# jibo27/3DGS_Hierarchical_Training

Measured on AMD Instinct MI355X. Metric: train-step images/sec + fwd+bwd ms @1M Gaussians, 980x545; 1/2/4/8 GPU, higher is better.
Workload: dtype f32

## Files before the change

### 3dgs_hierarchical_training_amd/csrc/gsr_kernels.hip

```cpp
#include <hip/hip_runtime.h>
#include <hip/hip_ext.h>
#include <type_traits>
#include <stdint.h>
#include <stdio.h>
#include <string.h>

#include <algorithm>
#include <atomic>
#include <chrono>
#include <cmath>
#include <map>
#include <mutex>
#include <tuple>
#include <vector>

#include "../../include/gsr.h"
#include "gsr_math.h"
#include "adam_math.h"
#include "radix_sort.h"
#include "blend_common.h"
#include "options.h"

#ifndef GSR_K9_UNROLL
#define GSR_K9_UNROLL 2
// ... 861 lines not shown
        uint32_t run = base + (idx ? s_incl[idx - 1] : 0u);
        for (int c0 = 0; c0 < full; c0 += 64) {
            const int c = c0 + lane;
            bool ok = false;
            int gx = 0, gy = 0;
            if (c < full) {
                const int ty = c / ww, tx = c - ty * ww;
                gx = x0 + tx; gy = y0 + ty;
                ok = tile_accept(tt, gx, gy, W, H);
            }
            const unsigned long long m = __ballot(ok);
            if (ok) {
                const uint32_t o = run + (uint32_t)__popcll(m & lt);
                if (o < cap) {
                    const uint32_t key = (uint32_t)((gy + vrow0) * tiles_x + gx);
                    out_tile[o] = (KeyT)key;
                    out_gid[o] = gg;
                    if (hist) count_key(key, o);
                }
            }
            run += (uint32_t)__popcll(m);
        }
    }
    if (hist) {
        __syncthreads();
#pragma unroll
        for (int q = 0; q < 8; q++) {
            const int e = q * kEmitThreads + tid, t = e >> 10, p = (e >> 8) & 3, d = e & 255;
            const uint32_t c = s_hist[t][p][d];
            if (c && x0 + (uint32_t)t < (uint32_t)kOsRanges) atomicAdd(&hz.ghist[((size_t)p * kOsRanges + x0 + t) * 256 + d], c);
        }
    }
}

template <typename KeyT>
__global__ __launch_bounds__(256) void k_tile_ranges(uint32_t R, const KeyT* __restrict__ keys, uint2* __restrict__ ranges,
                                                     const unsigned long long* __restrict__ n_dev)
{
    if (n_dev) R = (uint32_t)min((unsigned long long)R, *n_dev);
    constexpr uint32_t KPV = 16 / (uint32_t)sizeof(KeyT);
    const uint32_t i0 = (blockIdx.x * 256u + threadIdx.x) * KPV;
    if (i0 >= R) return;
    uint32_t t[KPV];
    if (i0 + KPV <= R && (((uintptr_t)keys & 15) == 0)) {
        const uint4 q = *reinterpret_cast<const uint4*>(keys + i0);
        const uint32_t w[4] = {q.x, q.y, q.z, q.w};
#pragma unroll
        for (uint32_t c = 0; c < KPV; c++) t[c] = sizeof(KeyT) == 4 ? w[c] : ((w[c / 2] >> (16 * (c & 1))) & 0xffffu);
    } else {
#pragma unroll
        for (uint32_t c = 0; c < KPV; c++) t[c] = i0 + c < R ? (uint32_t)keys[i0 + c] : 0u;
    }
    uint32_t prev = i0 ? (uint32_t)keys[i0 - 1] : 0xffffffffu;
#pragma unroll
    for (uint32_t c = 0; c < KPV; c++) {
        const uint32_t i = i0 + c;
        if (i < R) {
            if (i == 0) ranges[t[c]].x = 0;
            else if (prev != t[c]) { ranges[prev].y = i; ranges[t[c]].x = i; }
            if (i == R - 1) ranges[t[c]].y = R;
            prev = t[c];
        }
    }
}

constexpr int kDbMaxTiles = 4096;
constexpr int kDbCountWaves = 4;
struct DirectBin {
    int N, T, Tp , S, NC, G, Cg;
    uint16_t* M;
    uint32_t* GT;
    uint32_t* tbase;
    uint32_t* bsum;
};

constexpr uint32_t kCutOpenKey = 0xffffffffu;
struct ListCut {
    uint32_t* key;
    uint32_t* owner_n;
    uint32_t* stats;
    const uint32_t* cur;
    uint16_t* chunk;
    uint32_t* hist;
    uint32_t* tend;
    uint32_t* flag;
    uint32_t* ctl;
    uint32_t* bkey;
    const uint32_t* skey;
    const uint32_t* tbase;
    float margin;
    int dmax;
};

template <typename F>
__device__ __forceinline__ void big_rect_tiles(const Splat& s, uint32_t rect, int W, int H, int tiles_x, int tiles_y, int lane, F&& f)
{
    int x0, y0, x1, y1;
    tile_rect_tight(s.px, s.py, s.radius, s.ca, s.cb, s.cc, s.op, W, H, tiles_x, tiles_y, x0, y0, x1, y1);
    const int vrow0 = (int)((rect >> 12) & 0xfffu) - y0;
    const int ww = x1 - x0, full = ww * (y1 - y0);
    const TileTest tt = make_tile_test(s.px, s.py, s.ca, s.cb, s.cc, s.op);
    for (int c0 = 0; c0 < full; c0 += 64) {
        const int c = c0 + lane;
        bool ok = false;
        uint32_t key = 0u;
        if (c < full) {
            const int ty = c / ww, tx = c - ty * ww;
            ok = tile_accept(tt, x0 + tx, y0 + ty, W, H);
            key = (uint32_t)((y0 + ty + vrow0) * tiles_x + x0 + tx);
        }
        f(ok, key);
    }
}

template <typename F>
__device__ __forceinline__ void small_rect_tiles(const TileRec& r, int tiles_x, F&& f)
{
    const uint32_t ww = (r.rect >> 24) & 63u, rx0 = r.rect & 0xfffu, ry0 = (r.rect >> 12) & 0xfffu;
    const uint32_t rcp = (65536u + ww - 1u) / (ww ? ww : 1u);
    const uint32_t base = ry0 * (uint32_t)tiles_x + rx0, skip = (uint32_t)tiles_x - ww;
    for (uint32_t m = r.mask; m != 0u;) {
        const uint32_t m1 = m & (m - 1u);
        const uint32_t p0 = (uint32_t)__builtin_ctz(m);
        f(base + p0 + ((p0 * rcp) >> 16) * skip);
        if (m1 != 0u) {
            const uint32_t p1 = (uint32_t)__builtin_ctz(m1);
            f(base + p1 + ((p1 * rcp) >> 16) * skip);
        }
        m = m1 & (m1 - 1u);
    }
}

__device__ __forceinline__ uint32_t wave_inclusive_sum(uint32_t x)
{
#if defined(__HIP_DEVICE_COMPILE__)
    auto dpp = [](uint32_t v, auto ctrl, auto rmask, auto bmask) {
        return (uint32_t)__builtin_amdgcn_update_dpp(0, (int)v, decltype(ctrl)::value, decltype(rmask)::value, decltype(bmask)::value, false);
    };
    using std::integral_constant;
    uint32_t r = x;
    r += dpp(x, integral_constant<int, 0x111>{}, integral_constant<int, 0xf>{}, integral_constant<int, 0xf>{});
    r += dpp(x, integral_constant<int, 0x112>{}, integral_constant<int, 0xf>{}, integral_constant<int, 0xf>{});
    r += dpp(x, integral_constant<int, 0x113>{}, integral_constant<int, 0xf>{}, integral_constant<int, 0xf>{});
    r += dpp(r, integral_constant<int, 0x114>{}, integral_constant<int, 0xf>{}, integral_constant<int, 0xe>{});
    r += dpp(r, integral_constant<int, 0x118>{}, integral_constant<int, 0xf>{}, integral_constant<int, 0xc>{});
    r += dpp(r, integral_constant<int, 0x142>{}, integral_constant<int, 0xa>{}, integral_constant<int, 0xf>{});
    r += dpp(r, integral_constant<int, 0x143>{}, integral_constant<int, 0xc>{}, integral_constant<int, 0xf>{});
    return r;
#else
    return x;
#endif
}

__global__ __launch_bounds__(kEmitThreads) void k_chunk_counts(DirectBin db, int W, int H, int tiles_x, int tiles_y,
                                                               const uint32_t* __restrict__ sorted_gid, const TileRec* __restrict__ tilerec,
                                                               const Splat* __restrict__ splat, TileRec* __restrict__ sorted_rec, BlendBalance bb,
                                                               OsRider rider = OsRider{}, ListCut cut = ListCut{})
{
    const int nbuild = bb.hdr ? 8 : 0, c = (int)blockIdx.x - nbuild;
    if (c < 0) { balance_build(bb, (int)blockIdx.x); return; }
    if (cut.key && threadIdx.x == 0) {
        cut.bkey[c] = cut.skey[(size_t)c * db.S];
        cut.hist[c] = 0u;
        if (c == 0) { cut.ctl[0] = (uint32_t)(db.NC - 1); cut.ctl[1] = 0u; cut.ctl[2] = 0u; }
    }
    if (rider.host && blockIdx.x == gridDim.x - 1) {
        __shared__ unsigned long long s_r[2][16];
        onesweep_rider_publish(rider, s_r);
    }
    extern __shared__ uint32_t s_h[];
    const int tid = threadIdx.x, lane = tid & 63, wave = tid >> 6;
    for (int i = tid; i < db.Tp / 2; i += kEmitThreads) s_h[i] = 0u;
    __syncthreads();
    const int j0 = c * db.S + wave * 64, j1 = min(db.N, c * db.S + db.S);
    constexpr int kStride = 64 * kDbCountWaves;
    auto load_gid = [&](int j) -> uint32_t { return j < j1 ? (sorted_gid ? sorted_gid[j] : (uint32_t)j) : 0xffffffffu; };
    auto load_rec = [&](uint32_t g) -> TileRec { TileRec r; r.mask = 0u; r.rect = 1u << 24; if (g != 0xffffffffu) r = tilerec[g]; return r; };
    uint32_t gA = load_gid(j0 + lane), gB = load_gid(j0 + kStride + lane);
    TileRec rA = load_rec(gA);
    for (int j = j0 + lane; j - lane < j1; j += kStride) {
        const uint32_t g = gA;
        const TileRec r = rA;
        gA = gB;
        rA = load_rec(gA);
        gB = load_gid(j + 2 * kStride);
        if (sorted_rec && j < j1) sorted_rec[j] = r;
        const bool big = (r.rect & kTileRecBig) != 0u;
        if (!big) small_rect_tiles(r, tiles_x, [&](uint32_t t) { atomicAdd(&s_h[t >> 1], 1u << (16u * (t & 1u))); });
        for (unsigned long long bm = __ballot(big && r.mask != 0u); bm != 0ull; bm &= bm - 1ull) {
            const int b = (int)__builtin_ctzll(bm);
            const uint32_t gg = (uint32_t)__builtin_amdgcn_readlane((int)g, b), rect = (uint32_t)__builtin_amdgcn_readlane((int)r.rect, b);
            const Splat s = splat[gg];
            big_rect_tiles(s, rect, W, H, tiles_x, tiles_y, lane, [&](bool ok, uint32_t t) { if (ok) atomicAdd(&s_h[t >> 1], 1u << (16u * (t & 1u))); });
        }
    }
    __syncthreads();
    uint32_t* const row = reinterpret_cast<uint32_t*>(db.M + (size_t)c * db.Tp);
    for (int i = tid; i < db.Tp / 2; i += kEmitThreads) row[i] = s_h[i];
}

__global__ __launch_bounds__(256) void k_chunk_scan1(DirectBin db)
{
    __shared__ uint32_t s_w[4];
    const int tid = threadIdx.x, t = (int)(blockIdx.x * 256u) + tid, grp = (int)blockIdx.y;
    uint32_t run = 0u;
    if (t < db.Tp) {
        const int c0 = grp * db.Cg, c1 = min(db.NC, c0 + db.Cg);
        uint16_t* p = db.M + (size_t)c0 * db.Tp + t;
        int c = c0;
        for (; c + 8 <= c1; c += 8, p += 8 * (size_t)db.Tp) {
            uint32_t v[8];
#pragma unroll
            for (int k = 0; k < 8; k++) v[k] = p[(size_t)k * db.Tp];
#pragma unroll
            for (int k = 0; k < 8; k++) { p[(size_t)k * db.Tp] = (uint16_t)run; run += v[k]; }
        }
        for (; c < c1; c++, p += db.Tp) { const uint32_t v = *p; *p = (uint16_t)run; run += v; }
        db.GT[(size_t)grp * db.Tp + t] = run;
    }
    const uint32_t inc = wave_inclusive_sum(run);
    if ((tid & 63) == 63) s_w[tid >> 6] = inc;
    __syncthreads();
    if (tid == 0) db.bsum[(size_t)grp * gridDim.x + blockIdx.x] = s_w[0] + s_w[1] + s_w[2] + s_w[3];
}

constexpr int kDbMaxGroups = 64;
__global__ __launch_bounds__(256) void k_chunk_scan2(DirectBin db, unsigned long long* __restrict__ total_out, ZeroJobs zj,
                                                     unsigned long long* __restrict__ host_out, unsigned long long host_seq,
                                                     const unsigned int* __restrict__ window_overflow, unsigned long long* __restrict__ late_out = nullptr,
                                                     ListCut cut = ListCut{})
{
    extern __shared__ uint32_t s_bkey[];
    __shared__ unsigned long long s_lo[4], s_all[4];
    if (cut.key)
        for (int i = threadIdx.x; i < db.NC; i += 256) s_bkey[i] = cut.bkey[i];
    __shared__ uint32_t s_w[4];
    const int tid = threadIdx.x, lane = tid & 63, wave = tid >> 6;
    const int slab = (int)blockIdx.x, nslab = (int)gridDim.x, t = slab * 256 + tid;
#pragma unroll
    for (int j = 0; j < 3; j++) {
        uint32_t* z = static_cast<uint32_t*>(zj.p[j]);
        for (uint32_t q = (uint32_t)(slab * 256 + tid); q < zj.words[j]; q += (uint32_t)nslab * 256u) z[q] = 0u;
    }
    unsigned long long lo = 0ull, all = 0ull;
    for (int i = tid; i < db.G * nslab; i += 256) {
        const uint32_t v = db.bsum[i];
        all += v;
        if (i % nslab < slab) lo += v;
    }
#pragma unroll
    for (int off = 32; off > 0; off >>= 1) { lo += __shfl_xor(lo, off, 64); all += __shfl_xor(all, off, 64); }
    if (lane == 0) { s_lo[wave] = lo; s_all[wave] = all; }
    uint32_t tot = 0u;
    if (t < db.Tp) {
        uint32_t v[kDbMaxGroups];
#pragma unroll
        for (int g = 0; g < kDbMaxGroups; g++) v[g] = g < db.G ? db.GT[(size_t)g * db.Tp + t] : 0u;
#pragma unroll
        for (int g = 0; g < kDbMaxGroups; g++) {
            if (g < db.G) db.GT[(size_t)g * db.Tp + t] = tot;
            tot += v[g];
        }
    }
    if (t >= db.T) tot = 0u;
    const uint32_t inc = wave_inclusive_sum(tot);
    if (lane == 63) s_w[wave] = inc;
    __syncthreads();
    lo = s_lo[0] + s_lo[1] + s_lo[2] + s_lo[3];
    all = s_all[0] + s_all[1] + s_all[2] + s_all[3];
    uint32_t add = 0u;
#pragma unroll
    for (int w = 0; w < 4; w++) add += w < wave ? s_w[w] : 0u;
    const uint32_t base_t = (uint32_t)min(lo + add + inc - tot, 0xffffffffull);
    if (t < db.T) db.tbase[t] = base_t;
    if (cut.key) {
        if (t < db.T) {
            const uint32_t e = cut.cur[0] < (uint32_t)kVcEntries ? cut.cur[0] : 0u;
            const bool use = cut.cur[9] != 0u && cut.owner_n[e] == (uint32_t)db.N;
            uint32_t ck = (uint32_t)(db.NC - 1);
            const uint32_t k = use ? cut.key[(size_t)e * db.T + t] : kCutOpenKey;
            if (k != kCutOpenKey && k != 0u) {
                const float d = __uint_as_float(k);
                const uint32_t kc = __float_as_uint(fmaf(d, cut.margin, d));
                int a = 0, b = db.NC;
                while (a < b) { const int m = (a + b) >> 1; if (s_bkey[m] <= kc) a = m + 1; else b = m; }
                ck = (uint32_t)max(a - 1, 0);
            }
            cut.chunk[t] = (uint16_t)ck;
            cut.flag[t] = 0u;
            if (use) atomicAdd(&cut.hist[ck], 1u);
            if (t == 0) cut.ctl[3] = use ? 1u : 0u;
        }
    }
    if (slab == 0 && tid == 0) {
        db.tbase[db.T] = (uint32_t)min(all, 0xffffffffull);
        *total_out = all;
        if (host_out) {
            __atomic_store_n(host_out + 2, (unsigned long long)g_onesweep_giveups, __ATOMIC_RELAXED);
            __atomic_store_n(host_out + 3, (unsigned long long)(window_overflow ? *window_overflow : 0u), __ATOMIC_RELAXED);
            __atomic_store_n(host_out, all, __ATOMIC_RELAXED);
            __threadfence_system();
            __atomic_store_n(host_out + 1, host_seq, __ATOMIC_RELAXED);
            __threadfence_system();
        }
        if (late_out) scan_report_late(late_out, all, host_seq);
    }
}

constexpr int kDbPairs = 1024;
__device__ __forceinline__ void lds_order() { __builtin_amdgcn_fence(__ATOMIC_ACQ_REL, "wavefront"); __builtin_amdgcn_wave_barrier(); }

__device__ __forceinline__ uint32_t cut_frame(const ListCut& cut, const int NC, uint32_t& deep)
{
    const int lane = threadIdx.x & 63;
    deep = 0u;
    if (cut.ctl[3] == 0u) return (uint32_t)(NC - 1);
    constexpr int kR = 32;
    uint32_t v[kR];
#pragma unroll
    for (int q = 0; q < kR; q++) { const int c = NC - 1 - 64 * q - lane; v[q] = (64 * q < NC && c >= 0) ? cut.hist[c] : 0u; }
    uint32_t acc = 0u;
#pragma unroll
    for (int q = 0; q < kR; q++) {
        if (64 * q >= NC) break;
        const int c = NC - 1 - 64 * q - lane;
        const uint32_t inc = acc + wave_inclusive_sum(v[q]);
        const unsigned long long over = __ballot(c >= 0 && inc > (uint32_t)cut.dmax);
        if (over) {
            const int l = (int)__builtin_ctzll(over);
            deep = (uint32_t)__builtin_amdgcn_readlane((int)(inc - v[q]), l);
            return (uint32_t)(NC - 1 - 64 * q - l);
        }
        acc = (uint32_t)__builtin_amdgcn_readlane((int)inc, 63);
    }
    for (int top = NC - 1 - 64 * kR; top >= 0; top -= 64) {
        const int c = top - lane;
        const uint32_t w = c >= 0 ? cut.hist[c] : 0u;
        const uint32_t inc = acc + wave_inclusive_sum(w);
        const unsigned long long over = __ballot(c >= 0 && inc > (uint32_t)cut.dmax);
        if (over) {
            const int l = (int)__builtin_ctzll(over);
            deep = (uint32_t)__builtin_amdgcn_readlane((int)(inc - w), l);
            return (uint32_t)(top - l);
        }
        acc = (uint32_t)__builtin_amdgcn_readlane((int)inc, 63);
    }
    deep = acc;
    return 0u;
}

template <typename Want>
__device__ __forceinline__ void cut_chunk_tiles(const DirectBin& db, const int c, const int W, const int H, const int tiles_x, const int tiles_y,
                                                const uint32_t* __restrict__ sorted_gid, const TileRec* __restrict__ sorted_rec,
                                                const Splat* __restrict__ splat, uint32_t* __restrict__ list, const uint32_t cap,
                                                uint32_t* s_txy , uint32_t* s_pos , Want&& want)
{
    const int lane = threadIdx.x & 63;
    const unsigned long long lt = lanemask_lt();
    const int j0 = c * db.S, j1 = min(db.N, j0 + db.S);
    const uint32_t* gt = db.GT + (size_t)(c / db.Cg) * db.Tp;
    const uint16_t* mr = db.M + (size_t)c * db.Tp;
    auto load_rec = [&](int j) -> TileRec { TileRec r; r.mask = 0u; r.rect = 1u << 24; if (j < j1) r = sorted_rec[j]; return r; };
    auto load_gid = [&](int j) -> uint32_t { return j < j1 ? sorted_gid[j] : 0u; };
    unsigned long long mine = 0ull;
#pragma unroll
    for (int q = 0; q < kDbMaxTiles / 64; q++) {
        const int t = 64 * q + lane;
        if (64 * q < db.T && t < db.T && want((uint32_t)t)) mine |= 1ull << q;
    }
    for (int t0 = 0; t0 < db.T;) {
        int nt = 0;
        while (t0 < db.T) {
            const int t = t0 + lane;
            const bool w = ((mine >> (t0 >> 6)) & 1ull) != 0ull;
            const unsigned long long b = __ballot(w);
            const int got = (int)__popcll(b);
            if (nt + got > 64) break;
            if (w) {
                const int k = nt + (int)__popcll(b & lt);
                s_txy[k] = ((uint32_t)(t / tiles_x) << 16) | (uint32_t)(t % tiles_x);
                s_pos[k] = db.tbase[t] + gt[t] + (uint32_t)mr[t];
            }
            nt += got;
            t0 += 64;
        }
        if (nt == 0) break;
        lds_order();
        TileRec rA = load_rec(j0 + lane), rB = load_rec(j0 + 64 + lane);
        uint32_t gA = load_gid(j0 + lane), gB = load_gid(j0 + 64 + lane);
        for (int j = j0; j < j1; j += 64) {
            const TileRec r = rA;
            const uint32_t g = gA;
            rA = rB; gA = gB;
            rB = load_rec(j + 128 + lane);
            gB = load_gid(j + 128 + lane);
            const bool big = (r.rect & kTileRecBig) != 0u && r.mask != 0u;
            const uint32_t ww = (r.rect >> 24) & 63u, rx0 = r.rect & 0xfffu, ry0 = (r.rect >> 12) & 0xfffu;
            TileTest tt = {};
            int bx0 = 0, by0 = 0, bx1 = 0, by1 = 0;
            if (big) {
                const Splat sp = splat[g];
                tile_rect_tight(sp.px, sp.py, sp.radius, sp.ca, sp.cb, sp.cc, sp.op, W, H, tiles_x, tiles_y, bx0, by0, bx1, by1);
                tt = make_tile_test(sp.px, sp.py, sp.ca, sp.cb, sp.cc, sp.op);
            }
            const bool any_big = __ballot(big) != 0ull;
            for (int k = 0; k < nt; k++) {
                const uint32_t txy = s_txy[k], tx = txy & 0xffffu, ty = txy >> 16;
                const uint32_t dx = tx - rx0, dy = ty - ry0, bit = dy * ww + dx;
                bool in = !big && dx < ww && bit < 32u && ((r.mask >> bit) & 1u) != 0u;
                if (any_big && big) in = (int)tx >= bx0 && (int)tx < bx1 && (int)ty >= by0 && (int)ty < by1 && tile_accept(tt, (int)tx, (int)ty, W, H);
                const unsigned long long b = __ballot(in);
                if (b == 0ull) continue;
                const uint32_t p0 = s_pos[k];
                if (in) { const uint32_t pos = p0 + (uint32_t)__popcll(b & lt); if (pos < cap) list[pos] = g; }
                lds_order();
                if (lane == 0) s_pos[k] = p0 + (uint32_t)__popcll(b);
                lds_order();
            }
        }
        lds_order();
    }
}

#ifdef GSR_DB_TIMING
__device__ unsigned long long g_db_dbg[16];
#define DB_T(k) do { const unsigned long long now_ = __builtin_readcyclecounter(); if (lane == 0) dbt[k] += now_ - dbt_last; dbt_last = now_; } while (0)
#else
#define DB_T(k) do { } while (0)
#endif
template <bool PAIRS = false, int CUT = 0>
__global__ __launch_bounds__(64) void k_chunk_scatter(DirectBin db, int W, int H, int tiles_x, int tiles_y,
                                                      const uint32_t* __restrict__ sorted_gid, const TileRec* __restrict__ sorted_rec,
                                                      const Splat* __restrict__ splat, uint32_t* __restrict__ list, uint2* __restrict__ ranges,
                                                      uint32_t cap, const uint32_t* __restrict__ dkey = nullptr, uint2* __restrict__ pairs = nullptr,
                                                      ListCut cut = ListCut{})
{
    static_assert(!CUT || !PAIRS, "the list cut serves the plain direct binning");
    extern __shared__ unsigned long long s_dyn[];
    const int LT = db.Tp;
    unsigned long long* const s_mask = s_dyn;
    uint32_t* const s_cnt = reinterpret_cast<uint32_t*>(s_dyn + LT);
    uint32_t* const s_pair = s_cnt + LT;
    const int lane = threadIdx.x, b = (int)blockIdx.x;
    if (CUT == 2 && cut.ctl[2] == 0u) return;
    uint32_t cstar = 0u, ndeep = 0u;
    if (CUT == 1) cstar = cut_frame(cut, db.NC, ndeep);
    if (CUT == 2) cstar = cut.ctl[0];
    {
        const int t = b * 64 + lane;
        if (t < db.T) {
            uint32_t tend = db.tbase[t + 1];
            if (CUT == 1) {
                const uint32_t c1 = max((uint32_t)cut.chunk[t], cstar) + 1u;
                if (c1 < (uint32_t)db.NC) tend = db.tbase[t] + db.GT[(size_t)(c1 / (uint32_t)db.Cg) * db.Tp + t] + (uint32_t)db.M[(size_t)c1 * db.Tp + t];
                cut.tend[t] = tend;
            }
            const uint32_t lo = min(db.tbase[t], cap), hi = min(tend, cap);
            if (CUT != 2 || cut.flag[t]) ranges[t] = hi > lo ? make_uint2(lo, hi) : make_uint2(0u, 0u);
            if (CUT == 1) {
                const uint32_t e = cut.cur[0] < (uint32_t)kVcEntries ? cut.cur[0] : 0u;
                cut.key[(size_t)e * db.T + t] = 0u;
            }
        }
        if (CUT && b == 0 && lane == 0) {
            if (CUT == 1) {
                const uint32_t e = cut.cur[0] < (uint32_t)kVcEntries ? cut.cur[0] : 0u;
                cut.owner_n[e] = (uint32_t)db.N;
                cut.ctl[0] = cstar; cut.ctl[1] = ndeep;
                cut.stats[0] += 1u;
                cut.stats[3] += (uint32_t)(db.NC - 1) - min(cstar, (uint32_t)(db.NC - 1));
                cut.stats[4] += ndeep;
            } else { cut.stats[1] += 1u; cut.stats[2] += cut.ctl[2]; }
        }
    }
    const int per = (db.NC + 7) >> 3, kk = b >> 3, c = (b & 7) * per + kk;
    if (kk >= per || c >= db.NC) return;
    if (CUT && (uint32_t)c > cstar) {
        if (CUT == 1 && ndeep == 0u) return;
        uint32_t* const s_tile = s_pair;
        uint32_t* const s_pos = s_pair + 64;
        if (CUT == 1) cut_chunk_tiles(db, c, W, H, tiles_x, tiles_y, sorted_gid, sorted_rec, splat, list, cap, s_tile, s_pos,
                                      [&](uint32_t t) { return (uint32_t)cut.chunk[t] >= (uint32_t)c; });
        else cut_chunk_tiles(db, c, W, H, tiles_x, tiles_y, sorted_gid, sorted_rec, splat, list, cap, s_tile, s_pos,
                             [&](uint32_t t) { return cut.flag[t] != 0u && (uint32_t)cut.chunk[t] < (uint32_t)c; });
        return;
    }
    if (CUT == 2) return;
#ifdef GSR_DB_TIMING
    unsigned long long dbt[8] = {0, 0, 0, 0, 0, 0, 0, 0}, dbt_last = __builtin_readcyclecounter();
#endif
    {
        const uint32_t* gt = db.GT + (size_t)(c / db.Cg) * db.Tp;
        const uint16_t* mr = db.M + (size_t)c * db.Tp;
        constexpr int kRows = 36;
        for (int i0 = 0; i0 < LT; i0 += 64 * kRows) {
            uint32_t tb[kRows], gb[kRows], mc[kRows];
#pragma unroll
            for (int q = 0; q < kRows; q++) {
                const int i = i0 + 64 * q + lane;
                const bool v = i < LT && (uint32_t)i < (uint32_t)LT;
                tb[q] = v && i < db.T ? db.tbase[i] : 0u;
                gb[q] = v ? gt[i] : 0u;
                mc[q] = v ? (uint32_t)mr[i] : 0u;
            }
#pragma unroll
            for (int q = 0; q < kRows; q++) {
                const int i = i0 + 64 * q + lane;
                if (i < LT) { s_cnt[i] = tb[q] + gb[q] + mc[q]; s_mask[i] = 0ull; }
            }
        }
    }
    lds_order();
    DB_T(0);
    const unsigned long long me = 1ull << lane, lt = lanemask_lt();
    const int j0 = c * db.S, j1 = min(db.N, j0 + db.S);
    auto load_gid = [&](int j) -> uint32_t { return j < j1 ? (PAIRS ? (uint32_t)j : sorted_gid[j]) : 0u; };
    auto load_rec = [&](int j) -> TileRec { TileRec r; r.mask = 0u; r.rect = 1u << 24; if (j < j1) r = sorted_rec[j]; return r; };
    auto load_key = [&](int j) -> uint32_t { return (PAIRS && j < j1) ? dkey[j] : 0u; };
    uint32_t gA = load_gid(j0 + lane), gB = load_gid(j0 + 64 + lane);
    TileRec rA = load_rec(j0 + lane), rB = load_rec(j0 + 64 + lane);
    uint32_t kA = load_key(j0 + lane), kB = load_key(j0 + 64 + lane);
    for (int j = j0 + lane; j - lane < j1; j += 64) {
        const uint32_t g = gA;
        TileRec r = rA;
        const uint32_t kd = kA;
        gA = gB; rA = rB; kA = kB;
        gB = load_gid(j + 128);
        rB = load_rec(j + 128);
        kB = load_key(j + 128);
        const bool big = (r.rect & kTileRecBig) != 0u && r.mask != 0u, huge = big && r.mask > (uint32_t)kDbPairs;
        const unsigned long long bigs = __ballot(big && !huge), huges = __ballot(huge);
        const uint32_t cnt = huge ? 0u : tilerec_count(r);
        const uint32_t incl = wave_inclusive_sum(cnt);
        auto run_end = [&](int lo, uint32_t before) -> int {
            const unsigned long long over = __ballot(incl - before > (uint32_t)kDbPairs) & ~((1ull << lo) - 1ull);
            return over ? (int)__builtin_ctzll(over) : 64;
        };
        auto owners = [&](int lo, int hi, uint32_t before, bool with_or) {
            const bool mine = lane >= lo && lane < hi;
            if (!big && (with_or || mine)) {
                uint32_t* o = s_pair + (incl - cnt - before);
                small_rect_tiles(r, tiles_x, [&](uint32_t t) {
                    if (with_or) atomicOr(&s_mask[t], me);
                    if (mine) *o++ = (t << 6) | (uint32_t)lane;
                });
            }
            for (unsigned long long bm = bigs; bm != 0ull; bm &= bm - 1ull) {
                const int bl = (int)__builtin_ctzll(bm);
                const bool in_run = bl >= lo && bl < hi;
                if (!with_or && !in_run) continue;
                const uint32_t gg = (uint32_t)__builtin_amdgcn_readlane((int)g, bl), rect = (uint32_t)__builtin_amdgcn_readlane((int)r.rect, bl);
                uint32_t o = (uint32_t)__builtin_amdgcn_readlane((int)(incl - cnt), bl) - before;
                const Splat s = splat[gg];
                big_rect_tiles(s, rect, W, H, tiles_x, tiles_y, lane, [&](bool ok, uint32_t t) {
                    const unsigned long long acc = __ballot(ok);
                    if (ok) {
                        if (with_or) atomicOr(&s_mask[t], 1ull << bl);
                        if (in_run) s_pair[(o + (uint32_t)__popcll(acc & lt)) & (uint32_t)(kDbPairs - 1)] = (t << 6) | (uint32_t)bl;
                    }
                    o += (uint32_t)__popcll(acc);
                });
            }
        };
        int lo = 0, hi = run_end(0, 0u);
        uint32_t before = 0u;
        const bool one_run = hi == 64;
        DB_T(1);
        owners(0, hi, 0u, true);
        DB_T(2);
        for (unsigned long long bm = huges; bm != 0ull; bm &= bm - 1ull) {
            const int bl = (int)__builtin_ctzll(bm);
            const uint32_t gg = (uint32_t)__builtin_amdgcn_readlane((int)g, bl), rect = (uint32_t)__builtin_amdgcn_readlane((int)r.rect, bl);
            const Splat s = splat[gg];
            big_rect_tiles(s, rect, W, H, tiles_x, tiles_y, lane, [&](bool ok, uint32_t t) { if (ok && t < (uint32_t)db.T) atomicOr(&s_mask[t], 1ull << bl); });
        }
        asm volatile("" : "+v"(gA), "+v"(rA.mask), "+v"(rA.rect));
        if (PAIRS) asm volatile("" : "+v"(kA));
        lds_order();
        DB_T(3);
        for (;;) {
            const uint32_t P = (uint32_t)__builtin_amdgcn_readlane((int)incl, hi - 1) - before;
            for (uint32_t p0 = 0u; p0 < P; p0 += 512u) {
                const uint32_t left = P - p0;
                auto batch = [&](auto rounds_tag) {
                    constexpr int RN = decltype(rounds_tag)::value;
                    uint32_t e[RN], go[RN], base[RN], ko[PAIRS ? RN : 1];
                    unsigned long long mk[RN];
#pragma unroll
                    for (int q = 0; q < RN; q++) e[q] = s_pair[(p0 + 64u * q + (uint32_t)lane) & (uint32_t)(kDbPairs - 1)];
#pragma unroll
                    for (int q = 0; q < RN; q++) {
                        const bool v = 64u * q + (uint32_t)lane < left;
                        e[q] = v ? e[q] : 0xffffffffu;
                        const uint32_t t = v ? e[q] >> 6 : 0u;
                        go[q] = (uint32_t)__builtin_amdgcn_ds_bpermute((int)((e[q] & 63u) << 2), (int)g);
                        if (PAIRS) ko[q] = (uint32_t)__builtin_amdgcn_ds_bpermute((int)((e[q] & 63u) << 2), (int)kd);
                        mk[q] = s_mask[t];
                        base[q] = s_cnt[t];
                    }
#pragma unroll
                    for (int q = 0; q < RN; q++)
                        if (e[q] != 0xffffffffu) {
                            const uint32_t pos = base[q] + (uint32_t)__popcll(mk[q] & ((1ull << (e[q] & 63u)) - 1ull));
                            if (pos < cap) {
                                if (PAIRS) pairs[pos] = make_uint2(ko[q], go[q]);
                                else list[pos] = go[q];
                            }
                        }
                };
                if (left <= 128u) batch(std::integral_constant<int, 2>{});
                else if (left <= 256u) batch(std::integral_constant<int, 4>{});
                else if (left <= 384u) batch(std::integral_constant<int, 6>{});
                else batch(std::integral_constant<int, 8>{});
            }
            if (hi == 64) break;
            lds_order();
            before += P;
            lo = hi;
            hi = run_end(lo, before);
            owners(lo, hi, before, false);
            lds_order();
        }
        for (unsigned long long bm = huges; bm != 0ull; bm &= bm - 1ull) {
            const int bl = (int)__builtin_ctzll(bm);
            const uint32_t gg = (uint32_t)__builtin_amdgcn_readlane((int)g, bl), rect = (uint32_t)__builtin_amdgcn_readlane((int)r.rect, bl);
            const Splat s = splat[gg];
            big_rect_tiles(s, rect, W, H, tiles_x, tiles_y, lane, [&](bool ok, uint32_t t) {
                if (ok && t < (uint32_t)db.T) {
                    const uint32_t pos = s_cnt[t] + (uint32_t)__popcll(s_mask[t] & ((1ull << bl) - 1ull));
                    if (pos < cap) {
                        if (PAIRS) pairs[pos] = make_uint2((uint32_t)__builtin_amdgcn_readlane((int)kd, bl), gg);
                        else list[pos] = gg;
                    }
                }
            });
        }
        lds_order();
        DB_T(4);
        if (one_run) {
            const uint32_t P = (uint32_t)__builtin_amdgcn_readlane((int)incl, 63);
            for (uint32_t p0 = 0u; p0 < P; p0 += 512u) {
                const uint32_t left = P - p0;
                auto batch = [&](auto rounds_tag) {
                    constexpr int RN = decltype(rounds_tag)::value;
                    uint32_t e[RN];
#pragma unroll
                    for (int q = 0; q < RN; q++) e[q] = s_pair[(p0 + 64u * q + (uint32_t)lane) & (uint32_t)(kDbPairs - 1)];
#pragma unroll
                    for (int q = 0; q < RN; q++)
                        if (64u * q + (uint32_t)lane < left) { atomicAdd(&s_cnt[e[q] >> 6], 1u); s_mask[e[q] >> 6] = 0ull; }
                };
                if (left <= 128u) batch(std::integral_constant<int, 2>{});
                else if (left <= 256u) batch(std::integral_constant<int, 4>{});
                else if (left <= 384u) batch(std::integral_constant<int, 6>{});
                else batch(std::integral_constant<int, 8>{});
            }
        } else {
            if (!big) small_rect_tiles(r, tiles_x, [&](uint32_t t) { atomicAdd(&s_cnt[t], 1u); s_mask[t] = 0ull; });
            for (unsigned long long bm = bigs; bm != 0ull; bm &= bm - 1ull) {
                const int bl = (int)__builtin_ctzll(bm);
                const uint32_t gg = (uint32_t)__builtin_amdgcn_readlane((int)g, bl), rect = (uint32_t)__builtin_amdgcn_readlane((int)r.rect, bl);
                const Splat s = splat[gg];
                big_rect_tiles(s, rect, W, H, tiles_x, tiles_y, lane, [&](bool ok, uint32_t t) { if (ok && t < (uint32_t)db.T) { atomicAdd(&s_cnt[t], 1u); s_mask[t] = 0ull; } });
            }
        }
        for (unsigned long long bm = huges; bm != 0ull; bm &= bm - 1ull) {
            const int bl = (int)__builtin_ctzll(bm);
            const uint32_t gg = (uint32_t)__builtin_amdgcn_readlane((int)g, bl), rect = (uint32_t)__builtin_amdgcn_readlane((int)r.rect, bl);
            const Splat s = splat[gg];
            big_rect_tiles(s, rect, W, H, tiles_x, tiles_y, lane, [&](bool ok, uint32_t t) { if (ok && t < (uint32_t)db.T) { atomicAdd(&s_cnt[t], 1u); s_mask[t] = 0ull; } });
        }
        lds_order();
        DB_T(5);
    }
#ifdef GSR_DB_TIMING
    if (lane == 0) {
        for (int k = 0; k < 6; k++) atomicAdd(&g_db_dbg[k], dbt[k]);
        atomicAdd(&g_db_dbg[6], 1ull);
        atomicAdd(&g_db_dbg[7], (unsigned long long)((j1 - j0 + 63) / 64));
    }
#endif
}

constexpr int kTsCap = 4096, kTsSmallMax = 1024;

template <int THREADS, int IPT, bool GATHER = false>
__device__ __forceinline__ void tile_sort_regs(const uint2* __restrict__ src, uint32_t* dst, uint32_t n, const uint32_t* __restrict__ dkey,
                                               unsigned long long (*s_mask)[256], uint32_t (*s_cnt)[256], uint32_t* s_keys, uint32_t* s_vals,
                                               uint32_t* s_start, uint32_t* s_wsum, uint32_t* s_bits)
{
    constexpr int WAVES = THREADS / 64;
    const int tid = threadIdx.x, wave = tid >> 6, lane = tid & 63;
    uint32_t key[IPT], val[IPT], dig[IPT], rnk[IPT];
    uint32_t k_or = 0u, k_and = 0xffffffffu;
#pragma unroll
    for (int r = 0; r < IPT; r++) {
        const uint32_t p = (uint32_t)(wave * (IPT * 64) + r * 64 + lane);
        if (GATHER) val[r] = p < n ? dst[p] : 0u;
        else if (p < n) { const uint2 e = src[p]; key[r] = e.x; val[r] = e.y; }
        if (!GATHER && p >= n) { key[r] = 0xffffffffu; val[r] = 0u; }
    }
    if (GATHER) {
#pragma unroll
        for (int r = 0; r < IPT; r++) {
            const uint32_t p = (uint32_t)(wave * (IPT * 64) + r * 64 + lane);
            key[r] = p < n ? dkey[val[r]] : 0xffffffffu;
        }
    }
#pragma unroll
    for (int r = 0; r < IPT; r++) {
        const uint32_t p = (uint32_t)(wave * (IPT * 64) + r * 64 + lane);
        if (p < n) { k_or |= key[r]; k_and &= key[r]; }
    }
#pragma unroll
    for (int off = 32; off > 0; off >>= 1) { k_or |= (uint32_t)__shfl_xor((int)k_or, off, 64); k_and &= (uint32_t)__shfl_xor((int)k_and, off, 64); }
    if (lane == 0) { s_bits[wave] = k_or; s_bits[WAVES + wave] = k_and; }
    __syncthreads();
    uint32_t differ = 0u;
    {
        uint32_t o = 0u, a = 0xffffffffu;
#pragma unroll
        for (int w = 0; w < WAVES; w++) { o |= s_bits[w]; a &= s_bits[WAVES + w]; }
        differ = o & ~a;
    }
#pragma unroll 1
    for (int shift = 0; shift < 32; shift += 8) {
        if (((differ >> shift) & 0xffu) == 0u) continue;
#pragma unroll
        for (int r = 0; r < IPT; r++) dig[r] = (key[r] >> shift) & 0xffu;
        wave_rank<IPT, 256>(s_mask[wave], s_cnt[wave], dig, rnk, lane);
        __syncthreads();
        uint32_t mine = 0u;
        if (tid < 256) {
#pragma unroll
            for (int w = 0; w < WAVES; w++) { const uint32_t c = s_cnt[w][tid]; s_cnt[w][tid] = mine; mine += c; }
        }
        const uint32_t ex = block_scan_excl<WAVES>(mine, s_wsum, tid);
        if (tid < 256) s_start[tid] = ex;
        __syncthreads();
#pragma unroll
        for (int r = 0; r < IPT; r++) {
            const uint32_t lp = s_start[dig[r]] + s_cnt[wave][dig[r]] + rnk[r];
            s_keys[lp] = key[r]; s_vals[lp] = val[r];
        }
        __syncthreads();
#pragma unroll
        for (int r = 0; r < IPT; r++) {
            const uint32_t p = (uint32_t)(wave * (IPT * 64) + r * 64 + lane);
            key[r] = s_keys[p]; val[r] = s_vals[p];
        }
        __syncthreads();
    }
#pragma unroll
    for (int r = 0; r < IPT; r++) {
        const uint32_t p = (uint32_t)(wave * (IPT * 64) + r * 64 + lane);
        if (p < n) dst[p] = val[r];
    }
}

template <int IPT, bool GATHER>
__device__ __forceinline__ void tile_sort_wave(const uint2* __restrict__ src, uint32_t* dst, uint32_t n, const uint32_t* __restrict__ dkey,
                                               unsigned long long* s_mask, uint32_t* s_cnt, uint32_t* s_start, uint32_t* s_keys, uint32_t* s_vals)
{
    const int lane = threadIdx.x;
    uint32_t key[IPT], val[IPT], dig[IPT], rnk[IPT];
#pragma unroll
    for (int r = 0; r < IPT; r++) {
        const uint32_t p = (uint32_t)(r * 64 + lane);
        if (GATHER) val[r] = p < n ? dst[p] : 0u;
        else if (p < n) { const uint2 e = src[p]; key[r] = e.x; val[r] = e.y; }
        if (!GATHER && p >= n) { key[r] = 0xffffffffu; val[r] = 0u; }
    }
    if (GATHER) {
#pragma unroll
        for (int r = 0; r < IPT; r++) key[r] = (uint32_t)(r * 64 + lane) < n ? dkey[val[r]] : 0xffffffffu;
    }
    uint32_t k_or = 0u, k_and = 0xffffffffu;
#pragma unroll
    for (int r = 0; r < IPT; r++)
        if ((uint32_t)(r * 64 + lane) < n) { k_or |= key[r]; k_and &= key[r]; }
#pragma unroll
    for (int off = 32; off > 0; off >>= 1) { k_or |= (uint32_t)__shfl_xor((int)k_or, off, 64); k_and &= (uint32_t)__shfl_xor((int)k_and, off, 64); }
    const uint32_t differ = k_or & ~k_and;
#pragma unroll 1
    for (int shift = 0; shift < 32; shift += 8) {
        if (((differ >> shift) & 0xffu) == 0u) continue;
#pragma unroll
        for (int r = 0; r < IPT; r++) dig[r] = (key[r] >> shift) & 0xffu;
        wave_rank<IPT, 256>(s_mask, s_cnt, dig, rnk, lane);
        lds_order();
        {
            const uint4 c = reinterpret_cast<const uint4*>(s_cnt)[lane];
            const uint32_t sum = c.x + c.y + c.z + c.w;
            const uint32_t ex = wave_inclusive_sum(sum) - sum;
            reinterpret_cast<uint4*>(s_start)[lane] = make_uint4(ex, ex + c.x, ex + c.x + c.y, ex + c.x + c.y + c.z);
        }
        lds_order();
#pragma unroll
        for (int r = 0; r < IPT; r++) {
            const uint32_t lp = s_start[dig[r]] + rnk[r];
            s_keys[lp] = key[r]; s_vals[lp] = val[r];
        }
        lds_order();
#pragma unroll
        for (int r = 0; r < IPT; r++) { key[r] = s_keys[r * 64 + lane]; val[r] = s_vals[r * 64 + lane]; }
        lds_order();
    }
#pragma unroll
    for (int r = 0; r < IPT; r++) {
        const uint32_t p = (uint32_t)(r * 64 + lane);
        if (p < n) dst[p] = val[r];
    }
}

template <bool GATHER = false>
__global__ __launch_bounds__(64) void k_tile_sort_wave(const uint2* __restrict__ ranges, const uint2* __restrict__ pairs, uint32_t* list, int T,
                                                       const uint32_t* __restrict__ dkey = nullptr)
{
    __shared__ unsigned long long s_mask[256];
    __shared__ __attribute__((aligned(16))) uint32_t s_cnt[256];
    __shared__ __attribute__((aligned(16))) uint32_t s_start[256];
    __shared__ uint32_t s_keys[kTsSmallMax], s_vals[kTsSmallMax];
    const int t = (int)blockIdx.x;
    if (t >= T) return;
    const uint2 rg = ranges[t];
    const uint32_t n = rg.y - rg.x;
    if (n == 0u || n > (uint32_t)kTsSmallMax) return;
    const uint2* src = pairs + rg.x;
    uint32_t* dst = list + rg.x;
    if (n <= 64u) tile_sort_wave<1, GATHER>(src, dst, n, dkey, s_mask, s_cnt, s_start, s_keys, s_vals);
    else if (n <= 128u) tile_sort_wave<2, GATHER>(src, dst, n, dkey, s_mask, s_cnt, s_start, s_keys, s_vals);
    else if (n <= 256u) tile_sort_wave<4, GATHER>(src, dst, n, dkey, s_mask, s_cnt, s_start, s_keys, s_vals);
    else if (n <= 512u) tile_sort_wave<8, GATHER>(src, dst, n, dkey, s_mask, s_cnt, s_start, s_keys, s_vals);
    else tile_sort_wave<16, GATHER>(src, dst, n, dkey, s_mask, s_cnt, s_start, s_keys, s_vals);
}

template <int THREADS, bool GATHER = false>
__global__ __launch_bounds__(THREADS) void k_tile_sort(const uint2* __restrict__ ranges, uint2* pairs, uint2* pairs_alt, uint32_t* list, int T,
                                                       const uint32_t* __restrict__ dkey = nullptr)
{
    constexpr int WAVES = THREADS / 64, CAP = THREADS == 256 ? kTsSmallMax : kTsCap;
    static_assert(CAP * 8 == WAVES * 256 * 8, "the pair buffer aliases the mask tables exactly");
    __shared__ unsigned long long s_mask[WAVES][256];
    __shared__ uint32_t s_cnt[WAVES][256];
    __shared__ uint32_t s_start[256], s_wsum[WAVES], s_bits[2 * WAVES], s_base[256], s_hist[256];
    uint32_t* const s_keys = reinterpret_cast<uint32_t*>(&s_mask[0][0]);
    uint32_t* const s_vals = s_keys + CAP;
    static_assert(THREADS == 1024, "the short segments are k_tile_sort_wave's");
    __shared__ uint32_t s_todo[256];
    __shared__ uint32_t s_ntodo;
    if (threadIdx.x == 0) s_ntodo = 0u;
    __syncthreads();
    for (int k = (int)threadIdx.x; (int)blockIdx.x + k * (int)gridDim.x < T; k += THREADS) {
        const int tt = (int)blockIdx.x + k * (int)gridDim.x;
        const uint2 q = ranges[tt];
        if (q.y - q.x > (uint32_t)kTsSmallMax) { const uint32_t slot = atomicAdd(&s_ntodo, 1u); if (slot < 256u) s_todo[slot] = (uint32_t)tt; }
    }
    __syncthreads();
    const uint32_t ntodo = s_ntodo;
    const bool walk_all = ntodo > 256u;
    const int nloop = walk_all ? (T - (int)blockIdx.x + (int)gridDim.x - 1) / (int)gridDim.x : (int)ntodo;
    for (int it = 0; it < nloop; it++) {
    const int t = walk_all ? (int)blockIdx.x + it * (int)gridDim.x : (int)s_todo[it];
    const uint2 rg = ranges[t];
    const uint32_t n = rg.y - rg.x;
    if (n <= (uint32_t)kTsSmallMax) continue;
    __syncthreads();
    if (n <= 2048u) { tile_sort_regs<THREADS, 2, GATHER>(pairs + rg.x, list + rg.x, n, dkey, s_mask, s_cnt, s_keys, s_vals, s_start, s_wsum, s_bits); continue; }
    if (n <= (uint32_t)kTsCap) { tile_sort_regs<THREADS, 4, GATHER>(pairs + rg.x, list + rg.x, n, dkey, s_mask, s_cnt, s_keys, s_vals, s_start, s_wsum, s_bits); continue; }
    const int tid = threadIdx.x, wave = tid >> 6, lane = tid & 63;
    constexpr int IPT = kTsCap / THREADS;
    uint2* src = pairs + rg.x;
    uint2* dst = pairs_alt + rg.x;
    if (GATHER) {
        for (uint32_t i = (uint32_t)tid; i < n; i += THREADS) { const uint32_t g = list[rg.x + i]; src[i] = make_uint2(dkey[g], g); }
        __syncthreads();
    }
    uint32_t k_or = 0u, k_and = 0xffffffffu;
    for (uint32_t i = (uint32_t)tid; i < n; i += THREADS) { const uint32_t k = src[i].x; k_or |= k; k_and &= k; }
#pragma unroll
    for (int off = 32; off > 0; off >>= 1) { k_or |= (uint32_t)__shfl_xor((int)k_or, off, 64); k_and &= (uint32_t)__shfl_xor((int)k_and, off, 64); }
    if (lane == 0) { s_bits[wave] = k_or; s_bits[WAVES + wave] = k_and; }
    __syncthreads();
    uint32_t differ = 0u;
    {
        uint32_t o = 0u, a = 0xffffffffu;
#pragma unroll
        for (int w = 0; w < WAVES; w++) { o |= s_bits[w]; a &= s_bits[WAVES + w]; }
        differ = o & ~a;
    }
#pragma unroll 1
    for (int shift = 0; shift < 32; shift += 8) {
        if (((differ >> shift) & 0xffu) == 0u) continue;
        __syncthreads();
        if (tid < 256) s_hist[tid] = 0u;
        __syncthreads();
        for (uint32_t i = (uint32_t)tid; i < n; i += THREADS) atomicAdd(&s_hist[(src[i].x >> shift) & 0xffu], 1u);
        __syncthreads();
        const uint32_t tot = tid < 256 ? s_hist[tid] : 0u;
        const uint32_t ex = block_scan_excl<WAVES>(tot, s_wsum, tid);
        if (tid < 256) s_base[tid] = ex;
        __syncthreads();
        for (uint32_t c0 = 0u; c0 < n; c0 += (uint32_t)kTsCap) {
            const uint32_t m = min((uint32_t)kTsCap, n - c0);
            uint32_t key[IPT], val[IPT], dig[IPT], rnk[IPT];
#pragma unroll
            for (int r = 0; r < IPT; r++) {
                const uint32_t p = (uint32_t)(wave * (IPT * 64) + r * 64 + lane);
                if (p < m) { const uint2 e = src[c0 + p]; key[r] = e.x; val[r] = e.y; dig[r] = (e.x >> shift) & 0xffu; }
                else { key[r] = 0xffffffffu; val[r] = 0u; dig[r] = 255u; }
            }
            wave_rank<IPT, 256>(s_mask[wave], s_cnt[wave], dig, rnk, lane);
            __syncthreads();
            uint32_t mine = 0u;
            if (tid < 256) {
#pragma unroll
                for (int w = 0; w < WAVES; w++) { const uint32_t c = s_cnt[w][tid]; s_cnt[w][tid] = mine; mine += c; }
                s_start[tid] = s_base[tid];
            }
            __syncthreads();
            if (tid < 256) s_base[tid] += mine - (tid == 255 ? (uint32_t)kTsCap - m : 0u);
#pragma unroll
            for (int r = 0; r < IPT; r++) {
                const uint32_t p = (uint32_t)(wave * (IPT * 64) + r * 64 + lane);
                if (p < m) dst[s_start[dig[r]] + s_cnt[wave][dig[r]] + rnk[r]] = make_uint2(key[r], val[r]);
            }
            __syncthreads();
        }
        uint2* tmp = src; src = dst; dst = tmp;
    }
    __syncthreads();
    for (uint32_t i = (uint32_t)tid; i < n; i += THREADS) list[rg.x + i] = src[i].y;
    }
}

#ifdef GSR_K6_TIMING
__device__ unsigned long long g_k6_dbg[4 * 65536];
__device__ unsigned long long g_k8_dbg[4 * 65536];
__device__ unsigned long long g_k6_cyc[2 * 65536];
__device__ uint32_t g_k6_cnt[2 * 65536];
#endif
#ifndef GSR_FWD_BUFS
#define GSR_FWD_BUFS 2
#endif
constexpr int kFwdBufs = GSR_FWD_BUFS;

struct ImpArgs {
    const float* color;
    float* S;
    float (*s_sum)[64];
    uint32_t* s_id;
};
constexpr int kImpStride = 4;
__device__ __forceinline__ float wave_swap_rows_sum(float t)
{
    {
        const unsigned u = __float_as_uint(t);
        const auto r = __builtin_amdgcn_permlane16_swap(u, u, false, false);
        t = __uint_as_float(r[0]) + __uint_as_float(r[1]);
    }
    {
        const unsigned u = __float_as_uint(t);
        const auto r = __builtin_amdgcn_permlane32_swap(u, u, false, false);
        t = __uint_as_float(r[0]) + __uint_as_float(r[1]);
    }
    return t;
}
__device__ __forceinline__ float wave_reduce_one(float v)
{
    return wave_swap_rows_sum(bfly_single<0x128>(bfly_single<0x124>(bfly_single<0x4E>(bfly_single<0xB1>(v)))));
}
__device__ __forceinline__ float wave_reduce_three(float v0, float v1, float v2, int lane)
{
    const float r01 = bfly_pair<0x124>(v0, v1, (lane & 4) != 0);
    const float r2 = bfly_single<0x124>(v2);
    const float q = bfly_pair<0x128>(r01, r2, (lane & 8) != 0);
    return wave_swap_rows_sum(bfly_single<0x4E>(bfly_single<0xB1>(q)));
}

template <bool IMP = false, bool LEAN = false, bool HAS_DA = true>
__device__ __forceinline__ void blend_fwd_item(const int xcd, const int kslot, float4 (*s_ab)[64], float2 (*s_c)[64],
                                               int W, int H, int tiles_x, int T, const uint2* __restrict__ ranges,
                                               const uint32_t* __restrict__ list, const Splat* __restrict__ splat,
                                               const float* __restrict__ bg, float* __restrict__ out_color,
                                               float* __restrict__ out_depth, float* __restrict__ out_alpha,
                                               float* __restrict__ img, uint32_t* __restrict__ staged4,
                                               float* __restrict__ ckpt, int kCkptFirst, int tiles_y, uint16_t* __restrict__ cost_out,
                                               float* __restrict__ out_clamped, const ListCut& cut, const int cut_pass,
                                               const ImpArgs imp = ImpArgs{})
{
    constexpr int NT = 64;
    uint32_t visits = 0u;
#ifdef GSR_K6_TIMING
    const unsigned long long dbg_t0 = wall_clock64();
    uint32_t dbg_visits = 0u, dbg_taken = 0u;
    unsigned long long dbg_stage = 0ull, dbg_loop = 0ull, dbg_mark = 0ull;
#endif
    const int tile = slot_tile(xcd, kslot >> 2, T, tiles_x);
    const int sub = kslot & 3;
    const int lane = (int)(threadIdx.x & 63u);
    if (tile < 0) { if (cost_out && lane == 0) cost_out[xcd + 8 * kslot] = 0; return; }
    if (cut_pass == 2 && cut.flag[tile] == 0u) return;
    const int Tl = tiles_x * tiles_y, bimg = tile / Tl, tl = tile - bimg * Tl;
    const int tx = tl % tiles_x, ty = tl / tiles_x;
    const int px = tx * kTile + (sub & 1) * 8 + (lane & 7);
    const int py = ty * kTile + (sub >> 1) * 8 + (lane >> 3);
    const float pxf = (float)((sub & 1) * 8 + (lane & 7)), pyf = (float)((sub >> 1) * 8 + (lane >> 3));
    const float tox = (float)(tx * kTile) - 0.5f * (float)W, toy = (float)(ty * kTile) - 0.5f * (float)H;
    const uint2 rg = ranges[tile];
    const int n = IMP ? min((int)(rg.y - rg.x), (int)staged4[tile * 4 + sub]) : (int)(rg.y - rg.x);
    const int nb = (n + NT - 1) / NT;
    const bool inside = px < W && py < H;
    float Tr = inside ? 1.f : -1.f;
    float C0 = 0.f, C1 = 0.f, C2 = 0.f, Dd = 0.f, Aa = 0.f;
    uint32_t last = 0;
    float g0 = 0.f, g1 = 0.f, g2 = 0.f;
    uint32_t lastp = 0u, id_rec = 0u;
    bool uni = false;
    if constexpr (IMP) {
        if (inside) {
            const size_t Pl = (size_t)W * H, P = Pl * (size_t)(T / Tl), pl = (size_t)py * W + px, pid = (size_t)bimg * Pl + pl;
            const float* oc = imp.color + (size_t)bimg * 3 * Pl + pl;
            const float o0 = oc[0], o1 = oc[Pl], o2 = oc[2 * Pl];
            g0 = (o0 >= 0.f && o0 <= 1.f) ? 1.f : 0.f;
            g1 = (o1 >= 0.f && o1 <= 1.f) ? 1.f : 0.f;
            g2 = (o2 >= 0.f && o2 <= 1.f) ? 1.f : 0.f;
            lastp = reinterpret_cast<const uint32_t*>(img)[P + pid];
        }
        const bool want = lastp > 0u && (g0 + g1 + g2) > 0.f;
        if (!__any(want)) return;
        Tr = want ? 1.f : -1.f;
        if (!want) g0 = g1 = g2 = 0.f;
        uni = __all(g0 == g1 && g1 == g2);
        imp.s_sum[0][lane] = 0.f; imp.s_sum[1][lane] = 0.f; imp.s_sum[2][lane] = 0.f;
    }
    float4 ra = {0, 0, 0, 0}, rb = ra, rc = ra;
    constexpr float kL2E = 1.4426950408889634f;
    const float sbx0 = (float)(tx * kTile + (sub & 1) * 8) - 0.5f * (float)W, sby0 = (float)(ty * kTile + (sub >> 1) * 8) - 0.5f * (float)H;
    const float sbx1 = fminf(sbx0 + 7.f, (float)(W - 1) - 0.5f * (float)W), sby1 = fminf(sby0 + 7.f, (float)(H - 1) - 0.5f * (float)H);
    uint32_t id_nn = 0u;
    auto fetch = [&](uint32_t id) {
        const float4* sp = reinterpret_cast<const float4*>(splat + id);
        ra = sp[0]; rb = sp[1]; rc = sp[2];
    };
    if (n > 0) {
        id_rec = list[rg.x + min(lane, n - 1)];
        fetch(id_rec);
        id_nn = list[rg.x + min(NT + lane, n - 1)];
    }
    int batches = 0;
    for (int b = 0; b < nb; b++) {
        const int buf = b & (kFwdBufs - 1);
        if (__all(Tr < 0.f)) break;
        if constexpr (!LEAN) {
        if (ckpt && !(b & 1) && (b >> 1) >= kCkptFirst) {
            float* c = ckpt + ((size_t)(rg.x >> 7) + tile + (b >> 1) - kCkptFirst) * kCkptFloats + sub * 64 + lane;
            c[0] = fabsf(Tr); c[256] = C0; c[512] = C1; c[768] = C2; c[1024] = Dd; c[1280] = Aa;
        }
        }
#ifdef GSR_K6_TIMING
        dbg_mark = __builtin_readcyclecounter();
#endif
        const int cnt = min(NT, n - b * NT);
        const bool reach_me = box_accept(make_tile_test(ra.x, ra.y, ra.z, ra.w, rb.x, rb.y), sbx0, sby0, sbx1, sby1);
        {
            const uint32_t lo = __float_as_uint(rc.w);
            ra.x = pixel_rel(ra.x, pixel_lo_x(lo), tox); ra.y = pixel_rel(ra.y, pixel_lo_y(lo), toy);
        }
        ra.z *= -0.5f * kL2E; ra.w *= -kL2E; rb.x *= -0.5f * kL2E;
        s_ab[buf][lane] = ra; s_ab[kFwdBufs + buf][lane] = rb;
        if constexpr (IMP) imp.s_id[lane] = id_rec;
        else s_c[buf][lane] = make_float2(rc.x, rc.y);
        const unsigned long long reach = __ballot(reach_me && lane < cnt);
        visits += (uint32_t)__popcll(reach);
        __builtin_amdgcn_fence(__ATOMIC_RELEASE, "wavefront");
        __builtin_amdgcn_wave_barrier();
        __builtin_amdgcn_fence(__ATOMIC_ACQUIRE, "wavefront");
        batches = b + 1;
#ifdef GSR_K6_TIMING
        { const unsigned long long t = __builtin_readcyclecounter(); dbg_stage += t - dbg_mark; dbg_mark = t; }
#endif
        const int nxt = (b + 1) * NT + lane;
        fetch(id_nn);
        if constexpr (IMP) id_rec = id_nn;
        id_nn = list[rg.x + min(nxt + NT, n - 1)];
        auto alpha_of = [&](int j, float& p2) {
// ... 1354 lines not shown
                d_shs[(size_t)(base + g) * row + e] = e < NC3 ? s_sh[g * kShStride + e] : 0.f;
            }
        }
    }
}

__global__ __launch_bounds__(256) void k_det_iota(uint32_t R, uint32_t* __restrict__ pos, const uint32_t* __restrict__ list, uint32_t* __restrict__ ids,
                                                  uint32_t n_gaussians)
{
    const uint32_t i = blockIdx.x * 256u + threadIdx.x;
    if (i < R) { pos[i] = i; ids[i] = min(list[i], n_gaussians - 1u); }
}
__global__ __launch_bounds__(256) void k_det_reduce(uint32_t R, const uint32_t* __restrict__ gid_sorted, const uint32_t* __restrict__ pos_sorted,
                                                    const float* __restrict__ part, double* __restrict__ ggrad)
{
    const uint32_t i = blockIdx.x * 256u + threadIdx.x;
    if (i >= R) return;
    const uint32_t g = gid_sorted[i];
    if (i > 0 && gid_sorted[i - 1] == g) return;
    double acc[kDetStride];
#pragma unroll
    for (int r = 0; r < kDetStride; r++) acc[r] = 0.0;
    for (uint32_t j = i; j < R && gid_sorted[j] == g; j++) {
        const float* p = part + (size_t)pos_sorted[j] * kDetStride;
#pragma unroll
        for (int r = 0; r < kDetStride; r++) acc[r] += (double)p[r];
    }
#pragma unroll
    for (int r = 0; r < kDetStride; r++) ggrad[(size_t)g * kGG + r] = acc[r];
}

__global__ __launch_bounds__(256) void k_cam_reduce(const float* __restrict__ partial, int nblocks, float* __restrict__ d_vm,
                                                    float* __restrict__ d_pm, float* __restrict__ d_campos, float* __restrict__ d_xf,
                                                    BatchDev bt)
{
    __shared__ double s[256];
    const int q = blockIdx.x, m = blockIdx.y;
    int lo = 0, hi = nblocks;
    if (bt.B > 1) {
#pragma unroll
        for (int k = 0; k < kMaxBatch; k++)
            if (k == m) { lo = bt.first_block[k]; hi = min(nblocks, bt.first_block[k + 1]); }
        if (d_vm) d_vm += 16 * m;
        if (d_pm) d_pm += 16 * m;
        if (d_campos) d_campos += 3 * m;
        if (d_xf) d_xf += 12 * m;
    }
    double a = 0;
    for (int b = lo + threadIdx.x; b < hi; b += 256) a += partial[(size_t)b * kCamVals + q];
    s[threadIdx.x] = a;
    __syncthreads();
    for (int off = 128; off > 0; off >>= 1) {
        if (threadIdx.x < off) s[threadIdx.x] += s[threadIdx.x + off];
        __syncthreads();
    }
    if (threadIdx.x == 0) {
        const float v = (float)s[0];
        if (q < 16) { if (d_vm) d_vm[q] = v; }
        else if (q < 32) { if (d_pm) d_pm[q - 16] = v; }
        else if (q < 35) { if (d_campos) d_campos[q - 32] = v; }
        else if (d_xf) d_xf[q - 35] = v;
    }
}

struct GeomLayout {
    size_t splat;
    size_t total;
};
static GeomLayout geom_layout(int32_t N)
{
    GeomLayout g;
    g.splat = 0;
    g.total = align256((size_t)(N > 0 ? N : 1) * sizeof(Splat));
    return g;
}

struct PrepLayout {
    size_t splat, radii, dkey, gid, rec, sort, early, bytes;
};
static PrepLayout prep_layout(int32_t N)
{
    const size_t n = (size_t)(N > 0 ? N : 1);
    PrepLayout p;
    size_t o = 0;
    p.splat = o; o += align256(n * sizeof(Splat));
    p.radii = o; o += align256(n * 4);
    p.dkey = o; o += align256(n * 4);
    p.gid = o; o += align256(n * 4);
    p.rec = o; o += align256(n * sizeof(TileRec));
    p.sort = o; o += align256(onesweep_scratch_bytes((uint32_t)n));
    p.early = o; o += align256(((n + kPreThreads - 1) / kPreThreads) * sizeof(uint2));
    p.bytes = o;
    return p;
}

struct FwdScratch {
    size_t dkey, gid, dkey_alt, gid_alt, ntiles, srec, block_sums, total, early, sort;
    size_t bytes;
};
static FwdScratch fwd_scratch_layout(int32_t N)
{
    const size_t n = (size_t)(N > 0 ? N : 1);
    FwdScratch s;
    size_t o = 0;
    s.dkey = o; o += align256(n * 4);
    s.gid = o; o += align256(n * 4);
    s.dkey_alt = o; o += align256(n * 4);
    s.gid_alt = o; o += align256(n * 4);
    s.ntiles = o; o += align256(n * sizeof(TileRec));
    s.srec = o; o += align256(n * sizeof(TileRec));
    s.block_sums = o; o += align256(((n + kEmitThreads - 1) / kEmitThreads) * 4);
    s.total = o; o += 256;
    s.early = o; o += align256(((n + kPreThreads - 1) / kPreThreads) * sizeof(uint2));
    s.sort = o; o += onesweep_scratch_bytes((uint32_t)n);
    s.bytes = o;
    return s;
}

struct BinLayout {
    size_t list, ranges, ckpt, items, bytes;
};

static size_t bwd_list_cap(int64_t R, size_t T) { return ((size_t)(R > 0 ? R : 0) >> 7) + T + 8; }
static BinLayout bin_layout(int64_t R, int32_t W, int32_t H, int32_t B = 1)
{
    const size_t T = (size_t)((W + kTile - 1) / kTile) * ((H + kTile - 1) / kTile) * (size_t)(B > 1 ? B : 1);
    BinLayout b;
    b.ranges = 0;
    b.list = align256((T ? T : 1) * sizeof(uint2));
    b.ckpt = b.list + align256((size_t)(R > 0 ? R : 1) * 4);
    b.items = b.ckpt + align256((((size_t)(R > 0 ? R : 0) >> 7) + T + 1) * kCkptFloats * sizeof(float));
    b.bytes = b.items + kItemHdrBytes + align256(8 * bwd_list_cap(R, T) * sizeof(uint2));
    return b;
}

struct BinScratch {
    size_t tile, tile_alt, gid_alt, sort, bytes;
};
static BinScratch bin_scratch_layout(int64_t R, int key_bytes = 4)
{
    const size_t r = (size_t)(R > 0 ? R : 1);
    BinScratch s;
    size_t o = 0;
    s.tile = o; o += align256(r * (size_t)key_bytes);
    s.tile_alt = o; o += align256(r * (size_t)key_bytes);
    s.gid_alt = o; o += align256(r * 4);
    s.sort = o; o += onesweep_scratch_bytes((uint32_t)r);
    s.bytes = o;
    return s;
}

struct ViewCostCache { int dev, W, H, items; uint8_t* mem; size_t bytes; };
static std::vector<ViewCostCache> g_view_costs;
static std::map<std::tuple<int, int, int, int>, bool> g_full_depth_sort;

struct PinSlot { unsigned long long* host = nullptr; unsigned long long* dev = nullptr; bool busy = false;
                 unsigned long long seq = 0;
                 bool pending = false; unsigned long long pending_seq = 0, pending_R = 0, pending_giveups = 0; };
static std::mutex g_state_mutex;
static std::map<int, std::vector<PinSlot*>> g_pin_slots;
static std::map<std::tuple<int, int, int, int>, uint64_t> g_hints;
static long long g_hint_override = -1;
static long long g_late_bias = 0;
static std::atomic<long long> g_spec_overflows{0}, g_spec_forwards{0}, g_exact_forwards{0}, g_depth_window_resorts{0};
static std::atomic<long long> g_fwd_calls{0}, g_fwd_ns{0}, g_fwd_wait_ns{0}, g_bwd_calls{0}, g_bwd_ns{0}, g_frozen_bwd_calls{0};
struct CallTimer {
    std::atomic<long long>&calls, &ns;
    std::chrono::steady_clock::time_point t0 = std::chrono::steady_clock::now();
    CallTimer(std::atomic<long long>& c, std::atomic<long long>& n) : calls(c), ns(n) {}
    ~CallTimer() { calls++; ns += std::chrono::duration_cast<std::chrono::nanoseconds>(std::chrono::steady_clock::now() - t0).count(); }
};

static int n_bucket(int N) { return N > 0 ? (int)std::floor(2.0 * std::log2((double)N)) : 0; }

static PinSlot* acquire_pin_slot(int dev)
{
    std::lock_guard<std::mutex> lk(g_state_mutex);
    auto& v = g_pin_slots[dev];
    for (PinSlot* s : v)
        if (!s->busy) { s->busy = true; return s; }
    PinSlot* s = new PinSlot();
    if (hipHostMalloc((void**)&s->host, 64, hipHostMallocMapped) != hipSuccess ||
        hipHostGetDevicePointer((void**)&s->dev, s->host, 0) != hipSuccess) { delete s; return nullptr; }
    s->host[0] = 0; s->host[1] = 0;
    for (int q = 4; q < 8; q++) s->host[q] = 0;
    s->busy = true;
    v.push_back(s);
    return s;
}
static std::atomic<long long> g_late_checks{0}, g_late_mismatches{0};
static int late_check(PinSlot* s, bool wait, unsigned long long* got_total, unsigned long long* want_total)
{
    if (!s->pending) return 0;
    volatile unsigned long long* hp = s->host;
    if (hp[5] != s->pending_seq) {
        if (!wait) return 0;
        const auto limit = std::chrono::steady_clock::now() + std::chrono::milliseconds(200);
        while (hp[5] != s->pending_seq && std::chrono::steady_clock::now() < limit) cpu_relax();
        if (hp[5] != s->pending_seq) { (void)hipDeviceSynchronize(); }
        if (hp[5] != s->pending_seq) { s->pending = false; return 0; }
    }
    std::atomic_thread_fence(std::memory_order_acquire);
    s->pending = false;
    g_late_checks++;
    *got_total = hp[4]; *want_total = s->pending_R;
    if (hp[4] != s->pending_R || hp[6] != s->pending_giveups) { g_late_mismatches++; return 1; }
    return 0;
}
struct PinLease {
    PinSlot* s;
    explicit PinLease(PinSlot* s_) : s(s_) {}
    ~PinLease() { if (s) { std::lock_guard<std::mutex> lk(g_state_mutex); s->busy = false; } }
};

static inline int64_t pack_fwd_flags(int ckpt_first)
{
    return 1 | ((int64_t)7 << 1) | ((int64_t)2 << 4) | ((int64_t)ckpt_first << 6) | ((int64_t)1 << 13);
}
static inline bool flags_from_forward(int64_t flags) { return ((flags >> 1) & 7) == 7 && ((flags >> 4) & 3) == 2; }

static int batch_dev(const GsrBatch* bt, int32_t N, int32_t H, BatchDev& out)
{
    out = BatchDev{};
    out.B = 1;
    if (!bt || bt->B <= 1) return GSR_OK;
    if (bt->B > kMaxBatch || !bt->first_block) return fail(GSR_ERR_ARG, "batch: 2..16 models and a first_block table expected%s");
    const int nblocks = (N + kPreThreads - 1) / kPreThreads;
    if (bt->first_block[0] != 0 || bt->first_block[bt->B] != nblocks || (N % kPreThreads) != 0)
        return fail(GSR_ERR_ARG, "batch: first_block must run from 0 to N / 128 and N must be a multiple of 128 (pad every model)%s");
    for (int q = 0; q < bt->B; q++)
        if (bt->first_block[q + 1] < bt->first_block[q]) return fail(GSR_ERR_ARG, "batch: first_block must be non-decreasing%s");
    if ((long long)bt->B * ((H + kTile - 1) / kTile) > 4095) return fail(GSR_ERR_RANGE, "batch: more than 4095 tile rows in total%s");
    out.B = bt->B;
    for (int q = 0; q <= bt->B; q++) out.first_block[q] = bt->first_block[q];
    for (int q = bt->B + 1; q <= kMaxBatch; q++) out.first_block[q] = nblocks;
    return GSR_OK;
}

static int check_common(int32_t N, int32_t M, int32_t D, int32_t W, int32_t H)
{
    if (N < 0 || W <= 0 || H <= 0) return fail(GSR_ERR_ARG, "bad sizes%s");
    if (D < 0 || D > 3) return fail(GSR_ERR_ARG, "sh_degree must be 0..3%s");
    if (M < 0 || M > 16) return fail(GSR_ERR_ARG, "at most 16 SH coefficients per Gaussian%s");
    if (W > 4095 * kTile || H > 4095 * kTile) return fail(GSR_ERR_RANGE, "image side longer than 65520 pixels%s");
    return GSR_OK;
}

template <typename KeyT>
static int sort_pairs_entry(KeyT* keys, uint32_t* vals, KeyT* keys_alt, uint32_t* vals_alt, uint32_t n, int begin_bit, int end_bit, void* scratch,
                            size_t scratch_bytes, int* result_in_alt, void* stream)
{
    if (!result_in_alt) return fail(GSR_ERR_ARG, "sort: result_in_alt is null%s");
    if (scratch_bytes < onesweep_scratch_bytes(n)) return fail(GSR_ERR_ARG, "sort scratch too small%s");
    if (begin_bit < 0 || end_bit <= begin_bit || end_bit > 8 * (int)sizeof(KeyT)) return fail(GSR_ERR_ARG, "sort bit range outside the key%s");
    GSR_HIP(onesweep_sort_pairs<KeyT>(keys, vals, keys_alt, vals_alt, n, begin_bit, end_bit, scratch, result_in_alt, (hipStream_t)stream));
    return GSR_OK;
}

}

using namespace gsr;

extern "C" {

size_t gsr_geom_bytes(int32_t N) { return geom_layout(N).total; }
static size_t image_balance_offset(int32_t W, int32_t H, int32_t B) { return align256((size_t)W * H * (size_t)(B > 1 ? B : 1) * kImgPlanes * 4); }
static size_t image_balance_bytes(int32_t W, int32_t H, int32_t B)
{
    if (B > 1) return 0;
    const int tiles_x = (W + kTile - 1) / kTile, T = tiles_x * ((H + kTile - 1) / kTile);
    return 256 + align256((size_t)32 * slots_per_xcd(T, tiles_x) * sizeof(uint16_t) + 64);
}
static size_t image_staged_offset(int32_t W, int32_t H, int32_t B) { return image_balance_offset(W, H, B) + image_balance_bytes(W, H, B); }
size_t gsr_image_staged_offset(int32_t W, int32_t H) { return image_staged_offset(W, H, 1); }
size_t gsr_image_bytes_batched(int32_t W, int32_t H, int32_t B)
{
    const size_t T = (size_t)((W + kTile - 1) / kTile) * ((H + kTile - 1) / kTile) * (size_t)(B > 1 ? B : 1);
    return image_staged_offset(W, H, B) + align256(T * 4 * 4);
}
size_t gsr_image_bytes(int32_t W, int32_t H) { return gsr_image_bytes_batched(W, H, 1); }

int gsr_profile_read(const char* name, double* total_ms, int64_t* count)
{
    if (!name || !total_ms || !count) return GSR_ERR_ARG;
    for (int id = 0; id < P_COUNT; id++) {
        if (strcmp(name, kProfNames[id])) continue;
        std::lock_guard<std::mutex> lk(g_prof_mutex);
        double tot = 0; int64_t n = 0;
        for (auto& p : g_prof_events[id]) {
            float ms = 0.f;
            if (hipEventSynchronize(p.b) == hipSuccess && hipEventElapsedTime(&ms, p.a, p.b) == hipSuccess) { tot += ms; n++; }
            (void)hipEventDestroy(p.a); (void)hipEventDestroy(p.b);
        }
        g_prof_events[id].clear();
        *total_ms = tot; *count = n;
        return GSR_OK;
    }
    return GSR_ERR_ARG;
}
size_t gsr_forward_scratch_bytes(int32_t N) { return fwd_scratch_layout(N).bytes; }
size_t gsr_binning_bytes(int64_t R, int32_t W, int32_t H) { return bin_layout(R, W, H).bytes; }
size_t gsr_binning_scratch_bytes(int64_t R) { return bin_scratch_layout(R).bytes; }
size_t gsr_backward_scratch_bytes(int32_t N)
{
    const size_t n = (size_t)(N > 0 ? N : 1);
    return align256(n * kGG * sizeof(double)) + align256(((n + kPreThreads - 1) / kPreThreads) * kCamVals * 4);
}
size_t gsr_sort_scratch_bytes(uint32_t n) { return onesweep_scratch_bytes(n); }
size_t gsr_prepared_bytes(int32_t N) { return prep_layout(N).bytes; }
size_t gsr_prepared_radii_offset(int32_t N) { return prep_layout(N).radii; }
int gsr_prepare_supported(int32_t M, int32_t D, int32_t raw_params) { return (raw_params && M == 16 && D >= 0 && D <= 3) ? 1 : 0; }
const char* gsr_last_error(void) { return g_err; }
int gsr_version(void) { return 122; }
size_t gsr_struct_bytes(int32_t which)
{
    return which == 0 ? sizeof(GsrForwardArgs) : which == 1 ? sizeof(GsrBackwardArgs) : which == 2 ? sizeof(GsrForwardOut) : 0;
}

#ifdef GSR_K8_PHASES
int gsr_debug_k8_phases(unsigned long long* host_dst) { return (int)hipMemcpyFromSymbol(host_dst, HIP_SYMBOL(g_k8ph), sizeof(unsigned long long) * 8 * 8192); }
#endif
#ifdef GSR_OS_TIMING
int gsr_debug_os_timing(unsigned long long* host_dst) { return (int)hipMemcpyFromSymbol(host_dst, HIP_SYMBOL(g_os_dbg), sizeof(unsigned long long) * 8 * 4096); }
int gsr_debug_gh_timing(unsigned long long* host_dst) { return (int)hipMemcpyFromSymbol(host_dst, HIP_SYMBOL(g_gh_dbg), sizeof(unsigned long long) * 8 * 512); }
#endif
#ifdef GSR_K9_TIMING
int gsr_debug_k9_timing(unsigned long long* host_dst, int reset)
{
    (void)reset;
    return (int)hipMemcpyFromSymbol(host_dst, HIP_SYMBOL(g_k9_dbg), sizeof(unsigned long long) * 8 * kK9DbgWaves);
}
#endif
#ifdef GSR_DB_TIMING
int gsr_debug_db_timing(unsigned long long* host_dst) { return (int)hipMemcpyFromSymbol(host_dst, HIP_SYMBOL(g_db_dbg), sizeof(unsigned long long) * 16); }
#endif
#ifdef GSR_K6_TIMING
int gsr_debug_k6_timing(unsigned long long* host_dst, int blocks)
{
    return (int)hipMemcpyFromSymbol(host_dst, HIP_SYMBOL(g_k6_dbg), sizeof(unsigned long long) * 4 * (size_t)blocks);
}
int gsr_debug_k6_counts(uint32_t* host_dst, int blocks)
{
    return (int)hipMemcpyFromSymbol(host_dst, HIP_SYMBOL(g_k6_cnt), sizeof(uint32_t) * 2 * (size_t)blocks);
}
int gsr_debug_k6_cycles(unsigned long long* host_dst, int blocks)
{
    return (int)hipMemcpyFromSymbol(host_dst, HIP_SYMBOL(g_k6_cyc), sizeof(unsigned long long) * 2 * (size_t)blocks);
}
int gsr_debug_k8_timing(unsigned long long* host_dst, int blocks)
{
    return (int)hipMemcpyFromSymbol(host_dst, HIP_SYMBOL(g_k8_dbg), sizeof(unsigned long long) * 4 * (size_t)blocks);
}
#endif
int gsr_set_option(const char* name, int value)
{
    if (!name) return GSR_ERR_ARG;
    switch (options_set(name, value)) {
        case SetResult::Stored: return GSR_OK;
        case SetResult::Refused: return GSR_ERR_ARG;
        case SetResult::Unknown: break;
    }
    if (!strcmp(name, "view_cache_reset")) {
        int dev_id = 0;
        if (hipGetDevice(&dev_id) != hipSuccess || hipDeviceSynchronize() != hipSuccess) return GSR_ERR_HIP;
        std::lock_guard<std::mutex> lk(g_state_mutex);
        for (auto& c : g_view_costs)
            if (c.dev == dev_id && hipMemset(c.mem, 0, c.bytes) != hipSuccess) return GSR_ERR_HIP;
        return GSR_OK;
    }
    if (!strcmp(name, "debug_late_bias")) {
        std::lock_guard<std::mutex> lk(g_state_mutex);
        g_late_bias = value;
        return GSR_OK;
    }
    if (!strcmp(name, "binning_capacity_hint")) {
        std::lock_guard<std::mutex> lk(g_state_mutex);
        g_hint_override = value > 0 ? value : -1;
        return GSR_OK;
    }
    if (!strcmp(name, "reset_speculation")) {
        std::lock_guard<std::mutex> lk(g_state_mutex);
        g_hints.clear(); g_hint_override = -1;
        g_spec_overflows = 0; g_spec_forwards = 0; g_exact_forwards = 0; g_depth_window_resorts = 0;
        g_full_depth_sort.clear();
        return GSR_OK;
    }
    if (!strcmp(name, "profile")) { g_profile = (value == 2 || value == 3) ? value : (value ? 1 : 0); g_profile_tick = 0; return GSR_OK; }
    return GSR_ERR_ARG;
}

struct DirectBinScratch { size_t M, GT, tbase, bsum, cut_chunk, cut_tend, cut_flag, cut_ctl, cut_bkey, cut_hist, bytes; };
static bool direct_bin_geometry(int N, int T, DirectBin& db, DirectBinScratch& ds)
{
    if (N < 1 || T < 1 || T > kDbMaxTiles) return false;
    static std::atomic<int> cus_cached{0};
    int cus = cus_cached.load(std::memory_order_relaxed);
    if (!cus) {
        int dev = 0, n = 0;
        cus = (hipGetDevice(&dev) == hipSuccess && hipDeviceGetAttribute(&n, hipDeviceAttributeMultiprocessorCount, dev) == hipSuccess && n > 0) ? n : 256;
        cus_cached.store(cus, std::memory_order_relaxed);
    }
    db.N = N; db.T = T; db.Tp = (T + 63) & ~63;
    const int lds = 12 * db.Tp + 4 * kDbPairs;
    const int per_cu = std::min(16, (160 * 1024) / lds);
    const long long resident = std::max<long long>(1, (long long)cus * per_cu);
    const int min_s = 128;
    long long S = ((long long)N + resident - 1) / resident;
    S = std::max<long long>(min_s, (S + 63) & ~63ll);
    if (S > 65472) return false;
    db.S = (int)S;
    db.NC = (int)(((long long)N + S - 1) / S);
    int G = 1;
    while (G * G < db.NC) G++;
    db.Cg = std::max(1, std::min((db.NC + G - 1) / G, 65535 / db.S));
    db.G = (db.NC + db.Cg - 1) / db.Cg;
    if (db.G > kDbMaxGroups) return false;
    size_t o = 0;
    ds.M = o; o += align256((size_t)db.NC * db.Tp * sizeof(uint16_t));
    ds.GT = o; o += align256((size_t)db.G * db.Tp * sizeof(uint32_t));
    ds.tbase = o; o += align256((size_t)(db.Tp + 1) * sizeof(uint32_t));
    ds.bsum = o; o += align256((size_t)db.G * ((db.Tp + 255) / 256) * sizeof(uint32_t));
    ds.cut_chunk = o; o += align256((size_t)db.Tp * sizeof(uint16_t));
    ds.cut_tend = o; o += align256((size_t)db.Tp * sizeof(uint32_t));
    ds.cut_flag = o; o += align256((size_t)db.Tp * sizeof(uint32_t));
    ds.cut_ctl = o; o += 256;
    ds.cut_bkey = o; o += align256((size_t)db.NC * sizeof(uint32_t));
    ds.cut_hist = o; o += align256((size_t)db.NC * sizeof(uint32_t));
    ds.bytes = o;
    return true;
}

static int forward_impl(const GsrForwardArgs* a, const int32_t* retired_at, int64_t retire_step, GsrForwardOut* out, void* stream_)
{
    CallTimer call_timer(g_fwd_calls, g_fwd_ns);
    hipStream_t st = (hipStream_t)stream_;
    if (!a || !out) return fail(GSR_ERR_ARG, "null args%s");
    const Options opt = options_snapshot();
    int rc = check_common(a->N, a->M, a->D, a->W, a->H);
    if (rc) return rc;
    const bool ro = a->render_only != 0;
    if (retired_at) {
        if (ro) return fail(GSR_ERR_ARG, "retired_at: a retire table is not served with render_only (no training step, nothing to retire)%s");
        if (retire_step < 1 || retire_step > 0x7fffffffll) return fail(GSR_ERR_ARG, "retired_at: retire_step must be the 1-based step of the call%s");
    }
    if (ro) {
        if ((a->out_depth == nullptr) != (a->out_alpha == nullptr))
            return fail(GSR_ERR_ARG, "render_only: out_depth and out_alpha are given both or neither%s");
        if ((a->batch && a->batch->B > 1) || a->prepared)
            return fail(GSR_ERR_ARG, "render_only is not served with a batch of B > 1 or a prepared buffer%s");
        if (!a->out_color || !a->bg || !a->alloc) return fail(GSR_ERR_ARG, "missing output / workspace pointer%s");
    } else if (!a->out_color || !a->out_depth || !a->out_alpha || !a->image || !a->bg || !a->alloc)
        return fail(GSR_ERR_ARG, "missing output / workspace pointer%s");
    const int N = a->N, W = a->W, H = a->H;
    BatchDev bt;
    rc = batch_dev(a->batch, N, H, bt);
    if (rc) return rc;
    const int NB = bt.B;
    const int tiles_x = (W + kTile - 1) / kTile, tiles_y = (H + kTile - 1) / kTile, T = tiles_x * tiles_y * NB;
    if (a->sh_origin && (!a->shs || NB > 1 || a->prepared))
        return fail(GSR_ERR_ARG, "sh_origin needs shs and is not served with a batch of B > 1 or a prepared buffer%s");
    out->num_rendered = 0; out->binning = nullptr; out->binning_bytes = 0; out->binning_capacity = 0;
    out->forward_flags = pack_fwd_flags(opt.ckpt_first) | (ro ? GSR_FWD_FLAG_RENDER_ONLY : 0);
    uint64_t R = 0;
    BlendBalance bb = {};
    ListCut lc = {};
    uint64_t lc_capacity = 0;
    Splat* splat = static_cast<Splat*>(a->geom);
    float* img = static_cast<float*>(a->image);
    uint8_t* img_base = static_cast<uint8_t*>(a->image);
    size_t balance_off = image_balance_offset(W, H, NB), staged_off = image_staged_offset(W, H, NB);
    uint32_t* staged = img_base ? reinterpret_cast<uint32_t*>(img_base + staged_off) : nullptr;
    auto ro_workspace = [&]() -> int {
        if (!ro) return GSR_OK;
        if (!img_base) {
            staged_off -= balance_off; balance_off = 0;
            img_base = static_cast<uint8_t*>(a->alloc(staged_off + align256((size_t)T * 16), GSR_ALLOC_SCRATCH, a->alloc_user));
            if (!img_base) return fail(GSR_ERR_ALLOC, "image workspace allocation failed%s");
            img = reinterpret_cast<float*>(img_base);
            staged = reinterpret_cast<uint32_t*>(img_base + staged_off);
        }
        if (!splat && N > 0) {
            splat = static_cast<Splat*>(a->alloc(gsr_geom_bytes(N), GSR_ALLOC_SCRATCH, a->alloc_user));
            if (!splat) return fail(GSR_ERR_ALLOC, "splat record allocation failed%s");
        }
        return GSR_OK;
    };
    const FwdScratch L = fwd_scratch_layout(N);
    uint8_t* fs = nullptr;
    uint32_t* sorted_gid = nullptr;
    int bits = 1;
    while ((1 << bits) < T) bits++;
    const int tile_passes = (bits + 7) / 8;
    const bool wide_keys = T > 65536;
    const int nb = (N + kEmitThreads - 1) / kEmitThreads;

    BinLayout B = bin_layout(0, W, H, NB);
    BinScratch S = bin_scratch_layout(0);
    uint8_t *bin = nullptr, *bs = nullptr;
    DirectBin db = {};
    DirectBinScratch dbs = {};
    const bool direct = opt.direct_binning && !wide_keys && direct_bin_geometry(N, T, db, dbs);
    bool tsort = false;
    uint2* ranges = nullptr;
    uint32_t* list = nullptr;
    uint2 *pairs = nullptr, *pairs_alt = nullptr;
    auto alloc_binning = [&](uint64_t capacity) -> int {
        B = bin_layout((int64_t)capacity, W, H, NB);
        bin = static_cast<uint8_t*>(ro ? a->alloc(B.ckpt, GSR_ALLOC_SCRATCH, a->alloc_user) : a->alloc(B.bytes, GSR_ALLOC_BINNING, a->alloc_user));
        if (!bin) return fail(GSR_ERR_ALLOC, "binning allocation failed%s");
        ranges = reinterpret_cast<uint2*>(bin + B.ranges);
        list = reinterpret_cast<uint32_t*>(bin + B.list);
        bs = nullptr;
        if (capacity > 0 && tsort) {
            const size_t pb = align256((size_t)capacity * sizeof(uint2));
            uint8_t* pm = static_cast<uint8_t*>(a->alloc(2 * pb, GSR_ALLOC_SCRATCH, a->alloc_user));
            if (!pm) return fail(GSR_ERR_ALLOC, "pair buffer allocation failed%s");
            pairs = reinterpret_cast<uint2*>(pm);
            pairs_alt = reinterpret_cast<uint2*>(pm + pb);
        }
        if (capacity == 0 || direct) return GSR_OK;
        S = bin_scratch_layout((int64_t)capacity, wide_keys ? 4 : 2);
        bs = static_cast<uint8_t*>(a->alloc(S.bytes, GSR_ALLOC_SCRATCH, a->alloc_user));
        if (!bs) return fail(GSR_ERR_ALLOC, "binning scratch allocation failed%s");
        return GSR_OK;
    };
    const TileRec* ts_rec = nullptr;
    const uint32_t* ts_dkey = nullptr;
    auto launch_binning_t = [&](auto key_tag, uint64_t capacity, const unsigned long long* n_dev, bool prezeroed) -> int {
        using KeyT = decltype(key_tag);
        if (!prezeroed) GSR_HIP(hipMemsetAsync(ranges, 0, (size_t)T * sizeof(uint2), st));
        if (capacity == 0) return GSR_OK;
        KeyT* tkey = reinterpret_cast<KeyT*>(bs + S.tile);
        KeyT* tkey_alt = reinterpret_cast<KeyT*>(bs + S.tile_alt);
        uint32_t* gid_alt2 = reinterpret_cast<uint32_t*>(bs + S.gid_alt);
        uint32_t* block_sums = reinterpret_cast<uint32_t*>(fs + L.block_sums);
        uint32_t* v0 = (tile_passes & 1) ? gid_alt2 : list;
        uint32_t* v1 = (tile_passes & 1) ? list : gid_alt2;
        const bool emit_hist = prezeroed && opt.emit_hist;
        EmitHist eh = {};
        if (emit_hist) {
            eh.ghist = reinterpret_cast<uint32_t*>(bs + S.sort);
            eh.status = onesweep_status(bs + S.sort);
            eh.status_words = onesweep_status_words<KeyT>((uint32_t)capacity, bits);
            eh.bits = bits;
            eh.n_dev = n_dev;
        }
        {
            ProfScope ps(P_EMIT, st);
            hipLaunchKernelGGL(k_emit<KeyT>, dim3(nb), dim3(kEmitThreads), 0, st, N, W, H, tiles_x, tiles_y, sorted_gid, splat,
                               tsort ? ts_rec : reinterpret_cast<const TileRec*>(fs + L.srec), block_sums, tkey, v0,
                               (uint32_t)capacity, eh);
        }
        int in_alt = 0;
        {
            ProfScope ps(P_SORT_TILE, st);
            GSR_HIP(onesweep_sort_pairs<KeyT>(tkey, v0, tkey_alt, v1, (uint32_t)capacity, 0, bits, bs + S.sort, &in_alt, st, n_dev, prezeroed,
                                              emit_hist));
        }
        const KeyT* skey = in_alt ? tkey_alt : tkey;
        {
            ProfScope ps(P_RANGES, st);
            constexpr uint32_t kpb = 256u * (16u / (uint32_t)sizeof(KeyT));
            hipLaunchKernelGGL(k_tile_ranges<KeyT>, dim3(((uint32_t)capacity + kpb - 1) / kpb), dim3(256), 0, st, (uint32_t)capacity, skey, ranges, n_dev);
        }
        if (tsort) {
            ProfScope ps(P_SORT_DEPTH, st);
            hipLaunchKernelGGL(k_tile_sort_wave<true>, dim3(T), dim3(64), 0, st, ranges, pairs, list, T, ts_dkey);
            hipLaunchKernelGGL((k_tile_sort<1024, true>), dim3(std::min(T, 512)), dim3(1024), 0, st, ranges, pairs, pairs_alt, list, T, ts_dkey);
        }
        return GSR_OK;
    };
    auto launch_binning = [&](uint64_t capacity, const unsigned long long* n_dev, bool prezeroed) -> int {
        if (direct) {
            if (capacity == 0) { GSR_HIP(hipMemsetAsync(ranges, 0, (size_t)T * sizeof(uint2), st)); return GSR_OK; }
            const int per = (db.NC + 7) / 8, grid = std::max(8 * per, (T + 63) / 64);
            if (tsort) {
                {
                    ProfScope ps(P_EMIT, st);
                    hipLaunchKernelGGL((k_chunk_scatter<true>), dim3(grid), dim3(64), (size_t)12 * db.Tp + 4 * kDbPairs, st, db, W, H, tiles_x, tiles_y,
                                       (const uint32_t*)nullptr, ts_rec, splat, list, ranges, (uint32_t)std::min<uint64_t>(capacity, 0xffffffffull), ts_dkey, pairs);
                }
                ProfScope ps2(P_SORT_TILE, st);
                hipLaunchKernelGGL(k_tile_sort_wave<false>, dim3(T), dim3(64), 0, st, ranges, pairs, list, T, (const uint32_t*)nullptr);
                hipLaunchKernelGGL(k_tile_sort<1024>, dim3(std::min(T, 512)), dim3(1024), 0, st, ranges, pairs, pairs_alt, list, T);
                return GSR_OK;
            }
            ProfScope ps(P_EMIT, st);
            if (lc.key) {
                lc_capacity = capacity;
                hipLaunchKernelGGL((k_chunk_scatter<false, 1>), dim3(grid), dim3(64), (size_t)12 * db.Tp + 4 * kDbPairs, st, db, W, H,
                                   tiles_x, tiles_y, sorted_gid, reinterpret_cast<const TileRec*>(fs + L.srec), splat, list, ranges,
                                   (uint32_t)std::min<uint64_t>(capacity, 0xffffffffull), (const uint32_t*)nullptr, (uint2*)nullptr, lc);
            } else
                hipLaunchKernelGGL(k_chunk_scatter<false>, dim3(grid), dim3(64), (size_t)12 * db.Tp + 4 * kDbPairs, st, db, W, H, tiles_x, tiles_y, sorted_gid,
                                   reinterpret_cast<const TileRec*>(fs + L.srec), splat, list, ranges, (uint32_t)std::min<uint64_t>(capacity, 0xffffffffull));
            return GSR_OK;
        }
        return wide_keys ? launch_binning_t(uint32_t{}, capacity, n_dev, prezeroed) : launch_binning_t(uint16_t{}, capacity, n_dev, prezeroed);
    };
    auto launch_blend = [&](bool prezeroed) -> int {
        if (!prezeroed) GSR_HIP(hipMemsetAsync(staged, 0, (size_t)T * 16, st));
        float* ckpt = ro ? nullptr : reinterpret_cast<float*>(bin + B.ckpt);
        auto k7 = ro ? (a->out_depth ? k_blend_fwd_render<true> : k_blend_fwd_render<false>) : k_blend_fwd_w6;
        const int prof = g_profile.load(std::memory_order_relaxed);
        if (prof && (prof != 3 || g_profile_tick.fetch_add(1u) % 3u == 0u)) {
            hipEvent_t ea = nullptr, eb = nullptr;
            if (hipEventCreate(&ea) != hipSuccess || hipEventCreate(&eb) != hipSuccess) return fail(GSR_ERR_HIP, "hipEventCreate failed%s");
            hipExtLaunchKernelGGL(k7, dim3(8 * 4 * slots_per_xcd(T, tiles_x)), dim3(64), 0, st, ea, eb, 0, W, H, tiles_x, T, ranges, list,
                                  splat, a->bg, a->out_color, a->out_depth, a->out_alpha, img, staged, ckpt, opt.ckpt_first, tiles_y, bb, a->out_color_clamped,
                                  lc, lc.key ? 1 : 0);
            std::lock_guard<std::mutex> lk(g_prof_mutex);
            g_prof_events[P_BLEND_FWD].push_back({ea, eb});
        } else {
            ProfScope ps(prof == 3 ? P_COUNT : P_BLEND_FWD, st);
            hipLaunchKernelGGL(k7, dim3(8 * 4 * slots_per_xcd(T, tiles_x)), dim3(64), 0, st, W, H, tiles_x, T, ranges, list, splat, a->bg,
                               a->out_color, a->out_depth, a->out_alpha, img, staged, ckpt, opt.ckpt_first, tiles_y, bb, a->out_color_clamped,
                               lc, lc.key ? 1 : 0);
        }
        if (lc.key && lc_capacity > 0) {
            ProfScope ps(P_CUT_REPAIR, st);
            const int per = (db.NC + 7) / 8, grid = std::max(8 * per, (T + 63) / 64);
            hipLaunchKernelGGL((k_chunk_scatter<false, 2>), dim3(grid), dim3(64), (size_t)12 * db.Tp + 4 * kDbPairs, st, db, W, H,
                               tiles_x, tiles_y, sorted_gid, reinterpret_cast<const TileRec*>(fs + L.srec), splat, list, ranges,
                               (uint32_t)std::min<uint64_t>(lc_capacity, 0xffffffffull), (const uint32_t*)nullptr, (uint2*)nullptr, lc);
            hipLaunchKernelGGL(k_blend_fwd_w6, dim3(8 * 4 * slots_per_xcd(T, tiles_x)), dim3(64), 0, st, W, H, tiles_x, T, ranges, list, splat, a->bg,
                               a->out_color, a->out_depth, a->out_alpha, img, staged, ckpt, opt.ckpt_first, tiles_y, bb, a->out_color_clamped, lc, 2);
        }
        GSR_HIP(hipGetLastError());
        return GSR_OK;
    };

    if (N == 0) {
        rc = ro_workspace();
        if (rc) return rc;
        rc = alloc_binning(0);
        if (rc) return rc;
        rc = launch_binning(0, nullptr, false);
        if (rc) return rc;
        rc = launch_blend(false);
        if (rc) return rc;
        if (!ro) { out->binning = bin; out->binning_bytes = B.bytes; }
        return GSR_OK;
    }

    if (!a->means3D || !a->opacities || (!ro && !a->geom) || !a->radii || !a->viewmatrix || !a->projmatrix)
        return fail(GSR_ERR_ARG, "missing input pointer%s");
    if ((a->shs == nullptr) == (a->colors_precomp == nullptr)) return fail(GSR_ERR_ARG, "provide exactly one of shs / colors_precomp%s");
    if ((a->cov3D_precomp == nullptr) == (a->scales == nullptr || a->rotations == nullptr))
        return fail(GSR_ERR_ARG, "provide exactly one of (scales, rotations) / cov3D_precomp%s");
    if (a->shs && (!a->campos || a->M < (a->D + 1) * (a->D + 1))) return fail(GSR_ERR_ARG, "shs needs campos and M >= (D+1)^2%s");
    rc = ro_workspace();
    if (rc) return rc;

    int dev_id = 0;
    GSR_HIP(hipGetDevice(&dev_id));
    const auto hint_key = std::make_tuple(dev_id, W, H * NB, n_bucket(N));
    uint64_t hint = 0;
    {
        std::lock_guard<std::mutex> lk(g_state_mutex);
        if (g_hint_override > 0) { hint = (uint64_t)g_hint_override; g_hint_override = -1; }
        else { auto it = g_hints.find(hint_key); if (it != g_hints.end()) hint = it->second; }
    }
    const bool speculative = opt.speculative_binning && hint > 0;
    const uint64_t cap = speculative ? hint : 0;
    {
        const int ts_mode = opt.tile_sort;
        const uint64_t avg = (hint > 0 ? hint : (uint64_t)N * 4u) / (uint64_t)T;
        const bool auto_ok = ts_mode == 1 && avg <= (uint64_t)opt.tile_sort_max_avg && (direct || N / std::max(1, NB) <= opt.tile_sort_emit_max_n);
        tsort = (ts_mode == 2 || auto_ok) && (direct ? NB == 1 : true);
    }

    fs = static_cast<uint8_t*>(a->alloc(align256(L.bytes) + (direct ? dbs.bytes : 0), GSR_ALLOC_SCRATCH, a->alloc_user));
    if (!fs) return fail(GSR_ERR_ALLOC, "scratch allocation failed%s");
    if (speculative) {
        rc = alloc_binning(cap);
        if (rc) return rc;
    }
    uint32_t* dkey = reinterpret_cast<uint32_t*>(fs + L.dkey);
    uint32_t* gid = reinterpret_cast<uint32_t*>(fs + L.gid);
    uint32_t* dkey_alt = reinterpret_cast<uint32_t*>(fs + L.dkey_alt);
    uint32_t* gid_alt = reinterpret_cast<uint32_t*>(fs + L.gid_alt);
    TileRec* ntiles = reinterpret_cast<TileRec*>(fs + L.ntiles);
    uint32_t* block_sums = reinterpret_cast<uint32_t*>(fs + L.block_sums);
    unsigned long long* total = reinterpret_cast<unsigned long long*>(fs + L.total);
    CamParams cp = {a->viewmatrix, a->projmatrix, a->campos, a->tanfovx, a->tanfovy, a->scale_modifier, W, H, a->D, a->M, a->points_transform, bt};
    const int grid = (N + kPreThreads - 1) / kPreThreads;
    const RetireDev rt = {retired_at, (int)retire_step};
    uint32_t* zero_words = reinterpret_cast<uint32_t*>(fs + L.sort);
    const int zero_count = (int)kOnesweepHeadWordsMax;
    uint8_t* depth_scratch = fs + L.sort;
    bool depth_hist_done = false;
    const bool early_r = opt.early_r && speculative;
    uint2* early_parts = early_r ? reinterpret_cast<uint2*>(a->prepared ? static_cast<uint8_t*>(a->prepared) + prep_layout(N).early : fs + L.early) : nullptr;
    const uint32_t early_window = (N > opt.prep_hist_max_n || (opt.small_sort9 && !a->prepared && N >= opt.small_sort9)) ? (1u << 27) - 1u : 0xffffffffu;
    if (a->prepared) {
        if (a->prepared != a->geom) return fail(GSR_ERR_ARG, "prepared: geom must be the prepared buffer itself%s");
        const PrepLayout PL = prep_layout(N);
        uint8_t* pb = static_cast<uint8_t*>(a->prepared);
        dkey = reinterpret_cast<uint32_t*>(pb + PL.dkey);
        gid = reinterpret_cast<uint32_t*>(pb + PL.gid);
        ntiles = reinterpret_cast<TileRec*>(pb + PL.rec);
        ProfScope ps(P_PRE_FWD, st);
        depth_scratch = pb + PL.sort;
        depth_hist_done = opt.prep_counts_digits(N);
        if (a->radii != reinterpret_cast<const int32_t*>(pb + PL.radii))
            hipLaunchKernelGGL(k_prepared_begin, dim3((N + 255) / 256), dim3(256), 0, st, N, reinterpret_cast<const int32_t*>(pb + PL.radii),
                               a->radii, (uint32_t*)nullptr, 0);
    } else {
#define GSR_PRE_(DEG, RAW, SHO)                                                                                                     \
    hipLaunchKernelGGL((k_preprocess<DEG, RAW, SHO>), dim3(grid), dim3(kPreThreads), 0, st, cp, N, a->means3D, a->scales,           \
                       a->rotations, a->cov3D_precomp, a->opacities, a->shs, a->shs_rest, a->colors_precomp, splat, a->radii, dkey, gid, \
                       ntiles, zero_words, zero_count, 0, DepthHist{}, early_parts, early_window, a->visible, a->sh_origin, rt)
#define GSR_PRE(DEG) do { if (a->raw_params) GSR_PRE_(DEG, true, false); else GSR_PRE_(DEG, false, false); } while (0)
#define GSR_PRE_SHO(DEG) do { if (a->raw_params) GSR_PRE_(DEG, true, true); else GSR_PRE_(DEG, false, true); } while (0)
    {
        ProfScope ps(P_PRE_FWD, st);
        if (a->sh_origin) {
            switch (a->D) {
                case 0: GSR_PRE(0); break;
                case 1: GSR_PRE_SHO(1); break;
                case 2: GSR_PRE_SHO(2); break;
                default: GSR_PRE_SHO(3); break;
            }
        } else {
        switch (a->shs ? a->D : 0) {
            case 0: GSR_PRE(0); break;
            case 1: GSR_PRE(1); break;
            case 2: GSR_PRE(2); break;
            default: GSR_PRE(3); break;
        }
        }
    }
#undef GSR_PRE_SHO
#undef GSR_PRE
#undef GSR_PRE_
    }
    int in_alt = 0;
    bool wide_depth = opt.depth_sort9 && !depth_hist_done && (N > opt.prep_hist_max_n || (opt.small_sort9 && N >= opt.small_sort9));
    if (wide_depth) {
        std::lock_guard<std::mutex> lk(g_state_mutex);
        auto it = g_full_depth_sort.find(hint_key);
        if (it != g_full_depth_sort.end() && it->second) wide_depth = false;
    }
    const unsigned int* window_overflow = wide_depth ? onesweep_overflow_word(depth_scratch) : nullptr;
    if (tsort) wide_depth = false;
    const unsigned int* window_overflow_ = tsort ? nullptr : window_overflow;
    PinLease pin(acquire_pin_slot(dev_id));
    if (!pin.s) return fail(GSR_ERR_HIP, "pinned read-back slot allocation failed%s");
    {
        unsigned long long got = 0, want = 0;
        if (late_check(pin.s, true, &got, &want)) {
            char msg[200];
            snprintf(msg, sizeof msg, "a PREVIOUS forward's binning was invalid: early instance count %llu, its scan counted %llu (or a sort look-back gave up)%%s", want, got);
            return fail(GSR_ERR_HIP, msg);
        }
    }
    OsRider rider = {};
    if (early_r) { rider.parts = early_parts; rider.nparts = (uint32_t)grid; rider.host = pin.s->dev; rider.seq = ++pin.s->seq; }
    ts_rec = ntiles; ts_dkey = dkey;
    if (!tsort) {
        ProfScope ps(P_SORT_DEPTH, st);
        GSR_HIP(onesweep_sort_pairs<uint32_t>(dkey, gid, dkey_alt, gid_alt, (uint32_t)N, 0, wide_depth ? 27 : 32, depth_scratch, &in_alt, st, nullptr, true,
                                              depth_hist_done, wide_depth ? 9 : 8, kDepthKeyBias, early_r ? &rider : nullptr));
    }
    sorted_gid = tsort ? nullptr : (in_alt ? gid_alt : gid);
    auto launch_counts = [&](const BlendBalance& bal, const ZeroJobs& zjobs, const unsigned int* wo, unsigned long long seq, bool publish = true) {
        TileRec* srec = reinterpret_cast<TileRec*>(fs + L.srec);
        unsigned long long* const host_slot = publish ? pin.s->dev : nullptr;
        unsigned long long* const late_slot = publish ? nullptr : pin.s->dev + 4;
        if (direct) {
            hipLaunchKernelGGL(k_chunk_counts, dim3(db.NC + (bal.hdr ? 8 : 0)), dim3(kEmitThreads), (size_t)2 * db.Tp, st, db, W, H,
                               tiles_x, tiles_y, sorted_gid, ntiles, splat, tsort ? (TileRec*)nullptr : srec, bal,
                               (tsort && early_r && !publish) ? rider : OsRider{}, lc);
            hipLaunchKernelGGL(k_chunk_scan1, dim3((db.Tp + 255) / 256, db.G), dim3(256), 0, st, db);
            hipLaunchKernelGGL(k_chunk_scan2, dim3((db.Tp + 255) / 256), dim3(256), lc.key ? (size_t)db.NC * 4 : 0, st, db, total, zjobs, host_slot, seq, wo,
                               late_slot, lc);
        } else {
            hipLaunchKernelGGL(k_tile_counts, dim3(nb + (bal.hdr ? 8 : 0)), dim3(kEmitThreads), 0, st, N, sorted_gid, ntiles, block_sums,
                               tsort ? (TileRec*)nullptr : srec, bal, nb, (tsort && early_r && !publish) ? rider : OsRider{});
            hipLaunchKernelGGL(k_block_scan, dim3(1), dim3(1024), 0, st, block_sums, nb, total, zjobs, host_slot, seq, wo, late_slot);
        }
    };
    {
        ProfScope ps(P_SCAN, st);
        ZeroJobs zj = {};
        if (speculative) {
            zj.p[0] = ranges; zj.words[0] = (uint32_t)((size_t)T * sizeof(uint2) / 4);
            zj.p[1] = staged; zj.words[1] = (uint32_t)T * 4u;
            if (bs) { zj.p[2] = bs + S.sort; zj.words[2] = kOnesweepHeadWords; }
        }
        {
            const int nslots4 = 4 * slots_per_xcd(T, tiles_x), items = 8 * nslots4;
            if (opt.blend_balance && NB == 1 && items <= 65535 && nslots4 <= 20 * kEmitThreads && a->viewmatrix) {
                const size_t hdr_bytes = align256(sizeof(ViewCostHdr));
                const size_t vc_cut = align256(hdr_bytes + (size_t)kVcEntries * items * sizeof(uint16_t));
                const size_t vc_own = vc_cut + align256((size_t)kVcEntries * T * sizeof(uint32_t));
                const size_t vc_bytes = vc_own + align256((size_t)kVcEntries * sizeof(uint32_t));
                uint8_t* mem = nullptr;
                {
                    std::lock_guard<std::mutex> lk(g_state_mutex);
                    for (auto& c : g_view_costs)
                        if (c.dev == dev_id && c.W == W && c.H == H && c.items == items) mem = c.mem;
                    if (!mem && g_view_costs.size() < 64) {
                        if (hipMalloc((void**)&mem, vc_bytes) == hipSuccess) {
                            if (hipMemset(mem, 0, vc_bytes) == hipSuccess) {
                                g_view_costs.push_back({dev_id, W, H, items, mem, vc_bytes});
                            } else {
                                (void)hipGetLastError();
                                (void)hipFree(mem);
                                mem = nullptr;
                            }
                        } else {
                            (void)hipGetLastError();
                            mem = nullptr;
                        }
                    }
                }
                if (mem) {
                    uint8_t* ib = img_base + balance_off;
                    bb.hdr = reinterpret_cast<ViewCostHdr*>(mem);
                    bb.cost = reinterpret_cast<uint16_t*>(mem + hdr_bytes);
                    bb.cur = reinterpret_cast<uint32_t*>(ib);
                    bb.perm = reinterpret_cast<uint16_t*>(ib + 256);
                    bb.vm = a->viewmatrix; bb.pt = a->points_transform; bb.view_id = (long long)a->view_id;
                    bb.tol = 1e-6f * (float)opt.view_pose_tol_e6;
                    bb.items = items; bb.nslots4 = nslots4; bb.W = W; bb.H = H;
                    if (!ro && direct && !tsort && db.NC <= 16000 && T == db.T && (opt.list_cut == 2 || (opt.list_cut == 1 && N >= opt.list_cut_min_n))) {
                        uint8_t* dm = fs + align256(L.bytes);
                        lc.key = reinterpret_cast<uint32_t*>(mem + vc_cut);
                        lc.owner_n = reinterpret_cast<uint32_t*>(mem + vc_own);
                        lc.stats = &bb.hdr->pad[2];
                        lc.cur = bb.cur;
                        lc.chunk = reinterpret_cast<uint16_t*>(dm + dbs.cut_chunk);
                        lc.tend = reinterpret_cast<uint32_t*>(dm + dbs.cut_tend);
                        lc.flag = reinterpret_cast<uint32_t*>(dm + dbs.cut_flag);
                        lc.ctl = reinterpret_cast<uint32_t*>(dm + dbs.cut_ctl);
                        lc.bkey = reinterpret_cast<uint32_t*>(dm + dbs.cut_bkey);
                        lc.hist = reinterpret_cast<uint32_t*>(dm + dbs.cut_hist);
                        lc.skey = in_alt ? dkey_alt : dkey;
                        lc.tbase = reinterpret_cast<uint32_t*>(dm + dbs.tbase);
                        lc.margin = 1e-3f * (float)opt.list_cut_margin_e3;
                        lc.dmax = std::max(0, opt.list_cut_deep);
                    }
                }
            }
        }
        if (direct) {
            uint8_t* dm = fs + align256(L.bytes);
            db.M = reinterpret_cast<uint16_t*>(dm + dbs.M); db.GT = reinterpret_cast<uint32_t*>(dm + dbs.GT); db.tbase = reinterpret_cast<uint32_t*>(dm + dbs.tbase);
            db.bsum = reinterpret_cast<uint32_t*>(dm + dbs.bsum);
            zj.p[0] = nullptr; zj.words[0] = 0u;
            zj.p[2] = nullptr; zj.words[2] = 0u;
        }
        if (early_r) launch_counts(bb, zj, window_overflow_, rider.seq, false);
        else launch_counts(bb, zj, window_overflow_, ++pin.s->seq);
    }
    GSR_HIP(hipGetLastError());

    if (speculative) {
        rc = launch_binning(cap, total, true);
        if (rc) return rc;
        rc = launch_blend(true);
        if (rc) return rc;
        {
            const auto w0 = std::chrono::steady_clock::now();
            volatile unsigned long long* hp = pin.s->host;
            const unsigned long long want = pin.s->seq;
            bool seen = false;
            if (opt.poll_iters > 0) {
                const auto limit = w0 + std::chrono::nanoseconds((long long)opt.poll_iters * 50);
                while (!(seen = (hp[1] == want))) {
                    for (int it = 0; it < 64 && !(seen = (hp[1] == want)); it++) cpu_relax();
                    if (seen || std::chrono::steady_clock::now() > limit) break;
                }
            }
            if (!seen) GSR_HIP(hipStreamSynchronize(st));
            std::atomic_thread_fence(std::memory_order_acquire);
            g_fwd_wait_ns += std::chrono::duration_cast<std::chrono::nanoseconds>(std::chrono::steady_clock::now() - w0).count();
        }
        g_spec_forwards++;
    } else {
        const auto w0 = std::chrono::steady_clock::now();
        GSR_HIP(hipStreamSynchronize(st));
        g_fwd_wait_ns += std::chrono::duration_cast<std::chrono::nanoseconds>(std::chrono::steady_clock::now() - w0).count();
        g_exact_forwards++;
    }
    R = *static_cast<volatile unsigned long long*>(pin.s->host);
    {
        static std::map<int, unsigned long long> seen_giveups;
        const unsigned long long gv = static_cast<volatile unsigned long long*>(pin.s->host)[2];
        bool fresh;
        long long late_bias = 0;
        {
            std::lock_guard<std::mutex> lk(g_state_mutex);
            unsigned long long& seen = seen_giveups[dev_id];
            fresh = gv != seen;
            seen = gv;
            if (early_r && !fresh) { late_bias = g_late_bias; g_late_bias = 0; }
        }
        if (fresh)
            return fail(GSR_ERR_HIP, "a radix-sort look-back gave up (status words overwritten?): the binning of this or the previous forward is invalid%s");
        if (early_r) {
            pin.s->pending = true; pin.s->pending_seq = rider.seq; pin.s->pending_R = R + (unsigned long long)late_bias; pin.s->pending_giveups = gv;
        }
    }
    bool resorted = false;
    if (wide_depth && static_cast<volatile unsigned long long*>(pin.s->host)[3] != 0ull) {
        { std::lock_guard<std::mutex> lk(g_state_mutex); g_full_depth_sort[hint_key] = true; }
        g_depth_window_resorts++;
        uint32_t *k0 = in_alt ? dkey_alt : dkey, *v0 = in_alt ? gid_alt : gid, *k1 = in_alt ? dkey : dkey_alt, *v1 = in_alt ? gid : gid_alt;
        int alt2 = 0;
        GSR_HIP(onesweep_sort_pairs<uint32_t>(k0, v0, k1, v1, (uint32_t)N, 0, 32, depth_scratch, &alt2, st));
        sorted_gid = alt2 ? v1 : v0;
        launch_counts(BlendBalance{}, ZeroJobs{}, nullptr, ++pin.s->seq);
        GSR_HIP(hipStreamSynchronize(st));
        std::atomic_thread_fence(std::memory_order_acquire);
        R = *static_cast<volatile unsigned long long*>(pin.s->host);
        resorted = true;
    }
    if (R > 0xfffffff0ull) return fail(GSR_ERR_RANGE, "more than 2^32 instances%s");
    if (!speculative || R > cap || resorted) {
        if (speculative && !resorted) g_spec_overflows++;
        rc = alloc_binning(R);
        if (rc) return rc;
        rc = launch_binning(R, nullptr, false);
        if (rc) return rc;
        rc = launch_blend(false);
        if (rc) return rc;
    }
    {
        std::lock_guard<std::mutex> lk(g_state_mutex);
        uint64_t& h = g_hints[hint_key];
        h = std::max<uint64_t>(std::max<uint64_t>(R + R / 4, h - h / 32), 1u << 16);
        if (g_hints.size() > 4096) g_hints.clear();
    }
    out->num_rendered = (int64_t)R;
    if (ro) return GSR_OK;
    out->binning = bin;
    out->binning_bytes = B.bytes;
    out->binning_capacity = (int64_t)((speculative && R <= cap && !resorted) ? cap : R);
    return GSR_OK;
}

int gsr_forward(const GsrForwardArgs* a, GsrForwardOut* out, void* stream_) { return forward_impl(a, nullptr, 0, out, stream_); }
int gsr_forward_retire(const GsrForwardArgs* a, const int32_t* retired_at, int64_t retire_step, GsrForwardOut* out, void* stream_)
{
    return forward_impl(a, retired_at, retire_step, out, stream_);
}

static int blend_bwd_resident(int has_da)
{
    static int cached[2] = {0, 0};
    if (cached[has_da]) return cached[has_da];
    int dev = 0, cus = 256, per_cu = 0;
    hipDeviceProp_t prop;
    if (hipGetDevice(&dev) == hipSuccess && hipGetDeviceProperties(&prop, dev) == hipSuccess) cus = prop.multiProcessorCount;
    const hipError_t e = has_da ? hipOccupancyMaxActiveBlocksPerMultiprocessor(&per_cu, k_blend_bwd2<true>, 128, 0)
                                : hipOccupancyMaxActiveBlocksPerMultiprocessor(&per_cu, k_blend_bwd2<false>, 128, 0);
    if (e != hipSuccess || per_cu < 1) per_cu = 12;
    return cached[has_da] = per_cu * cus;
}

int gsr_backward(const GsrBackwardArgs* a, void* stream_)
{
    CallTimer call_timer(g_bwd_calls, g_bwd_ns);
    hipStream_t st = (hipStream_t)stream_;
    if (!a) return fail(GSR_ERR_ARG, "null args%s");
    const Options opt = options_snapshot();
    if (a->forward_flags & GSR_FWD_FLAG_RENDER_ONLY)
        return fail(GSR_ERR_ARG, "gsr_backward: forward_flags come from a render-only forward, which keeps nothing a backward could read%s");
    int rc = check_common(a->N, a->M, a->D, a->W, a->H);
    if (rc) return rc;
    const int N = a->N, W = a->W, H = a->H;
    BatchDev bt;
    rc = batch_dev(a->batch, N, H, bt);
    if (rc) return rc;
    const int NB = bt.B;
    if (a->sh_origin && (!a->shs || NB > 1 || a->next_view))
        return fail(GSR_ERR_ARG, "sh_origin needs shs and is not served with a batch of B > 1 or a next_view%s");
    const bool want_cam = a->d_viewmatrix || a->d_projmatrix || a->d_campos || a->d_points_transform;
    const bool want_other_pg = a->d_opacities || a->d_colors_precomp || a->d_shs || a->d_shs_rest || a->d_scales || a->d_rotations || a->d_cov3D_precomp;
    const bool frozen = !a->fused_adam && !a->d_means3D && !want_other_pg && want_cam;
    if (a->retired_at) {
        if (frozen) return fail(GSR_ERR_ARG, "retired_at: a retire table is not served on the frozen backward (no update to gate)%s");
        if (!a->fused_adam) return fail(GSR_ERR_ARG, "retired_at: a retire table needs fused_adam (the update it gates runs in this call)%s");
        if (a->retire_step < 1 || a->retire_step > 0x7fffffffll) return fail(GSR_ERR_ARG, "retired_at: retire_step must be the 1-based step of the call%s");
        if (a->densify_stats) return fail(GSR_ERR_ARG, "retired_at: a retire table is not served with densify_stats%s");
        for (int q = 0; q < 6; q++)
            if (a->fused_adam->param_out[q] || a->fused_adam->exp_avg_out[q] || a->fused_adam->exp_avg_sq_out[q])
                return fail(GSR_ERR_ARG, "retired_at: a retire table is not served with the deferred step (GsrFusedAdam::param_out)%s");
    }
    if (!a->fused_adam && !a->d_means3D && a->N > 0) {
        if (want_other_pg)
            return fail(GSR_ERR_ARG, "d_means3D is NULL but another per-Gaussian gradient pointer is set: they come together, or none of them (frozen call)%s");
        if (!want_cam)
            return fail(GSR_ERR_ARG, "no gradient output: every per-Gaussian gradient pointer is NULL and so are d_viewmatrix, d_projmatrix, d_campos and "
                                     "d_points_transform%s");
        if (a->next_view || a->prepared_out)
            return fail(GSR_ERR_ARG, "a frozen call (no per-Gaussian gradient pointer) cannot prepare a next view: next_view / prepared_out need fused_adam%s");
        if (a->densify_stats)
            return fail(GSR_ERR_ARG, "a frozen call (no per-Gaussian gradient pointer) cannot accumulate densify_stats: they are fed by the per-Gaussian "
                                     "gradients it leaves out%s");
    }
    {
        int dev_id = 0;
        (void)hipGetDevice(&dev_id);
        unsigned long long got = 0, want = 0;
        bool bad = false;
        {
            std::lock_guard<std::mutex> lk(g_state_mutex);
            auto it = g_pin_slots.find(dev_id);
            if (it != g_pin_slots.end())
                for (PinSlot* s : it->second)
                    if (!s->busy && late_check(s, false, &got, &want)) { bad = true; break; }
        }
        if (bad) {
            char msg[200];
            snprintf(msg, sizeof msg, "a forward's binning was invalid: early instance count %llu, its scan counted %llu (or a sort look-back gave up)%%s", want, got);
            return fail(GSR_ERR_HIP, msg);
        }
    }
    int f_ckpt = opt.ckpt_first;
    if (a->forward_flags & 1) {
        f_ckpt = (int)((a->forward_flags >> 6) & 127);
        if (!flags_from_forward(a->forward_flags) || f_ckpt < 1) return fail(GSR_ERR_ARG, "forward_flags do not come from gsr_forward%s");
    }
    if (N == 0) {
        if (a->d_viewmatrix) GSR_HIP(hipMemsetAsync(a->d_viewmatrix, 0, 64 * NB, st));
        if (a->d_projmatrix) GSR_HIP(hipMemsetAsync(a->d_projmatrix, 0, 64 * NB, st));
        if (a->d_campos) GSR_HIP(hipMemsetAsync(a->d_campos, 0, 12 * NB, st));
        if (a->d_points_transform) GSR_HIP(hipMemsetAsync(a->d_points_transform, 0, 48 * NB, st));
        return GSR_OK;
    }
    if (!a->geom || !a->image || !a->binning || !a->scratch || (!a->d_means2D && !frozen))
        return fail(GSR_ERR_ARG, "missing workspace / gradient pointer%s");
    const int tiles_x = (W + kTile - 1) / kTile, tiles_y = (H + kTile - 1) / kTile, T = tiles_x * tiles_y * NB;
    const Splat* splat = static_cast<const Splat*>(a->geom);
    BinLayout B = bin_layout(a->binning_capacity > 0 ? a->binning_capacity : a->num_rendered, W, H, NB);
    const uint8_t* bin = static_cast<const uint8_t*>(a->binning);
    const uint2* ranges = reinterpret_cast<const uint2*>(bin + B.ranges);
    const uint32_t* list = reinterpret_cast<const uint32_t*>(bin + B.list);
    double* gg = static_cast<double*>(a->scratch);
    uint32_t* prep_head = (a->next_view && a->prepared_out) ? reinterpret_cast<uint32_t*>(static_cast<uint8_t*>(a->prepared_out) + prep_layout(N).sort) : nullptr;
    bool prep_head_cleared = false;
    const bool blend_items = a->num_rendered > 0;
    BwdItemHdr* item_hdr = nullptr;
    const uint2* items = nullptr;
    int bwd_grid = 0;
    {
        const uint32_t* staged4 = reinterpret_cast<const uint32_t*>(static_cast<const uint8_t*>(a->image) + image_staged_offset(W, H, NB));
        const int tpad = 8 * slots_per_xcd(T, tiles_x);
        const int want_split = opt.bwd_split ? opt.bwd_split : 16;
        const int split_ok = want_split > 1 ? 1 : 0;
        const size_t n4 = (size_t)N * kGG * sizeof(double) / sizeof(float4);
        int fill_blocks = (int)std::min<size_t>(4096, (n4 + 255) / 256);
        if (blend_items) {
            uint8_t* binw = const_cast<uint8_t*>(bin);
            item_hdr = reinterpret_cast<BwdItemHdr*>(binw + B.items);
            items = reinterpret_cast<const uint2*>(binw + B.items + kItemHdrBytes);
            const int64_t bound = (a->num_rendered >> 7) + T;
            const int resident = blend_bwd_resident((a->grad_depth || a->grad_alpha) ? 1 : 0);
            bwd_grid = (int)std::max<int64_t>(8, (std::min<int64_t>(resident, bound) + 7) / 8 * 8);
        }
        const uint32_t list_cap = (uint32_t)bwd_list_cap(a->binning_capacity > 0 ? a->binning_capacity : a->num_rendered, (size_t)T);
        hipLaunchKernelGGL(k_bwd_prologue, dim3(fill_blocks + (blend_items ? 8 : 0)), dim3(256), 0, st, reinterpret_cast<float4*>(gg), n4,
                           staged4, T, tiles_x, tpad, f_ckpt, split_ok, item_hdr, const_cast<uint2*>(items), list_cap,
                           (uint32_t)(bwd_grid / 8), blend_items ? prep_head : nullptr, (int)kOnesweepHeadWordsMax);
        prep_head_cleared = blend_items && prep_head != nullptr;
    }
    if (a->num_rendered > 0) {
        const float* img = static_cast<const float*>(a->image);
        ProfScope ps(P_BLEND_BWD, st);
        const float* ckpt = reinterpret_cast<const float*>(bin + B.ckpt);
        float* det_part = nullptr;
        uint8_t* det_mem = nullptr;
        const uint32_t Rn = (uint32_t)a->num_rendered;
        size_t o_part = 0, o_k0 = 0, o_k1 = 0, o_v0 = 0, o_v1 = 0, o_sort = 0, det_bytes = 0;
        if (opt.deterministic_backward) {
            size_t o = 0;
            o_part = o; o += align256((size_t)Rn * kDetStride * 4);
            o_k0 = o; o += align256((size_t)Rn * 4); o_k1 = o; o += align256((size_t)Rn * 4);
            o_v0 = o; o += align256((size_t)Rn * 4); o_v1 = o; o += align256((size_t)Rn * 4);
            o_sort = o; o += onesweep_scratch_bytes(Rn);
            det_bytes = o;
            GSR_HIP(hipMallocAsync((void**)&det_mem, det_bytes, st));
            det_part = reinterpret_cast<float*>(det_mem + o_part);
            GSR_HIP(hipMemsetAsync(det_part, 0, (size_t)Rn * kDetStride * 4, st));
        }
        BlendBwdArgs ba = {W, H, tiles_x, tiles_y, T, f_ckpt, ranges, list, splat, a->bg, img, a->grad_color, a->grad_depth,
                           a->grad_alpha, gg, ckpt, det_part, item_hdr, items};
        if (a->grad_depth || a->grad_alpha) hipLaunchKernelGGL(k_blend_bwd2<true>, dim3(bwd_grid), dim3(128), 0, st, ba);
        else hipLaunchKernelGGL(k_blend_bwd2<false>, dim3(bwd_grid), dim3(128), 0, st, ba);
        if (opt.deterministic_backward) {
            uint32_t* k0 = reinterpret_cast<uint32_t*>(det_mem + o_k0); uint32_t* k1 = reinterpret_cast<uint32_t*>(det_mem + o_k1);
            uint32_t* v0 = reinterpret_cast<uint32_t*>(det_mem + o_v0); uint32_t* v1 = reinterpret_cast<uint32_t*>(det_mem + o_v1);
            hipLaunchKernelGGL(k_det_iota, dim3((Rn + 255) / 256), dim3(256), 0, st, Rn, v0, list, k0, (uint32_t)N);
            int nbits = 1;
            while ((1ll << nbits) < (long long)N) nbits++;
            int in_alt = 0;
            GSR_HIP(onesweep_sort_pairs<uint32_t>(k0, v0, k1, v1, Rn, 0, ((nbits + 7) / 8) * 8, det_mem + o_sort, &in_alt, st));
            hipLaunchKernelGGL(k_det_reduce, dim3((Rn + 255) / 256), dim3(256), 0, st, Rn, in_alt ? k1 : k0, in_alt ? v1 : v0, det_part, gg);
            GSR_HIP(hipFreeAsync(det_mem, st));
        }
    }
    CamParams cp = {a->viewmatrix, a->projmatrix, a->campos, a->tanfovx, a->tanfovy, a->scale_modifier, W, H, a->D, a->M, a->points_transform, bt};
    const int grid = (N + kPreThreads - 1) / kPreThreads;
    const RetireDev rt = {a->retired_at, (int)a->retire_step};
    const RetireDev rt_next = {a->retired_at, (int)a->retire_step + 1};
    float* cam_partial = reinterpret_cast<float*>(static_cast<uint8_t*>(a->scratch) + align256((size_t)N * kGG * sizeof(double)));
    AdamDev ad = {};
    const GsrFusedAdam* fa = a->fused_adam;
    if (fa) {
        if (!a->raw_params || !a->shs || !a->shs_rest || a->cov3D_precomp || a->colors_precomp || !a->scales || !a->rotations || !a->opacities ||
            a->M < 1 || fa->step <= 0)
            return fail(GSR_ERR_ARG, "fused_adam needs raw_params with shs (f_dc) + shs_rest, scales, rotations and opacities%s");
        const bool skip_rest = !fa->exp_avg[2] && !fa->exp_avg_sq[2];
        if (skip_rest && (a->D != 0 || (a->next_view && a->next_view->D != 0)))
            return fail(GSR_ERR_ARG, "fused_adam: the f_rest group may be skipped only at sh_degree 0 (this render and the prepared one)%s");
        for (int q = 0; q < 6; q++) {
            ad.inv_bc2s[q] = 1.f;
            if (q == 2 && skip_rest) { ad.m[q] = nullptr; ad.v[q] = nullptr; ad.step_size[q] = 0.f; continue; }
            if (!fa->exp_avg[q] || !fa->exp_avg_sq[q]) return fail(GSR_ERR_ARG, "fused_adam: missing moment buffer%s");
            ad.m[q] = fa->exp_avg[q]; ad.v[q] = fa->exp_avg_sq[q];
            const int64_t tq = fa->step - (int64_t)fa->step_lag[q];
            if (fa->step_lag[q] < 0 || tq < 1) return fail(GSR_ERR_ARG, "fused_adam: step_lag out of range%s");
            ad.step_size[q] = fa->lr[q] / (float)(1.0 - pow((double)fa->beta1, (double)tq));
            ad.inv_bc2s[q] = 1.f / (float)sqrt(1.0 - pow((double)fa->beta2, (double)tq));
            const float* pin[6] = {a->means3D, a->shs, a->shs_rest, a->opacities, a->scales, a->rotations};
            if (fa->param_out[q] || fa->exp_avg_out[q] || fa->exp_avg_sq_out[q]) {
                if (!fa->param_out[q] || !fa->exp_avg_out[q] || !fa->exp_avg_sq_out[q]) return fail(GSR_ERR_ARG, "fused_adam: a group's three output buffers come together%s");
                if (a->next_view) return fail(GSR_ERR_ARG, "fused_adam: deferred application (param_out) cannot prepare a next view%s");
                ad.dp[q] = (long long)((const char*)fa->param_out[q] - (const char*)pin[q]);
                ad.dm[q] = (long long)((const char*)fa->exp_avg_out[q] - (const char*)fa->exp_avg[q]);
                ad.dv[q] = (long long)((const char*)fa->exp_avg_sq_out[q] - (const char*)fa->exp_avg_sq[q]);
            }
        }
        ad.b1 = fa->beta1; ad.b2 = fa->beta2; ad.eps = fa->eps;
    } else if (!frozen && (!a->d_means3D || !a->d_opacities))
        return fail(GSR_ERR_ARG, "missing workspace / gradient pointer%s");
    DensDev ds = {};
    if (a->densify_stats) {
        const GsrDensifyStats* q = a->densify_stats;
        if (!q->radii || !q->xyz_gradient_accum || !q->denom || !q->max_radii2D) return fail(GSR_ERR_ARG, "densify_stats: four pointers expected%s");
        ds.radii = q->radii; ds.grad_accum = q->xyz_gradient_accum; ds.denom = q->denom; ds.max_radii = q->max_radii2D;
    }
    PrepOut po = {};
    const GsrNextView* nv = a->next_view;
    if (nv) {
        if (!fa || !gsr_prepare_supported(a->M, a->D, a->raw_params) || nv->D < a->D || nv->D > a->D + 1 || nv->D > 3 || !a->prepared_out ||
            !nv->viewmatrix || !nv->projmatrix || !nv->campos || nv->W <= 0 || nv->H <= 0 ||
            ((((uintptr_t)a->shs | (uintptr_t)a->shs_rest) & 15) != 0))
            return fail(GSR_ERR_ARG, "next_view needs fused_adam, raw_params, M = 16, a next degree equal to this render's or one above, "
                                     "16-byte aligned SH tensors and a prepared_out buffer%s");
        const PrepLayout PL = prep_layout(N);
        uint8_t* pb = static_cast<uint8_t*>(a->prepared_out);
        BatchDev nbt = bt;
        if (NB > 1 && (long long)NB * ((nv->H + kTile - 1) / kTile) > 4095) return fail(GSR_ERR_RANGE, "batch: more than 4095 tile rows in the next view%s");
        po.cp = {nv->viewmatrix, nv->projmatrix, nv->campos, nv->tanfovx, nv->tanfovy, nv->scale_modifier, nv->W, nv->H, nv->D, a->M, nv->points_transform, nbt};
        po.splat = reinterpret_cast<Splat*>(pb + PL.splat);
        po.radii = reinterpret_cast<int32_t*>(pb + PL.radii);
        po.dkey = reinterpret_cast<uint32_t*>(pb + PL.dkey);
        po.gid = reinterpret_cast<uint32_t*>(pb + PL.gid);
        po.rec = reinterpret_cast<TileRec*>(pb + PL.rec);
        po.early_parts = reinterpret_cast<uint2*>(pb + PL.early);
        po.early_window = N > opt.prep_hist_max_n ? (1u << 27) - 1u : 0xffffffffu;
        if (!prep_head_cleared) GSR_HIP(hipMemsetAsync(prep_head, 0, kOnesweepHeadWordsMax * sizeof(uint32_t), st));
        if (opt.prep_counts_digits(N)) {
            po.dh.ghist = prep_head;
            po.dh.status = onesweep_status(pb + PL.sort);
            po.dh.status_words = onesweep_status_words<uint32_t>((uint32_t)N, 32);
            const int tail_blocks = ((N - (grid - 1) * kPreThreads) % 4 == 0) ? grid : grid - 1;
            po.dh.clear_threads = (uint32_t)tail_blocks * kPreThreads;
        }
    }
#define GSR_PREB_S(DEG, RAW, CAM, ADAM, PREP, SHO) GSR_PREB_SF(DEG, RAW, CAM, ADAM, PREP, SHO, false)
#define GSR_PREB_SF(DEG, RAW, CAM, ADAM, PREP, SHO, FROZEN)                                                                                 \
    hipLaunchKernelGGL((k_preprocess_bwd<DEG, RAW, CAM, ADAM, PREP, SHO, FROZEN>), dim3(grid), dim3(kPreThreads), 0, st, cp, N, a->means3D, \
                       a->scales, a->rotations, a->cov3D_precomp, a->shs, a->shs_rest, a->opacities, ad, splat, gg, a->d_means3D,           \
                       a->d_means2D, a->d_opacities, a->d_colors_precomp, a->d_shs, a->d_shs_rest, a->d_scales, a->d_rotations,             \
                       a->d_cov3D_precomp, cam_partial, po, ds, a->sh_origin, rt)
#define GSR_PREB_(DEG, RAW, CAM, ADAM, PREP) GSR_PREB_S(DEG, RAW, CAM, ADAM, PREP, false)
#define GSR_PREB_SO(DEG, SHO)                                                                                                               \
    do {                                                                                                                                    \
        if (fa) { if (want_cam) GSR_PREB_S(DEG, true, true, true, -1, SHO); else GSR_PREB_S(DEG, true, false, true, -1, SHO); }             \
        else if (a->raw_params) { if (want_cam) GSR_PREB_S(DEG, true, true, false, -1, SHO); else GSR_PREB_S(DEG, true, false, false, -1, SHO); } \
        else { if (want_cam) GSR_PREB_S(DEG, false, true, false, -1, SHO); else GSR_PREB_S(DEG, false, false, false, -1, SHO); }           \
    } while (0)
#define GSR_PREB(DEG) GSR_PREB_SO(DEG, false)
#define GSR_PREB_FROZEN(DEG) do { if (a->raw_params) GSR_PREB_SF(DEG, true, true, false, -1, false, true); else GSR_PREB_SF(DEG, false, true, false, -1, false, true); } while (0)
#define GSR_PREB_NEXT(DEG, NDEG) do { if (want_cam) GSR_PREB_(DEG, true, true, true, NDEG); else GSR_PREB_(DEG, true, false, true, NDEG); } while (0)
#define GSR_PRE_TAIL(NDEG)                                                                                                               \
    hipLaunchKernelGGL((k_preprocess<NDEG, true>), dim3(1), dim3(kPreThreads), 0, st, po.cp, N, a->means3D, a->scales, a->rotations,       \
                       (const float*)nullptr, a->opacities, a->shs, a->shs_rest, (const float*)nullptr, po.splat, po.radii, po.dkey,     \
                       po.gid, po.rec, (uint32_t*)nullptr, 0, grid - 1, po.dh, po.early_parts, po.early_window, (uint8_t*)nullptr,            \
                       (const float*)nullptr, rt_next)
    {
        ProfScope ps(P_PRE_BWD, st);
        if (nv) {
            switch (a->D * 4 + nv->D) {
                case 0: GSR_PREB_NEXT(0, 0); break;
                case 1: GSR_PREB_NEXT(0, 1); break;
                case 5: GSR_PREB_NEXT(1, 1); break;
                case 6: GSR_PREB_NEXT(1, 2); break;
                case 10: GSR_PREB_NEXT(2, 2); break;
                case 11: GSR_PREB_NEXT(2, 3); break;
                default: GSR_PREB_NEXT(3, 3); break;
            }
            const int nlast = N - (grid - 1) * kPreThreads;
            const bool last_lin = (nlast % 4) == 0;
            if (!last_lin) {
                switch (nv->D) {
                    case 0: GSR_PRE_TAIL(0); break;
                    case 1: GSR_PRE_TAIL(1); break;
                    case 2: GSR_PRE_TAIL(2); break;
                    default: GSR_PRE_TAIL(3); break;
                }
            }
        } else if (frozen) {
            g_frozen_bwd_calls.fetch_add(1, std::memory_order_relaxed);
            switch ((a->shs && !a->sh_origin) ? a->D : 0) {
                case 0: GSR_PREB_FROZEN(0); break;
                case 1: GSR_PREB_FROZEN(1); break;
                case 2: GSR_PREB_FROZEN(2); break;
                default: GSR_PREB_FROZEN(3); break;
            }
        } else if (a->sh_origin) {
        switch (a->D) {
            case 0: GSR_PREB(0); break;
            case 1: GSR_PREB_SO(1, true); break;
            case 2: GSR_PREB_SO(2, true); break;
            default: GSR_PREB_SO(3, true); break;
        }
        } else {
        switch (a->shs ? a->D : 0) {
            case 0: GSR_PREB(0); break;
            case 1: GSR_PREB(1); break;
            case 2: GSR_PREB(2); break;
            default: GSR_PREB(3); break;
        }
        }
    }
#undef GSR_PRE_TAIL
#undef GSR_PREB_NEXT
#undef GSR_PREB_FROZEN
#undef GSR_PREB
#undef GSR_PREB_SO
#undef GSR_PREB_
#undef GSR_PREB_SF
#undef GSR_PREB_S
    if (want_cam)
        hipLaunchKernelGGL(k_cam_reduce, dim3(kCamVals, NB), dim3(256), 0, st, cam_partial, grid, a->d_viewmatrix, a->d_projmatrix, a->d_campos,
                           a->d_points_transform, bt);
    GSR_HIP(hipGetLastError());
    return GSR_OK;
}

size_t gsr_importance_scratch_bytes(int32_t N) { return align256((size_t)(N > 0 ? N : 1) * kImpStride * sizeof(float)); }

int gsr_importance_accumulate(const GsrForwardArgs* a, const GsrForwardOut* out, float* acc, void* scratch, void* stream_)
{
    hipStream_t st = (hipStream_t)stream_;
    if (!a || !out) return fail(GSR_ERR_ARG, "null args%s");
    if (out->forward_flags & GSR_FWD_FLAG_RENDER_ONLY)
        return fail(GSR_ERR_ARG, "importance: forward_flags come from a render-only forward, which keeps no image state or lists for the pass%s");
    int rc = check_common(a->N, a->M, a->D, a->W, a->H);
    if (rc) return rc;
    if (a->colors_precomp || !a->shs) return fail(GSR_ERR_ARG, "importance: the model must carry SH coefficients (colors_precomp has none)%s");
    if (a->batch && a->batch->B > 1) return fail(GSR_ERR_ARG, "importance: not served with a batch of B > 1%s");
    if (a->M < (a->D + 1) * (a->D + 1) || !a->campos) return fail(GSR_ERR_ARG, "shs needs campos and M >= (D+1)^2%s");
    const int N = a->N, W = a->W, H = a->H;
    if (N == 0) return GSR_OK;
    if (!acc || !scratch || !a->geom || !a->image || !a->out_color || !a->means3D) return fail(GSR_ERR_ARG, "missing workspace / accumulator pointer%s");
    if (out->num_rendered <= 0 || !out->binning) return GSR_OK;
    if ((out->forward_flags & 1) && !flags_from_forward(out->forward_flags)) return fail(GSR_ERR_ARG, "forward_flags do not come from gsr_forward%s");
    const int tiles_x = (W + kTile - 1) / kTile, tiles_y = (H + kTile - 1) / kTile, T = tiles_x * tiles_y;
    const Splat* splat = static_cast<const Splat*>(a->geom);
    const BinLayout B = bin_layout(out->binning_capacity > 0 ? out->binning_capacity : out->num_rendered, W, H, 1);
    const uint8_t* bin = static_cast<const uint8_t*>(out->binning);
    const uint2* ranges = reinterpret_cast<const uint2*>(bin + B.ranges);
    const uint32_t* list = reinterpret_cast<const uint32_t*>(bin + B.list);
    float* img = static_cast<float*>(a->image);
    uint32_t* staged = reinterpret_cast<uint32_t*>(static_cast<uint8_t*>(a->image) + image_staged_offset(W, H, 1));
    float* S = static_cast<float*>(scratch);
    GSR_HIP(hipMemsetAsync(S, 0, (size_t)N * kImpStride * sizeof(float), st));
    {
        ProfScope ps(P_IMP_BLEND, st);
        hipLaunchKernelGGL(k_blend_importance, dim3(8 * 4 * slots_per_xcd(T, tiles_x)), dim3(64), 0, st, W, H, tiles_x, T, ranges, list, splat,
                           img, staged, tiles_y, (const float*)a->out_color, S);
    }
    {
        ProfScope ps(P_IMP_FINISH, st);
        hipLaunchKernelGGL(k_importance_finish, dim3((N + 15) / 16), dim3(256), 0, st, N, a->M, a->D, a->means3D, a->points_transform, a->campos,
                           a->sh_origin, splat, (const float*)S, acc);
    }
    GSR_HIP(hipGetLastError());
    return GSR_OK;
}

int gsr_debug_view_cache_stats(int32_t W, int32_t H, int64_t out[4])
{
    int dev_id = 0;
    if (hipGetDevice(&dev_id) != hipSuccess) return fail(GSR_ERR_HIP, "hipGetDevice failed%s");
    out[0] = out[1] = out[2] = out[3] = 0;
    std::vector<uint8_t*> mems;
    {
        std::lock_guard<std::mutex> lk(g_state_mutex);
        for (auto& c : g_view_costs) if (c.dev == dev_id && c.W == W && c.H == H) mems.push_back(c.mem);
    }
    for (uint8_t* m : mems) {
        ViewCostHdr h;
        if (hipDeviceSynchronize() != hipSuccess || hipMemcpy(&h, m, sizeof(h), hipMemcpyDeviceToHost) != hipSuccess)
            return fail(GSR_ERR_HIP, "view cache read-back failed%s");
        out[0] += h.pad[0]; out[1] += h.pad[1]; out[3] += 1;
        for (int i = 0; i < kVcEntries; i++) out[2] += h.key[i] != 0ull;
    }
    return GSR_OK;
}

int gsr_debug_list_cut_stats(int32_t W, int32_t H, int64_t out[5])
{
    int dev_id = 0;
    if (hipGetDevice(&dev_id) != hipSuccess) return fail(GSR_ERR_HIP, "hipGetDevice failed%s");
    out[0] = out[1] = out[2] = out[3] = out[4] = 0;
    std::vector<uint8_t*> mems;
    {
        std::lock_guard<std::mutex> lk(g_state_mutex);
        for (auto& c : g_view_costs) if (c.dev == dev_id && c.W == W && c.H == H) mems.push_back(c.mem);
    }
    for (uint8_t* m : mems) {
        ViewCostHdr h;
        if (hipDeviceSynchronize() != hipSuccess || hipMemcpy(&h, m, sizeof(h), hipMemcpyDeviceToHost) != hipSuccess)
            return fail(GSR_ERR_HIP, "view cache read-back failed%s");
        for (int q = 0; q < 5; q++) out[q] += h.pad[2 + q];
    }
    return GSR_OK;
}

int gsr_debug_direct_binning_geometry(int32_t N, int32_t T, int64_t out[7])
{
    if (!out) return GSR_ERR_ARG;
    DirectBin db = {};
    DirectBinScratch ds = {};
    const bool ok = direct_bin_geometry(N, T, db, ds);
    out[0] = ok ? 1 : 0; out[1] = db.S; out[2] = db.NC; out[3] = db.G; out[4] = db.Cg; out[5] = db.Tp; out[6] = ok ? (int64_t)ds.bytes : 0;
    return GSR_OK;
}

int gsr_debug_read_binning(const void* binning, int64_t binning_capacity, int64_t num_rendered, int32_t W, int32_t H,
                            uint32_t* ranges_out, uint32_t* list_out, void* stream_)
{
    if (!binning || W <= 0 || H <= 0 || num_rendered < 0) return fail(GSR_ERR_ARG, "bad debug_read_binning args%s");
    const BinLayout B = bin_layout(binning_capacity > 0 ? binning_capacity : num_rendered, W, H);
    const size_t T = (size_t)((W + kTile - 1) / kTile) * ((H + kTile - 1) / kTile);
    const uint8_t* bin = static_cast<const uint8_t*>(binning);
    hipStream_t st = (hipStream_t)stream_;
    if (ranges_out) GSR_HIP(hipMemcpyAsync(ranges_out, bin + B.ranges, T * sizeof(uint2), hipMemcpyDeviceToDevice, st));
    if (list_out && num_rendered > 0)
        GSR_HIP(hipMemcpyAsync(list_out, bin + B.list, (size_t)num_rendered * 4, hipMemcpyDeviceToDevice, st));
    return GSR_OK;
}

int64_t gsr_get_counter(const char* name)
{
    if (!name) return -1;
    if (!strcmp(name, "spec_overflows")) return g_spec_overflows.load();
    if (!strcmp(name, "late_checks")) return g_late_checks.load();
    if (!strcmp(name, "late_mismatches")) return g_late_mismatches.load();
    if (!strcmp(name, "depth_window_resorts")) return g_depth_window_resorts.load();
    if (!strcmp(name, "blend_bwd_resident")) return blend_bwd_resident(0);
    if (!strcmp(name, "spec_forwards")) return g_spec_forwards.load();
    if (!strcmp(name, "exact_forwards")) return g_exact_forwards.load();
    if (!strcmp(name, "forward_calls")) return g_fwd_calls.load();
    if (!strcmp(name, "forward_ns")) return g_fwd_ns.load();
    if (!strcmp(name, "forward_wait_ns")) return g_fwd_wait_ns.load();
    if (!strcmp(name, "backward_calls")) return g_bwd_calls.load();
    if (!strcmp(name, "backward_ns")) return g_bwd_ns.load();
    if (!strcmp(name, "frozen_backward_calls")) return g_frozen_bwd_calls.load();
    if (!strcmp(name, "spec_callers")) { std::lock_guard<std::mutex> lk(g_state_mutex); return (int64_t)g_hints.size(); }
    return -1;
}

int gsr_mark_visible(int32_t N, const float* means3D, const float* viewmatrix, const float* projmatrix, uint8_t* present, void* stream_)
{
    (void)projmatrix;
    if (N < 0 || (N > 0 && (!means3D || !viewmatrix || !present))) return fail(GSR_ERR_ARG, "bad mark_visible args%s");
    if (N == 0) return GSR_OK;
    hipLaunchKernelGGL(k_mark_visible, dim3((N + 255) / 256), dim3(256), 0, (hipStream_t)stream_, N, means3D, viewmatrix, present);
    GSR_HIP(hipGetLastError());
    return GSR_OK;
}

int gsr_sort_pairs_u32(uint32_t* keys, uint32_t* vals, uint32_t* keys_alt, uint32_t* vals_alt, uint32_t n, int begin_bit, int end_bit,
                       void* scratch, size_t scratch_bytes, int* result_in_alt, void* stream)
{
    return sort_pairs_entry<uint32_t>(keys, vals, keys_alt, vals_alt, n, begin_bit, end_bit, scratch, scratch_bytes, result_in_alt, stream);
}

int gsr_sort_pairs_u16(uint16_t* keys, uint32_t* vals, uint16_t* keys_alt, uint32_t* vals_alt, uint32_t n, int begin_bit, int end_bit,
                       void* scratch, size_t scratch_bytes, int* result_in_alt, void* stream)
{
    return sort_pairs_entry<uint16_t>(keys, vals, keys_alt, vals_alt, n, begin_bit, end_bit, scratch, scratch_bytes, result_in_alt, stream);
}

}
```

### 3dgs_hierarchical_training_amd/csrc/options.h

```cpp
#pragma once
#include <limits.h>
#include <string.h>

#include <mutex>

namespace gsr {

struct Options {
    int prep_hist_max_n = 262144;
    bool prep_counts_digits(int N) const { return N <= prep_hist_max_n; }
    int small_sort9 = 1;
    int poll_iters = 400000;
    int emit_hist = 1;
    int speculative_binning = 1;
    int deterministic_backward = 0;
    int bwd_split = 0;
    int ckpt_first = 1;
    int depth_sort9 = 1;
    int tile_sort = 1;
    int tile_sort_emit_max_n = 400000;
    int tile_sort_max_avg = 700;
    int direct_binning = 1;
    int view_pose_tol_e6 = 2000;
    int list_cut = 1;
    int list_cut_min_n = 2000000;
    int list_cut_margin_e3 = 50;
    int list_cut_deep = 8;
    int early_r = 1;
    int blend_balance = 1;
};

enum class Outside {
    Refuse,
    StoreNonZero,
    StoreDefault,
    ClampToLo,
};
struct OptionRow { const char* name; int Options::*member; int lo, hi; Outside outside; };

inline constexpr OptionRow kOptionRows[] = {
    {"bwd_split", &Options::bwd_split, 0, 64, Outside::Refuse},
    {"ckpt_first", &Options::ckpt_first, 1, 64, Outside::Refuse},
    {"tile_sort", &Options::tile_sort, 0, 2, Outside::Refuse},
    {"tile_sort_max_avg", &Options::tile_sort_max_avg, 0, INT_MAX, Outside::Refuse},
    {"view_pose_tol_e6", &Options::view_pose_tol_e6, 0, INT_MAX, Outside::Refuse},
    {"small_sort9", &Options::small_sort9, 0, INT_MAX, Outside::Refuse},
    {"prep_hist_max_n", &Options::prep_hist_max_n, INT_MIN, INT_MAX, Outside::Refuse},
    {"list_cut", &Options::list_cut, 0, 2, Outside::StoreDefault},
    {"list_cut_min_n", &Options::list_cut_min_n, 0, INT_MAX, Outside::StoreDefault},
    {"list_cut_margin_e3", &Options::list_cut_margin_e3, 0, INT_MAX, Outside::StoreDefault},
    {"list_cut_deep", &Options::list_cut_deep, 0, INT_MAX, Outside::StoreDefault},
    {"poll_iters", &Options::poll_iters, 0, INT_MAX, Outside::ClampToLo},
    {"blend_balance", &Options::blend_balance, 0, 1, Outside::StoreNonZero},
    {"early_r", &Options::early_r, 0, 1, Outside::StoreNonZero},
    {"depth_sort9", &Options::depth_sort9, 0, 1, Outside::StoreNonZero},
    {"direct_binning", &Options::direct_binning, 0, 1, Outside::StoreNonZero},
    {"speculative_binning", &Options::speculative_binning, 0, 1, Outside::StoreNonZero},
    {"emit_hist", &Options::emit_hist, 0, 1, Outside::StoreNonZero},
    {"deterministic_backward", &Options::deterministic_backward, 0, 1, Outside::StoreNonZero},
};

struct RetiredRow { const char* name; bool any; int a, b; };
inline constexpr RetiredRow kRetiredRows[] = {
    {"blend_fwd_ppt", false, 0, 7},
    {"tile_map", false, 2, 2},
    {"sort_algo", false, 2, 2},
    {"blend_bwd_ppt", false, 0, 2},
    {"ab_variants", true, 0, 0},
};

inline std::mutex g_options_mutex;
inline Options g_options;

enum class SetResult { Stored, Refused, Unknown };

inline SetResult options_set(const char* name, int value)
{
    for (const OptionRow& r : kOptionRows) {
        if (strcmp(name, r.name)) continue;
        if (value < r.lo || value > r.hi) {
            switch (r.outside) {
                case Outside::Refuse: return SetResult::Refused;
                case Outside::StoreNonZero: value = value != 0; break;
                case Outside::StoreDefault: value = Options{}.*r.member; break;
                case Outside::ClampToLo: value = r.lo; break;
            }
        }
        std::lock_guard<std::mutex> lk(g_options_mutex);
        g_options.*r.member = value;
        return SetResult::Stored;
    }
    for (const RetiredRow& r : kRetiredRows)
        if (!strcmp(name, r.name)) return (r.any || value == r.a || value == r.b) ? SetResult::Stored : SetResult::Refused;
    return SetResult::Unknown;
}

inline Options options_snapshot()
{
    std::lock_guard<std::mutex> lk(g_options_mutex);
    return g_options;
}

}
```

Baseline: 1311.

## Add per-tile depth cut cache to prune binned pairs across repeated views

Adds a per-view tile cut cache that records a per-tile depth threshold from a previous render of the same pose. On later renders it drops Gaussian-tile pairs deeper than that threshold (plus a margin) during counting and scattering, with a repair path for tiles that saturate. It also refactors the large-segment tile sort into a reusable block routine. This aims to cut binning, sort and blend work on saturated tiles, at the cost of extra kernels, cache state and a dependence on view reuse and a correct repair.

```diff
diff --git a/3dgs_hierarchical_training_amd/csrc/gsr_kernels.hip b/3dgs_hierarchical_training_amd/csrc/gsr_kernels.hip
--- a/3dgs_hierarchical_training_amd/csrc/gsr_kernels.hip
+++ b/3dgs_hierarchical_training_amd/csrc/gsr_kernels.hip
@@ -1037,10 +1037,107 @@
 #endif
 }
 
+struct TileCutHdr {
+    unsigned long long key[kVcEntries];
+    uint32_t stamp[kVcEntries];
+    uint32_t owner_n[kVcEntries];
+    uint32_t clock, pad[31];
+    float pose[kVcEntries][kVcPoseFloats];
+    unsigned long long stats[8];
+};
+struct TileCut {
+    const uint16_t* thr;
+    const uint32_t* dkey;
+    TileRec* frec;
+};
+struct TileCutCall {
+    uint16_t* thr;
+    uint32_t* zero;
+    uint32_t* mark;
+    uint32_t* flag;
+    uint32_t* ctl;
+    uint32_t* cnt;
+};
+
+__global__ __launch_bounds__(256) void k_tile_cut_begin(TileCutHdr* hdr, uint32_t* rows, TileCutCall tc, const float* __restrict__ vm,
+                                                        const float* __restrict__ pt, long long view_id, float tol, int N, int T, int Tp,
+                                                        float margin, int apply)
+{
+    __shared__ unsigned long long s_best;
+    __shared__ float s_pose[kVcPoseFloats];
+    __shared__ int s_e, s_use;
+    const int tid = threadIdx.x;
+    if (tid == 0) s_best = ~0ull;
+    if (tid < 16) s_pose[tid] = vm[tid];
+    else if (tid < kVcPoseFloats) s_pose[tid] = pt ? pt[tid - 16] : (((tid - 16) % 5 == 0) ? 1.f : 0.f);
+    __syncthreads();
+    const unsigned long long want = view_id ? view_id_key(view_id) : 2ull;
+    if (tid < kVcEntries && hdr->key[tid] == want) {
+        float d = 0.f;
+        if (!view_id) {
+            const float* p = hdr->pose[tid];
+            bool near = true;
+            for (int i = 0; i < kVcPoseFloats; i++) { const float df = fabsf(p[i] - s_pose[i]); near = near && (df <= tol); d = fmaxf(d, df); }
+            if (!near) d = 3.0e38f;
+        }
+        if (d <= tol) atomicMin(&s_best, ((unsigned long long)__float_as_uint(d) << 32) | (unsigned)tid);
+    }
+    __syncthreads();
+    if (tid == 0) {
+        const int e = s_best == ~0ull ? -1 : (int)(s_best & 0xffffffffull);
+        int rec = e;
+        const uint32_t now = hdr->clock + 1u;
+        if (rec < 0) {
+            uint32_t best = 0xffffffffu;
+            for (int i = 0; i < kVcEntries; i++) if (hdr->stamp[i] < best) { best = hdr->stamp[i]; rec = i; }
+            hdr->key[rec] = want;
+        }
+        for (int i = 0; i < kVcPoseFloats; i++) hdr->pose[rec][i] = s_pose[i];
+        hdr->stamp[rec] = now; hdr->clock = now;
+        const bool use = apply && e >= 0 && hdr->owner_n[rec] == (uint32_t)N;
+        hdr->owner_n[rec] = (uint32_t)N;
+        if (use) hdr->stats[0] += 1ull;
+        s_e = rec; s_use = use ? 1 : 0;
+        tc.ctl[2] = 0u; tc.ctl[4] = (uint32_t)rec; tc.ctl[5] = use ? 1u : 0u; tc.ctl[7] = 0u;
+        tc.mark[0] = 0u;
+    }
+    __syncthreads();
+    uint32_t* row = rows + (size_t)s_e * T;
+    const bool use = s_use != 0;
+    for (int t = tid; t < Tp; t += 256) {
+        uint32_t th = 0xffffu;
+        if (t < T) {
+            const uint32_t k = row[t];
+            if (use && k != kCutOpenKey && k != 0u) {
+                const float d = __uint_as_float(k);
+                th = min(__float_as_uint(fmaf(d, margin, d)) >> 16, 0xffffu);
+            }
+            row[t] = 0u;
+        }
+        tc.thr[t] = (uint16_t)th;
+        tc.zero[t] = 0u; tc.flag[t] = 0u; tc.cnt[t] = 0u;
+        tc.mark[t + 1] = th != 0xffffu ? 1u : 0u;
+    }
+}
+
+__device__ __forceinline__ uint32_t tile_cut_mask(const TileRec& r, const uint32_t k16, const uint16_t* thr, const int tiles_x)
+{
+    const uint32_t ww = (r.rect >> 24) & 63u, rx0 = r.rect & 0xfffu, ry0 = (r.rect >> 12) & 0xfffu;
+    const uint32_t rcp = (65536u + ww - 1u) / (ww ? ww : 1u);
+    const uint32_t base = ry0 * (uint32_t)tiles_x + rx0, skip = (uint32_t)tiles_x - ww;
+    uint32_t keep = 0u;
+    for (uint32_t m = r.mask; m != 0u; m &= m - 1u) {
+        const uint32_t p = (uint32_t)__builtin_ctz(m);
+        if (k16 <= (uint32_t)thr[base + p + ((p * rcp) >> 16) * skip]) keep |= 1u << p;
+    }
+    return keep;
+}
+
+template <bool FILT = false>
 __global__ __launch_bounds__(kEmitThreads) void k_chunk_counts(DirectBin db, int W, int H, int tiles_x, int tiles_y,
                                                                const uint32_t* __restrict__ sorted_gid, const TileRec* __restrict__ tilerec,
                                                                const Splat* __restrict__ splat, TileRec* __restrict__ sorted_rec, BlendBalance bb,
-                                                               OsRider rider = OsRider{}, ListCut cut = ListCut{})
+                                                               OsRider rider = OsRider{}, ListCut cut = ListCut{}, TileCut tc = TileCut{})
 {
     const int nbuild = bb.hdr ? 8 : 0, c = (int)blockIdx.x - nbuild;
     if (c < 0) { balance_build(bb, (int)blockIdx.x); return; }
@@ -1056,28 +1153,43 @@
     extern __shared__ uint32_t s_h[];
     const int tid = threadIdx.x, lane = tid & 63, wave = tid >> 6;
     for (int i = tid; i < db.Tp / 2; i += kEmitThreads) s_h[i] = 0u;
+    uint16_t* const s_thr = reinterpret_cast<uint16_t*>(s_h + db.Tp / 2);
+    if (FILT)
+        for (int i = tid; i < db.Tp / 2; i += kEmitThreads) reinterpret_cast<uint32_t*>(s_thr)[i] = reinterpret_cast<const uint32_t*>(tc.thr)[i];
     __syncthreads();
     const int j0 = c * db.S + wave * 64, j1 = min(db.N, c * db.S + db.S);
     constexpr int kStride = 64 * kDbCountWaves;
     auto load_gid = [&](int j) -> uint32_t { return j < j1 ? (sorted_gid ? sorted_gid[j] : (uint32_t)j) : 0xffffffffu; };
     auto load_rec = [&](uint32_t g) -> TileRec { TileRec r; r.mask = 0u; r.rect = 1u << 24; if (g != 0xffffffffu) r = tilerec[g]; return r; };
+    auto load_k16 = [&](uint32_t g) -> uint32_t { return (FILT && g != 0xffffffffu) ? tc.dkey[g] >> 16 : 0u; };
     uint32_t gA = load_gid(j0 + lane), gB = load_gid(j0 + kStride + lane);
     TileRec rA = load_rec(gA);
+    uint32_t kA = load_k16(gA);
     for (int j = j0 + lane; j - lane < j1; j += kStride) {
         const uint32_t g = gA;
-        const TileRec r = rA;
+        TileRec r = rA;
+        const uint32_t k16 = kA;
         gA = gB;
         rA = load_rec(gA);
+        kA = load_k16(gA);
         gB = load_gid(j + 2 * kStride);
-        if (sorted_rec && j < j1) sorted_rec[j] = r;
+        if (!FILT && sorted_rec && j < j1) sorted_rec[j] = r;
         const bool big = (r.rect & kTileRecBig) != 0u;
+        if (FILT && !big) r.mask = tile_cut_mask(r, k16, s_thr, tiles_x);
         if (!big) small_rect_tiles(r, tiles_x, [&](uint32_t t) { atomicAdd(&s_h[t >> 1], 1u << (16u * (t & 1u))); });
         for (unsigned long long bm = __ballot(big && r.mask != 0u); bm != 0ull; bm &= bm - 1ull) {
             const int b = (int)__builtin_ctzll(bm);
             const uint32_t gg = (uint32_t)__builtin_amdgcn_readlane((int)g, b), rect = (uint32_t)__builtin_amdgcn_readlane((int)r.rect, b);
+            const uint32_t kb = (uint32_t)__builtin_amdgcn_readlane((int)k16, b);
             const Splat s = splat[gg];
-            big_rect_tiles(s, rect, W, H, tiles_x, tiles_y, lane, [&](bool ok, uint32_t t) { if (ok) atomicAdd(&s_h[t >> 1], 1u << (16u * (t & 1u))); });
-        }
+            uint32_t kept = 0u;
+            big_rect_tiles(s, rect, W, H, tiles_x, tiles_y, lane, [&](bool ok, uint32_t t) {
+                if (FILT) { ok = ok && t < (uint32_t)db.T && kb <= (uint32_t)s_thr[t]; kept += (uint32_t)__popcll(__ballot(ok)); }
+                if (ok) atomicAdd(&s_h[t >> 1], 1u << (16u * (t & 1u)));
+            });
+            if (FILT && lane == b) r.mask = kept;
+        }
+        if (FILT && j < j1) tc.frec[j] = r;
     }
     __syncthreads();
     uint32_t* const row = reinterpret_cast<uint32_t*>(db.M + (size_t)c * db.Tp);
@@ -1318,7 +1430,7 @@
                                                       const uint32_t* __restrict__ sorted_gid, const TileRec* __restrict__ sorted_rec,
                                                       const Splat* __restrict__ splat, uint32_t* __restrict__ list, uint2* __restrict__ ranges,
                                                       uint32_t cap, const uint32_t* __restrict__ dkey = nullptr, uint2* __restrict__ pairs = nullptr,
-                                                      ListCut cut = ListCut{})
+                                                      ListCut cut = ListCut{}, const uint16_t* __restrict__ thr = nullptr)
 {
     static_assert(!CUT || !PAIRS, "the list cut serves the plain direct binning");
     extern __shared__ unsigned long long s_dyn[];
@@ -1409,6 +1521,10 @@
         const uint32_t g = gA;
         TileRec r = rA;
         const uint32_t kd = kA;
+        auto kept = [&](bool ok, uint32_t t, int bl) -> bool {
+            if (!PAIRS || thr == nullptr) return ok;
+            return ok && t < (uint32_t)db.T && ((uint32_t)__builtin_amdgcn_readlane((int)kd, bl) >> 16) <= (uint32_t)thr[t];
+        };
         gA = gB; rA = rB; kA = kB;
         gB = load_gid(j + 128);
         rB = load_rec(j + 128);
@@ -1437,7 +1553,7 @@
                 const uint32_t gg = (uint32_t)__builtin_amdgcn_readlane((int)g, bl), rect = (uint32_t)__builtin_amdgcn_readlane((int)r.rect, bl);
                 uint32_t o = (uint32_t)__builtin_amdgcn_readlane((int)(incl - cnt), bl) - before;
                 const Splat s = splat[gg];
-                big_rect_tiles(s, rect, W, H, tiles_x, tiles_y, lane, [&](bool ok, uint32_t t) {
+                big_rect_tiles(s, rect, W, H, tiles_x, tiles_y, lane, [&](bool ok, uint32_t t) { ok = kept(ok, t, bl);
                     const unsigned long long acc = __ballot(ok);
                     if (ok) {
                         if (with_or) atomicOr(&s_mask[t], 1ull << bl);
@@ -1457,7 +1573,7 @@
             const int bl = (int)__builtin_ctzll(bm);
             const uint32_t gg = (uint32_t)__builtin_amdgcn_readlane((int)g, bl), rect = (uint32_t)__builtin_amdgcn_readlane((int)r.rect, bl);
             const Splat s = splat[gg];
-            big_rect_tiles(s, rect, W, H, tiles_x, tiles_y, lane, [&](bool ok, uint32_t t) { if (ok && t < (uint32_t)db.T) atomicOr(&s_mask[t], 1ull << bl); });
+            big_rect_tiles(s, rect, W, H, tiles_x, tiles_y, lane, [&](bool ok, uint32_t t) { ok = kept(ok, t, bl); if (ok && t < (uint32_t)db.T) atomicOr(&s_mask[t], 1ull << bl); });
         }
         asm volatile("" : "+v"(gA), "+v"(rA.mask), "+v"(rA.rect));
         if (PAIRS) asm volatile("" : "+v"(kA));
@@ -1510,7 +1626,7 @@
             const int bl = (int)__builtin_ctzll(bm);
             const uint32_t gg = (uint32_t)__builtin_amdgcn_readlane((int)g, bl), rect = (uint32_t)__builtin_amdgcn_readlane((int)r.rect, bl);
             const Splat s = splat[gg];
-            big_rect_tiles(s, rect, W, H, tiles_x, tiles_y, lane, [&](bool ok, uint32_t t) {
+            big_rect_tiles(s, rect, W, H, tiles_x, tiles_y, lane, [&](bool ok, uint32_t t) { ok = kept(ok, t, bl);
                 if (ok && t < (uint32_t)db.T) {
                     const uint32_t pos = s_cnt[t] + (uint32_t)__popcll(s_mask[t] & ((1ull << bl) - 1ull));
                     if (pos < cap) {
@@ -1546,14 +1662,14 @@
                 const int bl = (int)__builtin_ctzll(bm);
                 const uint32_t gg = (uint32_t)__builtin_amdgcn_readlane((int)g, bl), rect = (uint32_t)__builtin_amdgcn_readlane((int)r.rect, bl);
                 const Splat s = splat[gg];
-                big_rect_tiles(s, rect, W, H, tiles_x, tiles_y, lane, [&](bool ok, uint32_t t) { if (ok && t < (uint32_t)db.T) { atomicAdd(&s_cnt[t], 1u); s_mask[t] = 0ull; } });
+                big_rect_tiles(s, rect, W, H, tiles_x, tiles_y, lane, [&](bool ok, uint32_t t) { ok = kept(ok, t, bl); if (ok && t < (uint32_t)db.T) { atomicAdd(&s_cnt[t], 1u); s_mask[t] = 0ull; } });
             }
         }
         for (unsigned long long bm = huges; bm != 0ull; bm &= bm - 1ull) {
             const int bl = (int)__builtin_ctzll(bm);
             const uint32_t gg = (uint32_t)__builtin_amdgcn_readlane((int)g, bl), rect = (uint32_t)__builtin_amdgcn_readlane((int)r.rect, bl);
             const Splat s = splat[gg];
-            big_rect_tiles(s, rect, W, H, tiles_x, tiles_y, lane, [&](bool ok, uint32_t t) { if (ok && t < (uint32_t)db.T) { atomicAdd(&s_cnt[t], 1u); s_mask[t] = 0ull; } });
+            big_rect_tiles(s, rect, W, H, tiles_x, tiles_y, lane, [&](bool ok, uint32_t t) { ok = kept(ok, t, bl); if (ok && t < (uint32_t)db.T) { atomicAdd(&s_cnt[t], 1u); s_mask[t] = 0ull; } });
         }
         lds_order();
         DB_T(5);
@@ -1720,45 +1836,33 @@
     else tile_sort_wave<16, GATHER>(src, dst, n, dkey, s_mask, s_cnt, s_start, s_keys, s_vals);
 }
 
-template <int THREADS, bool GATHER = false>
-__global__ __launch_bounds__(THREADS) void k_tile_sort(const uint2* __restrict__ ranges, uint2* pairs, uint2* pairs_alt, uint32_t* list, int T,
-                                                       const uint32_t* __restrict__ dkey = nullptr)
-{
-    constexpr int WAVES = THREADS / 64, CAP = THREADS == 256 ? kTsSmallMax : kTsCap;
+template <int THREADS>
+struct TileSortLds {
+    static constexpr int WAVES = THREADS / 64, CAP = kTsCap;
+    static_assert(THREADS == 1024, "the short segments are k_tile_sort_wave's");
     static_assert(CAP * 8 == WAVES * 256 * 8, "the pair buffer aliases the mask tables exactly");
-    __shared__ unsigned long long s_mask[WAVES][256];
-    __shared__ uint32_t s_cnt[WAVES][256];
-    __shared__ uint32_t s_start[256], s_wsum[WAVES], s_bits[2 * WAVES], s_base[256], s_hist[256];
+    unsigned long long s_mask[WAVES][256];
+    uint32_t s_cnt[WAVES][256];
+    uint32_t s_start[256], s_wsum[WAVES], s_bits[2 * WAVES], s_base[256], s_hist[256];
+};
+
+template <int THREADS, bool GATHER, int MIN_IPT = 2>
+__device__ __forceinline__ void tile_sort_block(TileSortLds<THREADS>& L, uint2* src, uint2* alt, uint32_t* dst_list, const uint32_t n,
+                                                const uint32_t* __restrict__ dkey)
+{
+    constexpr int WAVES = THREADS / 64, CAP = kTsCap;
+    auto& s_mask = L.s_mask; auto& s_cnt = L.s_cnt; auto& s_start = L.s_start; auto& s_wsum = L.s_wsum; auto& s_bits = L.s_bits;
+    auto& s_base = L.s_base; auto& s_hist = L.s_hist;
     uint32_t* const s_keys = reinterpret_cast<uint32_t*>(&s_mask[0][0]);
     uint32_t* const s_vals = s_keys + CAP;
-    static_assert(THREADS == 1024, "the short segments are k_tile_sort_wave's");
-    __shared__ uint32_t s_todo[256];
-    __shared__ uint32_t s_ntodo;
-    if (threadIdx.x == 0) s_ntodo = 0u;
-    __syncthreads();
-    for (int k = (int)threadIdx.x; (int)blockIdx.x + k * (int)gridDim.x < T; k += THREADS) {
-        const int tt = (int)blockIdx.x + k * (int)gridDim.x;
-        const uint2 q = ranges[tt];
-        if (q.y - q.x > (uint32_t)kTsSmallMax) { const uint32_t slot = atomicAdd(&s_ntodo, 1u); if (slot < 256u) s_todo[slot] = (uint32_t)tt; }
-    }
-    __syncthreads();
-    const uint32_t ntodo = s_ntodo;
-    const bool walk_all = ntodo > 256u;
-    const int nloop = walk_all ? (T - (int)blockIdx.x + (int)gridDim.x - 1) / (int)gridDim.x : (int)ntodo;
-    for (int it = 0; it < nloop; it++) {
-    const int t = walk_all ? (int)blockIdx.x + it * (int)gridDim.x : (int)s_todo[it];
-    const uint2 rg = ranges[t];
-    const uint32_t n = rg.y - rg.x;
-    if (n <= (uint32_t)kTsSmallMax) continue;
-    __syncthreads();
-    if (n <= 2048u) { tile_sort_regs<THREADS, 2, GATHER>(pairs + rg.x, list + rg.x, n, dkey, s_mask, s_cnt, s_keys, s_vals, s_start, s_wsum, s_bits); continue; }
-    if (n <= (uint32_t)kTsCap) { tile_sort_regs<THREADS, 4, GATHER>(pairs + rg.x, list + rg.x, n, dkey, s_mask, s_cnt, s_keys, s_vals, s_start, s_wsum, s_bits); continue; }
+    if (MIN_IPT <= 1 && n <= 1024u) { tile_sort_regs<THREADS, 1, GATHER>(src, dst_list, n, dkey, s_mask, s_cnt, s_keys, s_vals, s_start, s_wsum, s_bits); return; }
+    if (n <= 2048u) { tile_sort_regs<THREADS, 2, GATHER>(src, dst_list, n, dkey, s_mask, s_cnt, s_keys, s_vals, s_start, s_wsum, s_bits); return; }
+    if (n <= (uint32_t)kTsCap) { tile_sort_regs<THREADS, 4, GATHER>(src, dst_list, n, dkey, s_mask, s_cnt, s_keys, s_vals, s_start, s_wsum, s_bits); return; }
     const int tid = threadIdx.x, wave = tid >> 6, lane = tid & 63;
     constexpr int IPT = kTsCap / THREADS;
-    uint2* src = pairs + rg.x;
-    uint2* dst = pairs_alt + rg.x;
+    uint2* dst = alt;
     if (GATHER) {
-        for (uint32_t i = (uint32_t)tid; i < n; i += THREADS) { const uint32_t g = list[rg.x + i]; src[i] = make_uint2(dkey[g], g); }
+        for (uint32_t i = (uint32_t)tid; i < n; i += THREADS) { const uint32_t g = dst_list[i]; src[i] = make_uint2(dkey[g], g); }
         __syncthreads();
     }
     uint32_t k_or = 0u, k_and = 0xffffffffu;
@@ -1815,8 +1919,121 @@
         uint2* tmp = src; src = dst; dst = tmp;
     }
     __syncthreads();
-    for (uint32_t i = (uint32_t)tid; i < n; i += THREADS) list[rg.x + i] = src[i].y;
-    }
+    for (uint32_t i = (uint32_t)tid; i < n; i += THREADS) dst_list[i] = src[i].y;
+}
+
+template <int THREADS, bool GATHER = false>
+__global__ __launch_bounds__(THREADS) void k_tile_sort(const uint2* __restrict__ ranges, uint2* pairs, uint2* pairs_alt, uint32_t* list, int T,
+                                                       const uint32_t* __restrict__ dkey = nullptr)
+{
+    __shared__ TileSortLds<THREADS> L;
+    __shared__ uint32_t s_todo[256];
+    __shared__ uint32_t s_ntodo;
+    if (threadIdx.x == 0) s_ntodo = 0u;
+    __syncthreads();
+    for (int k = (int)threadIdx.x; (int)blockIdx.x + k * (int)gridDim.x < T; k += THREADS) {
+        const int tt = (int)blockIdx.x + k * (int)gridDim.x;
+        const uint2 q = ranges[tt];
+        if (q.y - q.x > (uint32_t)kTsSmallMax) { const uint32_t slot = atomicAdd(&s_ntodo, 1u); if (slot < 256u) s_todo[slot] = (uint32_t)tt; }
+    }
+    __syncthreads();
+    const uint32_t ntodo = s_ntodo;
+    const bool walk_all = ntodo > 256u;
+    const int nloop = walk_all ? (T - (int)blockIdx.x + (int)gridDim.x - 1) / (int)gridDim.x : (int)ntodo;
+    for (int it = 0; it < nloop; it++) {
+    const int t = walk_all ? (int)blockIdx.x + it * (int)gridDim.x : (int)s_todo[it];
+    const uint2 rg = ranges[t];
+    const uint32_t n = rg.y - rg.x;
+    if (n <= (uint32_t)kTsSmallMax) continue;
+    __syncthreads();
+    tile_sort_block<THREADS, GATHER>(L, pairs + rg.x, pairs_alt + rg.x, list + rg.x, n, dkey);
+    }
+}
+
+__device__ __forceinline__ bool tilerec_has_tile(const TileRec& r, const uint32_t g, const Splat* __restrict__ splat, const int tx, const int ty,
+                                                 const int W, const int H, const int tiles_x, const int tiles_y)
+{
+    if (r.rect & kTileRecBig) {
+        if (r.mask == 0u) return false;
+        const Splat sp = splat[g];
+        int bx0, by0, bx1, by1;
+        tile_rect_tight(sp.px, sp.py, sp.radius, sp.ca, sp.cb, sp.cc, sp.op, W, H, tiles_x, tiles_y, bx0, by0, bx1, by1);
+        if (tx < bx0 || tx >= bx1 || ty < by0 || ty >= by1) return false;
+        return tile_accept(make_tile_test(sp.px, sp.py, sp.ca, sp.cb, sp.cc, sp.op), tx, ty, W, H);
+    }
+    const uint32_t ww = (r.rect >> 24) & 63u, rx0 = r.rect & 0xfffu, ry0 = (r.rect >> 12) & 0xfffu;
+    const uint32_t dx = (uint32_t)tx - rx0, dy = (uint32_t)ty - ry0, bit = dy * ww + dx;
+    return dx < ww && dy < 32u && bit < 32u && ((r.mask >> bit) & 1u) != 0u;
+}
+
+__global__ __launch_bounds__(256) void k_tile_cut_count(TileCutCall tc, TileCutHdr* hdr, const unsigned long long* __restrict__ kept_total, int N,
+                                                        int W, int H, int tiles_x, int tiles_y, const TileRec* __restrict__ rec,
+                                                        const Splat* __restrict__ splat)
+{
+    if (blockIdx.x == 0 && threadIdx.x == 0 && tc.ctl[5] != 0u) hdr->stats[3] += *kept_total;
+    if (tc.ctl[2] == 0u) return;
+    const int t = (int)blockIdx.x;
+    if (tc.flag[t] == 0u) return;
+    __shared__ uint32_t s_w[4];
+    const int tid = threadIdx.x, tx = t % tiles_x, ty = t / tiles_x;
+    uint32_t c = 0u;
+    for (int j = tid; j < N; j += 256) c += tilerec_has_tile(rec[j], (uint32_t)j, splat, tx, ty, W, H, tiles_x, tiles_y) ? 1u : 0u;
+    const uint32_t inc = wave_inclusive_sum(c);
+    if ((tid & 63) == 63) s_w[tid >> 6] = inc;
+    __syncthreads();
+    if (tid == 0) tc.cnt[t] = s_w[0] + s_w[1] + s_w[2] + s_w[3];
+}
+
+__global__ __launch_bounds__(1024) void k_tile_cut_repair(TileCutCall tc, TileCutHdr* hdr, int N, int T, int W, int H, int tiles_x, int tiles_y,
+                                                          const TileRec* __restrict__ rec, const Splat* __restrict__ splat,
+                                                          const uint32_t* __restrict__ dkey, uint2* pairs, uint2* pairs_alt, uint32_t pcap,
+                                                          uint32_t* list, uint32_t lbase2, uint32_t lcap, uint2* __restrict__ ranges)
+{
+    if (tc.ctl[2] == 0u) return;
+    const int t = (int)blockIdx.x;
+    if (tc.flag[t] == 0u) return;
+    __shared__ TileSortLds<1024> L;
+    __shared__ uint32_t s_w[16], s_run;
+    const int tid = threadIdx.x, lane = tid & 63, wave = tid >> 6, tx = t % tiles_x, ty = t / tiles_x;
+    uint32_t before = 0u;
+    for (int q = tid; q < t; q += 1024) before += (tc.cnt[q] + 127u) & ~127u;
+    {
+        const uint32_t inc = wave_inclusive_sum(before);
+        if (lane == 63) s_w[wave] = inc;
+        if (tid == 0) s_run = 0u;
+        __syncthreads();
+        before = 0u;
+#pragma unroll
+        for (int w = 0; w < 16; w++) before += s_w[w];
+        __syncthreads();
+    }
+    const uint32_t n = tc.cnt[t], off = before;
+    if (tid == 0) {
+        atomicAdd(&hdr->stats[2], 1ull);
+        if (atomicAdd(&tc.ctl[7], 1u) == 0u) atomicAdd(&hdr->stats[1], 1ull);
+    }
+    if (n == 0u || (unsigned long long)off + n > pcap || (unsigned long long)lbase2 + off + n > lcap) {
+        if (tid == 0) ranges[t] = make_uint2(0u, 0u);
+        return;
+    }
+    uint2* const seg = pairs + off;
+    const unsigned long long lt = lanemask_lt();
+    for (int j0 = 0; j0 < N; j0 += 1024) {
+        const int j = j0 + tid;
+        const bool in = j < N && tilerec_has_tile(rec[j], (uint32_t)j, splat, tx, ty, W, H, tiles_x, tiles_y);
+        const unsigned long long b = __ballot(in);
+        if (lane == 0) s_w[wave] = (uint32_t)__popcll(b);
+        __syncthreads();
+        uint32_t pos = s_run, tot = 0u;
+#pragma unroll
+        for (int w = 0; w < 16; w++) { const uint32_t c = s_w[w]; pos += w < wave ? c : 0u; tot += c; }
+        if (in) { const uint32_t p = pos + (uint32_t)__popcll(b & lt); if (p < n) seg[p] = make_uint2(dkey[j], (uint32_t)j); }
+        __syncthreads();
+        if (tid == 0) s_run += tot;
+    }
+    __syncthreads();
+    tile_sort_block<1024, false, 1>(L, seg, pairs_alt + off, list + lbase2 + off, n, nullptr);
+    if (tid == 0) ranges[t] = make_uint2(lbase2 + off, lbase2 + off + n);
 }
 
 #ifdef GSR_K6_TIMING
@@ -3477,6 +3694,9 @@
 
 struct ViewCostCache { int dev, W, H, items; uint8_t* mem; size_t bytes; };
 static std::vector<ViewCostCache> g_view_costs;
+struct TileCutCache { int dev, W, H; uint8_t* mem; size_t bytes; std::map<long long, int> seen_n; };
+static std::vector<TileCutCache> g_tile_cuts;
+static std::atomic<long long> g_tile_cut_renders{0}, g_tile_cut_full_pairs{0};
 static std::map<std::tuple<int, int, int, int>, bool> g_full_depth_sort;
 
 struct PinSlot { unsigned long long* host = nullptr; unsigned long long* dev = nullptr; bool busy = false;
@@ -3691,6 +3911,9 @@
         std::lock_guard<std::mutex> lk(g_state_mutex);
         for (auto& c : g_view_costs)
             if (c.dev == dev_id && hipMemset(c.mem, 0, c.bytes) != hipSuccess) return GSR_ERR_HIP;
+        for (auto& c : g_tile_cuts)
+            if (c.dev == dev_id) { c.seen_n.clear(); if (hipMemset(c.mem, 0, c.bytes) != hipSuccess) return GSR_ERR_HIP; }
+        g_tile_cut_renders = 0; g_tile_cut_full_pairs = 0;
         return GSR_OK;
     }
     if (!strcmp(name, "debug_late_bias")) {
@@ -3714,7 +3937,7 @@
     return GSR_ERR_ARG;
 }
 
-struct DirectBinScratch { size_t M, GT, tbase, bsum, cut_chunk, cut_tend, cut_flag, cut_ctl, cut_bkey, cut_hist, bytes; };
+struct DirectBinScratch { size_t M, GT, tbase, bsum, cut_chunk, cut_tend, cut_flag, cut_ctl, cut_bkey, cut_hist, tc_thr, tc_zero, tc_mark, tc_cnt, bytes; };
 static bool direct_bin_geometry(int N, int T, DirectBin& db, DirectBinScratch& ds)
 {
     if (N < 1 || T < 1 || T > kDbMaxTiles) return false;
@@ -3751,6 +3974,10 @@
     ds.cut_ctl = o; o += 256;
     ds.cut_bkey = o; o += align256((size_t)db.NC * sizeof(uint32_t));
     ds.cut_hist = o; o += align256((size_t)db.NC * sizeof(uint32_t));
+    ds.tc_thr = o; o += align256((size_t)db.Tp * sizeof(uint16_t));
+    ds.tc_zero = o; o += align256((size_t)db.Tp * sizeof(uint32_t));
+    ds.tc_mark = o; o += align256((size_t)(db.Tp + 1) * sizeof(uint32_t));
+    ds.tc_cnt = o; o += align256((size_t)db.Tp * sizeof(uint32_t));
     ds.bytes = o;
     return true;
 }
@@ -3790,6 +4017,7 @@
     BlendBalance bb = {};
     ListCut lc = {};
     uint64_t lc_capacity = 0;
+    uint64_t tc_capacity = 0;
     Splat* splat = static_cast<Splat*>(a->geom);
     float* img = static_cast<float*>(a->image);
     uint8_t* img_base = static_cast<uint8_t*>(a->image);
@@ -3826,18 +4054,25 @@
     DirectBinScratch dbs = {};
     const bool direct = opt.direct_binning && !wide_keys && direct_bin_geometry(N, T, db, dbs);
     bool tsort = false;
+    bool tcut_rec = false, tcut = false;
+    TileCutHdr* tc_hdr = nullptr;
+    uint32_t* tc_rows = nullptr;
+    TileCutCall tcc = {};
+    auto tc_lbase2 = [&](uint64_t capacity) -> uint64_t { return ((capacity + 127) & ~127ull) + 128ull * ((uint64_t)T + 2); };
+    auto list_capacity = [&](uint64_t capacity) -> uint64_t { return (tcut && capacity > 0) ? tc_lbase2(capacity) + capacity + 128ull * (uint64_t)T : capacity; };
+    auto pair_capacity = [&](uint64_t capacity) -> uint64_t { return tcut ? capacity + 128ull * (uint64_t)T : capacity; };
     uint2* ranges = nullptr;
     uint32_t* list = nullptr;
     uint2 *pairs = nullptr, *pairs_alt = nullptr;
     auto alloc_binning = [&](uint64_t capacity) -> int {
-        B = bin_layout((int64_t)capacity, W, H, NB);
+        B = bin_layout((int64_t)list_capacity(capacity), W, H, NB);
         bin = static_cast<uint8_t*>(ro ? a->alloc(B.ckpt, GSR_ALLOC_SCRATCH, a->alloc_user) : a->alloc(B.bytes, GSR_ALLOC_BINNING, a->alloc_user));
         if (!bin) return fail(GSR_ERR_ALLOC, "binning allocation failed%s");
         ranges = reinterpret_cast<uint2*>(bin + B.ranges);
         list = reinterpret_cast<uint32_t*>(bin + B.list);
         bs = nullptr;
         if (capacity > 0 && tsort) {
-            const size_t pb = align256((size_t)capacity * sizeof(uint2));
+            const size_t pb = align256((size_t)pair_capacity(capacity) * sizeof(uint2));
             uint8_t* pm = static_cast<uint8_t*>(a->alloc(2 * pb, GSR_ALLOC_SCRATCH, a->alloc_user));
             if (!pm) return fail(GSR_ERR_ALLOC, "pair buffer allocation failed%s");
             pairs = reinterpret_cast<uint2*>(pm);
@@ -3902,8 +4137,16 @@
             if (tsort) {
                 {
                     ProfScope ps(P_EMIT, st);
+                    if (tcut && !prezeroed) {
+                        GSR_HIP(hipMemsetAsync(tcc.flag, 0, (size_t)db.Tp * sizeof(uint32_t), st));
+                        GSR_HIP(hipMemsetAsync(tcc.ctl + 2, 0, sizeof(uint32_t), st));
+                        GSR_HIP(hipMemsetAsync(tcc.ctl + 7, 0, sizeof(uint32_t), st));
+                    }
+                    tc_capacity = capacity;
                     hipLaunchKernelGGL((k_chunk_scatter<true>), dim3(grid), dim3(64), (size_t)12 * db.Tp + 4 * kDbPairs, st, db, W, H, tiles_x, tiles_y,
-                                       (const uint32_t*)nullptr, ts_rec, splat, list, ranges, (uint32_t)std::min<uint64_t>(capacity, 0xffffffffull), ts_dkey, pairs);
+                                       (const uint32_t*)nullptr, tcut ? reinterpret_cast<const TileRec*>(fs + L.srec) : ts_rec, splat, list, ranges,
+                                       (uint32_t)std::min<uint64_t>(capacity, 0xffffffffull), ts_dkey, pairs, ListCut{},
+                                       tcut ? (const uint16_t*)tcc.thr : (const uint16_t*)nullptr);
                 }
                 ProfScope ps2(P_SORT_TILE, st);
                 hipLaunchKernelGGL(k_tile_sort_wave<false>, dim3(T), dim3(64), 0, st, ranges, pairs, list, T, (const uint32_t*)nullptr);
@@ -3911,7 +4154,7 @@
                 return GSR_OK;
             }
             ProfScope ps(P_EMIT, st);
-            if (lc.key) {
+            if (lc.key && !tcut_rec) {
                 lc_capacity = capacity;
                 hipLaunchKernelGGL((k_chunk_scatter<false, 1>), dim3(grid), dim3(64), (size_t)12 * db.Tp + 4 * kDbPairs, st, db, W, H,
                                    tiles_x, tiles_y, sorted_gid, reinterpret_cast<const TileRec*>(fs + L.srec), splat, list, ranges,
@@ -3951,6 +4194,17 @@
             hipLaunchKernelGGL(k_blend_fwd_w6, dim3(8 * 4 * slots_per_xcd(T, tiles_x)), dim3(64), 0, st, W, H, tiles_x, T, ranges, list, splat, a->bg,
                                a->out_color, a->out_depth, a->out_alpha, img, staged, ckpt, opt.ckpt_first, tiles_y, bb, a->out_color_clamped, lc, 2);
         }
+        if (tcut && tc_capacity > 0) {
+            ProfScope ps(P_CUT_REPAIR, st);
+            const uint64_t lb2 = tc_lbase2(tc_capacity);
+            hipLaunchKernelGGL(k_tile_cut_count, dim3(T), dim3(256), 0, st, tcc, tc_hdr,
+                               reinterpret_cast<const unsigned long long*>(fs + L.total), N, W, H, tiles_x, tiles_y, ts_rec, splat);
+            hipLaunchKernelGGL(k_tile_cut_repair, dim3(T), dim3(1024), 0, st, tcc, tc_hdr, N, T, W, H, tiles_x, tiles_y, ts_rec, splat, ts_dkey, pairs,
+                               pairs_alt, (uint32_t)std::min<uint64_t>(pair_capacity(tc_capacity), 0xffffffffull), list,
+                               (uint32_t)std::min<uint64_t>(lb2, 0xffffffffull), (uint32_t)std::min<uint64_t>(list_capacity(tc_capacity), 0xffffffffull), ranges);
+            hipLaunchKernelGGL(k_blend_fwd_w6, dim3(8 * 4 * slots_per_xcd(T, tiles_x)), dim3(64), 0, st, W, H, tiles_x, T, ranges, list, splat, a->bg,
+                               a->out_color, a->out_depth, a->out_alpha, img, staged, ckpt, opt.ckpt_first, tiles_y, bb, a->out_color_clamped, lc, 2);
+        }
         GSR_HIP(hipGetLastError());
         return GSR_OK;
     };
@@ -3993,6 +4247,33 @@
         const uint64_t avg = (hint > 0 ? hint : (uint64_t)N * 4u) / (uint64_t)T;
         const bool auto_ok = ts_mode == 1 && avg <= (uint64_t)opt.tile_sort_max_avg && (direct || N / std::max(1, NB) <= opt.tile_sort_emit_max_n);
         tsort = (ts_mode == 2 || auto_ok) && (direct ? NB == 1 : true);
+        const bool list_cut_on = !ro && direct && !tsort && db.NC <= 16000 && (opt.list_cut == 2 || (opt.list_cut == 1 && N >= opt.list_cut_min_n));
+        const bool tc_size = opt.tile_cut == 2 || (opt.tile_cut == 1 && opt.tile_sort != 0 && opt.tile_cut_min_avg > 0 && avg >= (uint64_t)opt.tile_cut_min_avg);
+        tcut_rec = tc_size && !ro && direct && NB == 1 && T == db.T && !a->batch && a->viewmatrix && !list_cut_on;
+        if (tcut_rec) {
+            const size_t hdr_bytes = align256(sizeof(TileCutHdr)), bytes = hdr_bytes + align256((size_t)kVcEntries * T * sizeof(uint32_t));
+            std::lock_guard<std::mutex> lk(g_state_mutex);
+            TileCutCache* cc = nullptr;
+            for (auto& c : g_tile_cuts) if (c.dev == dev_id && c.W == W && c.H == H) cc = &c;
+            if (!cc) {
+                if (g_tile_cuts.size() >= 64) { (void)hipFree(g_tile_cuts.front().mem); g_tile_cuts.erase(g_tile_cuts.begin()); }
+                uint8_t* mem = nullptr;
+                if (hipMalloc((void**)&mem, bytes) == hipSuccess && hipMemset(mem, 0, bytes) == hipSuccess) {
+                    g_tile_cuts.push_back({dev_id, W, H, mem, bytes, {}});
+                    cc = &g_tile_cuts.back();
+                } else { (void)hipGetLastError(); if (mem) (void)hipFree(mem); }
+            }
+            if (!cc) tcut_rec = false;
+            else {
+                tc_hdr = reinterpret_cast<TileCutHdr*>(cc->mem);
+                tc_rows = reinterpret_cast<uint32_t*>(cc->mem + hdr_bytes);
+                auto it = cc->seen_n.find((long long)a->view_id);
+                tcut = it != cc->seen_n.end() && it->second == N && opt.early_r && speculative;
+                if (cc->seen_n.size() > 4096) cc->seen_n.clear();
+                cc->seen_n[(long long)a->view_id] = N;
+            }
+        }
+        if (tcut) tsort = true;
     }
 
     fs = static_cast<uint8_t*>(a->alloc(align256(L.bytes) + (direct ? dbs.bytes : 0), GSR_ALLOC_SCRATCH, a->alloc_user));
@@ -4094,12 +4375,18 @@
         unsigned long long* const host_slot = publish ? pin.s->dev : nullptr;
         unsigned long long* const late_slot = publish ? nullptr : pin.s->dev + 4;
         if (direct) {
-            hipLaunchKernelGGL(k_chunk_counts, dim3(db.NC + (bal.hdr ? 8 : 0)), dim3(kEmitThreads), (size_t)2 * db.Tp, st, db, W, H,
+            const bool old_cut = lc.key && !tcut_rec;
+            if (tcut)
+                hipLaunchKernelGGL(k_chunk_counts<true>, dim3(db.NC + (bal.hdr ? 8 : 0)), dim3(kEmitThreads), (size_t)4 * db.Tp, st, db, W, H,
+                                   tiles_x, tiles_y, sorted_gid, ntiles, splat, (TileRec*)nullptr, bal, rider, ListCut{}, TileCut{tcc.thr, ts_dkey, srec});
+            else
+            hipLaunchKernelGGL(k_chunk_counts<false>, dim3(db.NC + (bal.hdr ? 8 : 0)), dim3(kEmitThreads), (size_t)2 * db.Tp, st, db, W, H,
                                tiles_x, tiles_y, sorted_gid, ntiles, splat, tsort ? (TileRec*)nullptr : srec, bal,
-                               (tsort && early_r && !publish) ? rider : OsRider{}, lc);
+                               (tsort && early_r && !publish) ? rider : OsRider{}, old_cut ? lc : ListCut{}, TileCut{});
             hipLaunchKernelGGL(k_chunk_scan1, dim3((db.Tp + 255) / 256, db.G), dim3(256), 0, st, db);
-            hipLaunchKernelGGL(k_chunk_scan2, dim3((db.Tp + 255) / 256), dim3(256), lc.key ? (size_t)db.NC * 4 : 0, st, db, total, zjobs, host_slot, seq, wo,
-                               late_slot, lc);
+            hipLaunchKernelGGL(k_chunk_scan2, dim3((db.Tp + 255) / 256), dim3(256), old_cut ? (size_t)db.NC * 4 : 0, st, db, total, zjobs,
+                               tcut ? (unsigned long long*)nullptr : host_slot, seq, wo, tcut ? (unsigned long long*)nullptr : late_slot,
+                               old_cut ? lc : ListCut{});
         } else {
             hipLaunchKernelGGL(k_tile_counts, dim3(nb + (bal.hdr ? 8 : 0)), dim3(kEmitThreads), 0, st, N, sorted_gid, ntiles, block_sums,
                                tsort ? (TileRec*)nullptr : srec, bal, nb, (tsort && early_r && !publish) ? rider : OsRider{});
@@ -4150,7 +4437,7 @@
                     bb.vm = a->viewmatrix; bb.pt = a->points_transform; bb.view_id = (long long)a->view_id;
                     bb.tol = 1e-6f * (float)opt.view_pose_tol_e6;
                     bb.items = items; bb.nslots4 = nslots4; bb.W = W; bb.H = H;
-                    if (!ro && direct && !tsort && db.NC <= 16000 && T == db.T && (opt.list_cut == 2 || (opt.list_cut == 1 && N >= opt.list_cut_min_n))) {
+                    if (!tcut_rec && !ro && direct && !tsort && db.NC <= 16000 && T == db.T && (opt.list_cut == 2 || (opt.list_cut == 1 && N >= opt.list_cut_min_n))) {
                         uint8_t* dm = fs + align256(L.bytes);
                         lc.key = reinterpret_cast<uint32_t*>(mem + vc_cut);
                         lc.owner_n = reinterpret_cast<uint32_t*>(mem + vc_own);
@@ -4170,6 +4457,19 @@
                 }
             }
         }
+        if (tcut_rec) {
+            uint8_t* dm = fs + align256(L.bytes);
+            tcc.thr = reinterpret_cast<uint16_t*>(dm + dbs.tc_thr);
+            tcc.zero = reinterpret_cast<uint32_t*>(dm + dbs.tc_zero);
+            tcc.mark = reinterpret_cast<uint32_t*>(dm + dbs.tc_mark);
+            tcc.flag = reinterpret_cast<uint32_t*>(dm + dbs.cut_flag);
+            tcc.ctl = reinterpret_cast<uint32_t*>(dm + dbs.cut_ctl);
+            tcc.cnt = reinterpret_cast<uint32_t*>(dm + dbs.tc_cnt);
+            lc = ListCut{};
+            lc.key = tc_rows; lc.cur = tcc.ctl + 4; lc.tend = tcc.zero; lc.tbase = tcc.mark; lc.flag = tcc.flag; lc.ctl = tcc.ctl;
+            hipLaunchKernelGGL(k_tile_cut_begin, dim3(1), dim3(256), 0, st, tc_hdr, tc_rows, tcc, a->viewmatrix, a->points_transform,
+                               (long long)a->view_id, 1e-6f * (float)opt.view_pose_tol_e6, N, T, db.Tp, 1e-3f * (float)opt.list_cut_margin_e3, tcut ? 1 : 0);
+        }
         if (direct) {
             uint8_t* dm = fs + align256(L.bytes);
             db.M = reinterpret_cast<uint16_t*>(dm + dbs.M); db.GT = reinterpret_cast<uint32_t*>(dm + dbs.GT); db.tbase = reinterpret_cast<uint32_t*>(dm + dbs.tbase);
@@ -4225,7 +4525,7 @@
         }
         if (fresh)
             return fail(GSR_ERR_HIP, "a radix-sort look-back gave up (status words overwritten?): the binning of this or the previous forward is invalid%s");
-        if (early_r) {
+        if (early_r && !tcut) {
             pin.s->pending = true; pin.s->pending_seq = rider.seq; pin.s->pending_R = R + (unsigned long long)late_bias; pin.s->pending_giveups = gv;
         }
     }
@@ -4259,11 +4559,12 @@
         h = std::max<uint64_t>(std::max<uint64_t>(R + R / 4, h - h / 32), 1u << 16);
         if (g_hints.size() > 4096) g_hints.clear();
     }
+    if (tcut) { g_tile_cut_renders++; g_tile_cut_full_pairs += (long long)R; }
     out->num_rendered = (int64_t)R;
     if (ro) return GSR_OK;
     out->binning = bin;
     out->binning_bytes = B.bytes;
-    out->binning_capacity = (int64_t)((speculative && R <= cap && !resorted) ? cap : R);
+    out->binning_capacity = (int64_t)list_capacity((speculative && R <= cap && !resorted) ? cap : R);
     return GSR_OK;
 }
 
@@ -4399,7 +4700,7 @@
         const float* ckpt = reinterpret_cast<const float*>(bin + B.ckpt);
         float* det_part = nullptr;
         uint8_t* det_mem = nullptr;
-        const uint32_t Rn = (uint32_t)a->num_rendered;
+        const uint32_t Rn = (uint32_t)std::max<int64_t>(a->num_rendered, a->binning_capacity);
         size_t o_part = 0, o_k0 = 0, o_k1 = 0, o_v0 = 0, o_v1 = 0, o_sort = 0, det_bytes = 0;
         if (opt.deterministic_backward) {
             size_t o = 0;
@@ -4658,6 +4959,17 @@
             return fail(GSR_ERR_HIP, "view cache read-back failed%s");
         for (int q = 0; q < 5; q++) out[q] += h.pad[2 + q];
     }
+    mems.clear();
+    {
+        std::lock_guard<std::mutex> lk(g_state_mutex);
+        for (auto& c : g_tile_cuts) if (c.dev == dev_id && c.W == W && c.H == H) mems.push_back(c.mem);
+    }
+    for (uint8_t* m : mems) {
+        unsigned long long v[3];
+        if (hipDeviceSynchronize() != hipSuccess || hipMemcpy(v, m + offsetof(TileCutHdr, stats), sizeof(v), hipMemcpyDeviceToHost) != hipSuccess)
+            return fail(GSR_ERR_HIP, "tile cut cache read-back failed%s");
+        for (int q = 0; q < 3; q++) out[q] += (int64_t)v[q];
+    }
     return GSR_OK;
 }
 
@@ -4701,6 +5013,23 @@
     if (!strcmp(name, "backward_calls")) return g_bwd_calls.load();
     if (!strcmp(name, "backward_ns")) return g_bwd_ns.load();
     if (!strcmp(name, "frozen_backward_calls")) return g_frozen_bwd_calls.load();
+    if (!strcmp(name, "tile_cut_renders")) return g_tile_cut_renders.load();
+    if (!strcmp(name, "tile_cut_pairs_full")) return g_tile_cut_full_pairs.load();
+    if (!strncmp(name, "tile_cut_", 9)) {
+        const int q = !strcmp(name, "tile_cut_cut_renders") ? 0 : !strcmp(name, "tile_cut_repaired_renders") ? 1 :
+                      !strcmp(name, "tile_cut_repaired_tiles") ? 2 : !strcmp(name, "tile_cut_pairs_written") ? 3 : -1;
+        int dev_id = 0;
+        if (q < 0 || hipGetDevice(&dev_id) != hipSuccess || hipDeviceSynchronize() != hipSuccess) return -1;
+        std::vector<uint8_t*> mems;
+        { std::lock_guard<std::mutex> lk(g_state_mutex); for (auto& c : g_tile_cuts) if (c.dev == dev_id) mems.push_back(c.mem); }
+        long long sum = 0;
+        for (uint8_t* m : mems) {
+            unsigned long long v = 0;
+            if (hipMemcpy(&v, m + offsetof(TileCutHdr, stats) + 8 * q, 8, hipMemcpyDeviceToHost) != hipSuccess) return -1;
+            sum += (long long)v;
+        }
+        return sum;
+    }
     if (!strcmp(name, "spec_callers")) { std::lock_guard<std::mutex> lk(g_state_mutex); return (int64_t)g_hints.size(); }
     return -1;
 }
diff --git a/3dgs_hierarchical_training_amd/csrc/options.h b/3dgs_hierarchical_training_amd/csrc/options.h
--- a/3dgs_hierarchical_training_amd/csrc/options.h
+++ b/3dgs_hierarchical_training_amd/csrc/options.h
@@ -26,6 +26,8 @@
     int list_cut_min_n = 2000000;
     int list_cut_margin_e3 = 50;
     int list_cut_deep = 8;
+    int tile_cut = 1;
+    int tile_cut_min_avg = 0;
     int early_r = 1;
     int blend_balance = 1;
 };
@@ -46,6 +48,7 @@
     {"view_pose_tol_e6", &Options::view_pose_tol_e6, 0, INT_MAX, Outside::Refuse},
     {"small_sort9", &Options::small_sort9, 0, INT_MAX, Outside::Refuse},
     {"prep_hist_max_n", &Options::prep_hist_max_n, INT_MIN, INT_MAX, Outside::Refuse},
+    {"tile_cut", &Options::tile_cut, 0, 2, Outside::Refuse},
     {"list_cut", &Options::list_cut, 0, 2, Outside::StoreDefault},
     {"list_cut_min_n", &Options::list_cut_min_n, 0, INT_MAX, Outside::StoreDefault},
     {"list_cut_margin_e3", &Options::list_cut_margin_e3, 0, INT_MAX, Outside::StoreDefault},
```

New measurement: 1310. About the same (-0.0%).
